# cbiffle/rtiow-rust

Hardware: AMD Instinct MI355X
Metric: Msamples/s (pixels*spp/s), book-1 random-spheres 1200x800 (higher is better)
Workload: dtype f32

## Files before the change

include/rtiow_gpu_debug.h:

```cpp
#ifndef RTIOW_GPU_DEBUG_H
#define RTIOW_GPU_DEBUG_H
#include "rtiow_gpu.h"
#ifdef __cplusplus
extern "C" {
#endif

int rtg_debug_box_plan(rtg_builder* b, const rtg_id* world, size_t n, const uint32_t* words, size_t n_records,
                       uint8_t* mask_out, size_t capacity);

int rtg_debug_production_program(rtg_builder* b, const rtg_id* world, size_t n, const uint32_t* words, size_t n_records,
                                 uint32_t* words_out, uint32_t* origin_out, uint8_t* mask_out, size_t capacity);

#ifdef __cplusplus
}
#endif
#endif
```

rtiow-rust_amd/capi.py:

```python
import ctypes as C
import math
import os
import time

import numpy as np

from . import noise

c_f32p = C.POINTER(C.c_float)
c_u32p = C.POINTER(C.c_uint32)
c_u8p = C.POINTER(C.c_uint8)

INVALID_ID = 0xFFFFFFFF
FLAG_COUNTERS = 1
FLAG_TRACE_KERNEL = 2
FLAG_PARTIAL = 4
FLAG_RESUME = 8
FLAG_SUM_SQUARES = 16
FLAG_SAMPLE_COUNTS = 32
FLAG_RETIRE = 64
RETIRE_MAX_RADIUS = 8
FLAG_DENOISE = 128
DENOISE_MAX_RADIUS = 8
DENOISE_MAX_PATCH = 3
# ... 288 lines not shown

    def copy_in(self, out=None, counts=None, retire=None):
        if out is not None:
            self.planes[...] = out
        if counts is not None:
            self.counts[...] = counts
        if retire is not None:
            C.memmove(C.addressof(self.retire), C.addressof(retire), C.sizeof(Retire))

    def copy_back(self, out=None, counts=None, retire=None):
        if out is not None:
            out[...] = self.planes
        if counts is not None:
            counts[...] = self.counts
        if retire is not None:
            C.memmove(C.addressof(retire), C.addressof(self.retire), C.sizeof(Retire))


class CountsFrame(Frame):

    def __init__(self, nx, ny, squares=False, retire=False, background=None):
        if retire and not squares:
            raise ValueError("a retire frame has two float planes: squares=True")
        super().__init__(nx, ny, squares, True, retire, background=background)


class DenoiseFrame(Frame):

    def __init__(self, nx, ny, counts=False, retire=False, denoise=None, error=False, background=None):
        super().__init__(nx, ny, True, counts, retire, denoise if _given(denoise) else True, None, error, background)


class FeaturesFrame(Frame):

    def __init__(self, nx, ny, squares=False, counts=False, retire=False, denoise=None, features=None, error=False, background=None):
        super().__init__(nx, ny, squares, counts, retire, denoise, features if _given(features) else True, error, background)


def features_frame(nx, ny, squares=False, counts=False, retire=False, denoise=None, features=None, error=False):
    return FeaturesFrame(nx, ny, squares, counts, retire, denoise, features, error)


def denoise_frame(nx, ny, counts=False, retire=False, denoise=None, error=False):
    return DenoiseFrame(nx, ny, counts, retire, denoise, error)


def counts_frame(nx, ny, squares=False, retire=False):
    return CountsFrame(nx, ny, squares, retire)


def _counts_call(out, counts, nx, ny, squares, retire=None):
    counts = np.asarray(counts)
    if counts.shape != (ny, nx):
        raise ValueError("counts= must have shape (ny, nx) = %s" % ((ny, nx),))
    if (out.dtype == np.float32 and out.flags.c_contiguous and counts.dtype == np.uint32 and counts.flags.c_contiguous
            and out.ctypes.data + out.nbytes == counts.ctypes.data
            and (retire is None or C.addressof(retire) == out.ctypes.data + retire_block_offset(nx, ny))):
        return out, None
    f = CountsFrame(nx, ny, squares, retire is not None)
    f.copy_in(out, counts, retire)
    return f.planes, f


def _host_frame(out, nx, ny, squares, kw):
    shape = (2, ny, nx, 3) if squares else (ny, nx, 3)
    if out is None:
        if _resumes(kw):
            raise ValueError("resume=True needs out= (the running sum to continue)")
        return np.zeros(shape, dtype=np.float32)
    if squares and not (isinstance(out, np.ndarray) and out.shape == shape and out.dtype == np.float32 and out.flags.c_contiguous):
        raise ValueError("squares=True needs out= a C-contiguous float32 array of shape %s" % (shape,))
    return out


def _render(supported, call, nx, ny, ns, seed, stats, out, counters, counts, retire, denoise, features, kw, exact, forward=False):
    kw = dict(kw)
    squares = kw.pop("squares", None)
    error = kw.pop("error", None)
    background = kw.pop("background", None)
    has_rt, has_dn, has_ft, has_er = _given(retire), _given(denoise), _given(features), _given(error)
    has_bg = _given(background)
    in_place = isinstance(out, Frame)
    f = None
    plain = forward and not (in_place or isinstance(counts, np.ndarray) or isinstance(retire, Retire) or has_bg
                             or isinstance(denoise, (dict, Denoise)) or isinstance(features, (dict, Features)))
    if plain:
        flags, parts = {"squares": squares, "counts": counts, "retire": retire, "denoise": denoise, "features": features}, ()
        if has_er:
            flags["error"], parts = True, ("error",)
    else:
        if has_er and not (has_dn or (in_place and out.denoise is not None)):
            raise ValueError("error=True needs denoise= (the filter writes the error plane)")
        if has_dn and not squares and (exact or not in_place):
            raise ValueError("denoise= needs squares=True (the filter reads both planes)")
        blocks = [make(x) for x, make in ((denoise, make_denoise), (features, make_features), (background, make_background))
                  if _given(x) and x is not True]
        if in_place:
            f, name = out, type(out).__name__
            if (f.nx, f.ny) != (nx, ny):
                raise ValueError("out= is a %s of another size" % name)
            if isinstance(counts, np.ndarray) or (exact and (counts is not None or retire is not None)):
                raise ValueError("out= a %s brings its own counts / retire views" % name)
            if has_ft and f.features is None:
                raise ValueError("features=: out= must be a FeaturesFrame or an array")
            if (has_dn and f.denoise is None) or (has_rt and f.retire is None):
                raise ValueError("out= a %s has no such block" % name)
            if ((squares is not None or exact) and bool(squares) != f.squares) or (
                    exact and (has_dn != (f.denoise is not None) or has_ft != (f.features is not None))):
                raise ValueError("out= a %s: squares= / denoise= / features= must say what the frame holds" % name)
            if (has_er and f.error is None) or (exact and not has_er and f.error is not None):
                raise ValueError("out= a %s: error= must say whether the frame has an error plane" % name)
            if has_bg and f.background is None:
                raise ValueError("background=: out= a %s has no background block (make the frame with background=)" % name)
            if isinstance(retire, Retire):
                blocks.append(retire)
            flags = f.flags()
        else:
            if has_rt and not (isinstance(retire, Retire) and isinstance(counts, np.ndarray) and squares):
                raise ValueError("retire= needs a Retire, squares=True and counts= a uint32 array (the call writes it)")
            if counts is not None and np.asarray(counts).shape != (ny, nx):
                raise ValueError("counts= must have shape (ny, nx) = %s" % ((ny, nx),))
            if out is None and _resumes(kw):
                raise ValueError("resume=True needs out= (the running sum to continue)")
            flags = {"squares": bool(squares), "counts": counts is not None, "retire": has_rt, "denoise": has_dn, "features": has_ft}
            if has_er:
                flags["error"] = True
            if has_bg:
                if background is True:
                    raise ValueError("background=True needs out= a frame that has the block")
                flags["background"] = True
        parts = sorted((part for part, on in flags.items() if on), key=lambda part: part != "error")
    for part in parts:
        supported(part)
    if in_place:
        for block in blocks:
            f.set_in(block)
        ret, buf = f, f.buf
    elif (has_dn or has_ft or has_bg) and not plain:
        bg = background if has_bg else None
        f = (FeaturesFrame(nx, ny, squares, counts is not None, has_rt, denoise if has_dn else None, features, has_er, bg) if has_ft else
             DenoiseFrame(nx, ny, counts is not None, has_rt, denoise, has_er, bg) if has_dn else
             Frame(nx, ny, squares, counts is not None, has_rt, background=bg))
        if not (has_dn or has_ft):
            out = _host_frame(out, nx, ny, squares, kw)
        f.copy_in(None if out is None else _host_frame(out, nx, ny, squares, kw), counts, retire if has_rt else None)
        ret, buf = f if has_dn or has_ft else out, f.buf
    else:
        ret = out = buf = _host_frame(out, nx, ny, squares, kw)
        if counts is not None and not plain:
            buf, f = _counts_call(out, counts, nx, ny, squares, retire if has_rt else None)
    p = make_params(nx, ny, ns, seed=seed, flags=FLAG_COUNTERS if stats and counters else 0, **flags, **kw)
    st = call(p, buf)
    if f is not None and not in_place:
        f.copy_back(out, counts if has_rt else None, retire if has_rt else None)
    return (ret, st.as_dict()) if stats else ret


def _adaptive_host(cast, nx, ny, ns, step, target_se, min_samples, budget_s, out, seed, stats, radius, denoise, features, kw,
                   error=False, background=None):
    if features is not None:
        f = FeaturesFrame(nx, ny, True, True, False, denoise, None, error, background) if out is None else out
        what = "features=: out= must be a FeaturesFrame(nx, ny, squares=True, counts=True, denoise=...)"
    elif denoise is not None:
        f = DenoiseFrame(nx, ny, True, error=error, background=background) if out is None else out
        what = "denoise=: out= must be a DenoiseFrame(nx, ny, counts=True)"
    else:
        f = CountsFrame(nx, ny, True, background=background) if out is None else out
        what = "out= must be a CountsFrame(nx, ny, squares=True)"
    on = {"denoise": True if denoise is not None else None, "features": True if features is not None else None}
    want = {"squares": True, "counts": True, "retire": False, "denoise": denoise is not None, "features": features is not None}
    if error:
        on["error"] = want["error"] = True
        what += " with error=True"
    if background is not None:
        on["background"] = want["background"] = True
        what += " with background="
    if not isinstance(f, Frame) or (f.nx, f.ny) != (nx, ny) or f.flags() != want:
        raise ValueError(what)
    for block in (features, denoise, background):
        if block is not None:
            f.set_in(block)
    more = () if features is None else (f,)
    f.counts[...] = ns
    active = np.ones((ny, nx), dtype=bool)
    t0 = time.perf_counter()
    done = 0
    while done < ns:
        end = min(ns, done + step)
        _, st = cast(end, seed=seed, out=f, sample_begin=done, resume=True, partial=True, squares=True, stats=True, counters=False,
                     **on, **kw)
        if features is not None:
            f.features.compute = 0
        if stats is not None:
            stats.append(st)
        done = end
        held = np.minimum(f.counts, done).astype(np.uint32)
        se = f.error.copy() if error else noise.standard_error_counts(f.planes[0], f.planes[1], held)
        if error:
            retire = noise.retire_filtered(active, done, se, f.counts, min_samples, target_se, radius=radius)
        elif radius:
            retire = noise.retire(active, done, se, min_samples, target_se, radius=radius, present=f.counts > 0)
        else:
            retire = noise.retire(active, done, se, min_samples, target_se)
        f.counts[retire] = done
        active &= ~retire
        pv = CountsFrame(nx, ny)
        pv.copy_in(f.planes[0], held)
        cast(done, seed=seed, out=pv, sample_begin=done, resume=True, **kw)
        if denoise is not None:
            yield (held, pv.planes, se, f.denoised.copy()) + more
        else:
            yield (held, pv.planes, se) + more
        if not active.any():
            return
        if budget_s is not None and time.perf_counter() - t0 >= budget_s:
            return


ERR_INVALID, ERR_EMPTY_BVH, ERR_NAN, ERR_RANGE, ERR_UNSUPPORTED, ERR_DEVICE = -1, -2, -3, -4, -5, -6


class RtError(RuntimeError):
    def __init__(self, code, msg):
        super().__init__("rt error %d: %s" % (code, msg))
        self.code = code


def _f3(v):
    return (C.c_float * 3)(float(v[0]), float(v[1]), float(v[2]))


ABI_SYMBOLS = [
    "version", "last_error", "device_count", "builder_create", "builder_destroy",
    "texture_constant", "texture_checker", "texture_perlin", "builder_set_perlin_tables",
    "material_lambertian", "material_metal", "material_dielectric", "material_diffuse_light",
    "material_isotropic", "object_sphere", "object_rect", "object_flip_normals", "object_translate",
    "object_scale", "object_rotate_y", "object_and", "object_rect_prism", "object_linear_move",
    "object_constant_medium", "object_bvh", "object_bvh_sah", "camera_look", "scene_create", "scene_destroy",
    "scene_set_option", "scene_info", "par_cast", "par_cast_device", "par_cast_multi", "multi_reset", "debug_hit_top", "debug_samples", "debug_math", "debug_flatten", "debug_flatten_pool2", "tonemap", "tonemap_device",
]


class Backend:

    def __init__(self, path, prefix):
        if not os.path.exists(path):
            raise FileNotFoundError(
                "%s not found -- build it first (python -c 'import __graft_entry__ as g; g.build()')" % path)
        self.path = path
        self.prefix = prefix
        self.lib = C.CDLL(path)
        f = self._fn
        f("last_error", C.c_char_p, [])
        f("version", C.c_char_p, [])
        f("builder_create", C.c_int, [C.POINTER(C.c_void_p)])
        f("builder_destroy", None, [C.c_void_p])
        f("texture_constant", C.c_uint32, [C.c_void_p, c_f32p])
        f("texture_checker", C.c_uint32, [C.c_void_p, C.c_uint32, C.c_uint32])
        f("texture_perlin", C.c_uint32, [C.c_void_p, C.c_float])
        f("builder_set_perlin_tables", C.c_int, [C.c_void_p, c_f32p, c_u8p, c_u8p, c_u8p])
        f("material_lambertian", C.c_uint32, [C.c_void_p, C.c_uint32])
        f("material_metal", C.c_uint32, [C.c_void_p, c_f32p, C.c_float])
        f("material_dielectric", C.c_uint32, [C.c_void_p, C.c_float])
        f("material_diffuse_light", C.c_uint32, [C.c_void_p, C.c_uint32, C.c_float])
        f("material_isotropic", C.c_uint32, [C.c_void_p, C.c_uint32])
        f("object_sphere", C.c_uint32, [C.c_void_p, C.c_float, C.c_uint32])
        f("object_rect", C.c_uint32, [C.c_void_p, C.c_int] + [C.c_float] * 5 + [C.c_uint32])
        f("object_flip_normals", C.c_uint32, [C.c_void_p, C.c_uint32])
        f("object_translate", C.c_uint32, [C.c_void_p, c_f32p, C.c_uint32])
        f("object_scale", C.c_uint32, [C.c_void_p, c_f32p, C.c_uint32])
        f("object_rotate_y", C.c_uint32, [C.c_void_p, C.c_float, C.c_uint32])
        f("object_and", C.c_uint32, [C.c_void_p, C.c_uint32, C.c_uint32])
        f("object_rect_prism", C.c_uint32, [C.c_void_p, c_f32p, c_f32p, C.c_uint32])
        f("object_linear_move", C.c_uint32, [C.c_void_p, C.c_uint32, c_f32p])
        f("object_constant_medium", C.c_uint32, [C.c_void_p, C.c_uint32, C.c_float, C.c_uint32])
        f("object_bvh", C.c_uint32, [C.c_void_p, c_u32p, C.c_size_t, C.c_float, C.c_float])
        f("object_bvh_sah", C.c_uint32, [C.c_void_p, c_u32p, C.c_size_t, C.c_float, C.c_float])
        f("camera_look", C.c_int, [c_f32p, c_f32p, c_f32p] + [C.c_float] * 6 + [C.POINTER(Camera)])
        f("scene_create", C.c_int, [C.c_void_p, c_u32p, C.c_size_t, C.c_int, C.POINTER(C.c_void_p)])
        f("scene_destroy", None, [C.c_void_p])
        self._declare_render()
        f("debug_hit_top", C.c_int, [C.c_void_p, C.c_size_t, c_f32p, C.c_uint64, C.c_float, c_f32p, c_u32p])
        f("debug_samples", C.c_int, [C.c_void_p, C.POINTER(Camera), C.POINTER(Params), C.c_size_t,
                                     c_u32p, c_u32p, c_u32p, c_f32p, c_u32p])
        f("debug_math", C.c_int, [C.c_int, C.c_int, C.c_size_t, c_f32p, c_f32p, c_f32p])
        f("tonemap", C.c_int, [C.c_int, C.c_size_t, c_f32p, c_u8p])

    def _declare_render(self):
        f = self._fn
        f("device_count", C.c_int, [C.POINTER(C.c_int)])
        f("scene_set_option", C.c_int, [C.c_void_p, C.c_char_p, C.c_int])
        f("scene_info", C.c_int, [C.c_void_p, c_u32p, c_u32p, c_u32p, C.POINTER(C.c_uint64), c_u32p])
        f("par_cast", C.c_int, [C.c_void_p, C.POINTER(Camera), C.POINTER(Params), c_f32p, C.POINTER(Stats)])
        f("par_cast_device", C.c_int, [C.c_void_p, C.POINTER(Camera), C.POINTER(Params), C.c_void_p,
                                       C.c_void_p, C.POINTER(Stats)])
        f("par_cast_multi", C.c_int, [C.POINTER(C.c_void_p), C.c_int, C.POINTER(Camera), C.POINTER(Params), c_f32p,
                                      C.POINTER(Stats)])
        f("multi_reset", C.c_int, [C.c_char_p, C.POINTER(C.c_uint64)])
        f("debug_flatten", C.c_int, [C.c_void_p, c_u32p, C.c_size_t, c_u32p, c_u32p, c_u32p, C.c_size_t])
        f("debug_flatten_pool2", C.c_int, [C.c_void_p, c_u32p, C.c_size_t, c_u32p, c_u32p, c_u32p, C.c_size_t])
        f("tonemap_device", C.c_int, [C.c_int, C.c_size_t, C.c_void_p, C.c_void_p, C.c_void_p])
        f("debug_box_plan", C.c_int, [C.c_void_p, c_u32p, C.c_size_t, c_u32p, C.c_size_t, c_u8p, C.c_size_t])
        f("debug_production_program", C.c_int, [C.c_void_p, c_u32p, C.c_size_t, c_u32p, C.c_size_t, c_u32p, c_u32p, c_u8p, C.c_size_t])

    def _fn(self, name, restype, argtypes):
        try:
            fn = getattr(self.lib, self.prefix + name)
        except AttributeError:
            def fn(*_a, _n=self.prefix + name):
                raise RtError(ERR_INVALID, "%s: symbol %s is not exported by this build" % (self.path, _n))
            setattr(self, "_" + name, fn)
            return fn
        fn.restype = restype
        fn.argtypes = argtypes
        setattr(self, "_" + name, fn)
        return fn

    def last_error(self):
        return (self._last_error() or b"").decode()

    def check(self, code):
        if code != 0:
            raise RtError(code, self.last_error())

    def check_id(self, i):
        if i == INVALID_ID:
            raise RtError(-1, self.last_error())
        return i

    def builder(self):
        return Builder(self)

    def device_count(self):
        n = C.c_int(0)
        self.check(self._device_count(C.byref(n)))
        return n.value

    def camera_look(self, look_from, look_at, up, fov, aspect, aperture, focus_dist, exposure=(0.0, 1.0)):
        cam = Camera()
        self.check(self._camera_look(_f3(look_from), _f3(look_at), _f3(up), fov, aspect, aperture,
                                     focus_dist, exposure[0], exposure[1], C.byref(cam)))
        return cam

    def par_cast_multi(self, scenes, camera, nx, ny, ns, seed=0xDEADBEEF, stats=False, out=None, counters=None, **kw):
        kw = dict(kw)
        counts, retire, denoise, features = (kw.pop(k, None) for k in ("counts", "retire", "denoise", "features"))
        return _render(lambda part: _supported(self, part), lambda p, buf: self._par_cast_multi_call(scenes, camera, p, buf),
                       nx, ny, ns, seed, stats, out, True if counters is None else counters, counts, retire, denoise, features, kw,
                       exact=False, forward=True)

    def _par_cast_multi_call(self, scenes, camera, p, buf):
        st = Stats.new()
        arr = (C.c_void_p * len(scenes))(*[s.h for s in scenes])
        self.check(self._par_cast_multi(arr, len(scenes), C.byref(camera), C.byref(p), buf.ctypes.data_as(c_f32p), C.byref(st)))
        return st

    def adaptive_multi(self, scenes, camera, nx, ny, ns, step, target_se, min_samples=16, budget_s=None, out=None, seed=0xDEADBEEF,
                       stats=None, radius=0, denoise=None, features=None, filtered_error=False, **kw):
        if step < 1:
            raise ValueError("step must be >= 1")
        if not 0 <= radius <= RETIRE_MAX_RADIUS:
            raise ValueError("radius must be in 0 .. %d" % RETIRE_MAX_RADIUS)
        if filtered_error:
            _supported(self, "error")
        _supported(self, "squares")
        _supported(self, "counts")
        if filtered_error and not _given(denoise):
            raise ValueError("filtered_error=True needs denoise= (the filter writes the error plane)")
        features = make_features(features) if _given(features) else None
        denoise = make_denoise(denoise) if _given(denoise) else None
        background = kw.pop("background", None)
        if _given(background):
            _supported(self, "background")
        background = make_background(background) if _given(background) else None
        yield from _adaptive_host(lambda n, **k: self.par_cast_multi(scenes, camera, nx, ny, n, **k), nx, ny, ns, step,
                                  target_se, min_samples, budget_s, out, seed, stats, radius, denoise, features, kw, bool(filtered_error),
                                  background)

    def multi_reset(self, rccl_library=None):
        n = C.c_uint64(0)
        self.check(self._multi_reset(rccl_library.encode() if rccl_library else None, C.byref(n)))
        return n.value

    def tonemap(self, img, device=0):
        x = np.ascontiguousarray(img, dtype=np.float32)
        out = np.empty(x.shape, dtype=np.uint8)
        self.check(self._tonemap(device, x.size, x.ctypes.data_as(c_f32p), out.ctypes.data_as(c_u8p)))
        return out

    def debug_math(self, op, x, y=None, device=0):
        x = np.ascontiguousarray(x, dtype=np.float32)
        out = np.empty_like(x)
        yp = None
        if y is not None:
            y = np.ascontiguousarray(y, dtype=np.float32)
            yp = y.ctypes.data_as(c_f32p)
        self.check(self._debug_math(device, op, x.size, x.ctypes.data_as(c_f32p), yp,
                                    out.ctypes.data_as(c_f32p)))
        return out


class Builder:

    def __init__(self, backend):
        self.be = backend
        h = C.c_void_p()
        backend.check(backend._builder_create(C.byref(h)))
        self.h = h
        self._scenes = []

    def close(self):
        if self.h:
            self.be._builder_destroy(self.h)
            self.h = None

    def __del__(self):
        try:
            self.close()
        except Exception:
            pass

    def constant(self, color):
        return self.be.check_id(self.be._texture_constant(self.h, _f3(color)))

    def checker(self, t0, t1):
        return self.be.check_id(self.be._texture_checker(self.h, t0, t1))

    def perlin(self, scale):
        return self.be.check_id(self.be._texture_perlin(self.h, scale))

    def set_perlin_tables(self, vecs, perm_x, perm_y, perm_z):
        vecs = np.ascontiguousarray(vecs, dtype=np.float32).reshape(768)
        px, py, pz = (np.ascontiguousarray(a, dtype=np.uint8) for a in (perm_x, perm_y, perm_z))
        self.be.check(self.be._builder_set_perlin_tables(
            self.h, vecs.ctypes.data_as(c_f32p), px.ctypes.data_as(c_u8p), py.ctypes.data_as(c_u8p),
            pz.ctypes.data_as(c_u8p)))

    def lambertian(self, albedo):
        return self.be.check_id(self.be._material_lambertian(self.h, albedo))

    def metal(self, albedo, fuzz):
        return self.be.check_id(self.be._material_metal(self.h, _f3(albedo), fuzz))

    def dielectric(self, ref_idx):
        return self.be.check_id(self.be._material_dielectric(self.h, ref_idx))

    def diffuse_light(self, emission, brightness):
        return self.be.check_id(self.be._material_diffuse_light(self.h, emission, brightness))

    def isotropic(self, albedo):
        return self.be.check_id(self.be._material_isotropic(self.h, albedo))

    def sphere(self, radius, material):
        return self.be.check_id(self.be._object_sphere(self.h, radius, material))

    def rect(self, orthogonal_to, range0, range1, k, material):
        return self.be.check_id(self.be._object_rect(self.h, orthogonal_to, range0[0], range0[1],
                                                     range1[0], range1[1], k, material))

    def flip_normals(self, obj):
        return self.be.check_id(self.be._object_flip_normals(self.h, obj))

    def translate(self, offset, obj):
        return self.be.check_id(self.be._object_translate(self.h, _f3(offset), obj))

    def scale(self, factor, obj):
        return self.be.check_id(self.be._object_scale(self.h, _f3(factor), obj))

    def rotate_y(self, degrees, obj):
        return self.be.check_id(self.be._object_rotate_y(self.h, degrees, obj))

    def and_(self, a, b):
        return self.be.check_id(self.be._object_and(self.h, a, b))

    def rect_prism(self, p0, p1, material):
        return self.be.check_id(self.be._object_rect_prism(self.h, _f3(p0), _f3(p1), material))

    def linear_move(self, obj, motion):
        return self.be.check_id(self.be._object_linear_move(self.h, obj, _f3(motion)))

    def constant_medium(self, boundary, density, material):
        return self.be.check_id(self.be._object_constant_medium(self.h, boundary, density, material))

    def bvh(self, objs, exposure=(0.0, 1.0)):
        arr = (C.c_uint32 * max(1, len(objs)))(*objs)
        return self.be.check_id(self.be._object_bvh(self.h, arr, len(objs), exposure[0], exposure[1]))

    def flatten(self, world):
        arr = (C.c_uint32 * max(1, len(world)))(*world)
        n, feat = C.c_uint32(), C.c_uint32()
        self.be.check(self.be._debug_flatten(self.h, arr, len(world), C.byref(n), C.byref(feat), None, 0))
        words = np.zeros((n.value, 8), dtype=np.uint32)
        self.be.check(self.be._debug_flatten(self.h, arr, len(world), C.byref(n), C.byref(feat),
                                             words.ctypes.data_as(c_u32p), n.value))
        return words, feat.value

    def flatten_pool2(self, world):
        arr = (C.c_uint32 * max(1, len(world)))(*world)
        n = C.c_uint32()
        table = np.zeros(24, dtype=np.uint32)
        self.be.check(self.be._debug_flatten_pool2(self.h, arr, len(world), C.byref(n), table.ctypes.data_as(c_u32p), None, 0))
        words = np.zeros((n.value, 8), dtype=np.uint32)
        self.be.check(self.be._debug_flatten_pool2(self.h, arr, len(world), C.byref(n), table.ctypes.data_as(c_u32p),
                                                   words.ctypes.data_as(c_u32p), n.value))
        items = [tuple(int(v) for v in table[4 * k:4 * k + 4]) for k in range(int(table[20]))]
        return words, items, int(table[21]), int(table[22])

    def box_plan(self, world=None, words=None):
        if words is not None:
            words = np.ascontiguousarray(words, dtype=np.uint32)
            mask = np.zeros(len(words), dtype=np.uint8)
            n = self.be._debug_box_plan(None, None, 0, words.ctypes.data_as(c_u32p), len(words), mask.ctypes.data_as(c_u8p), len(mask))
        else:
            arr = (C.c_uint32 * max(1, len(world)))(*world)
            n = self.be._debug_box_plan(self.h, arr, len(world), None, 0, None, 0)
            if n < 0:
                self.be.check(n)
            mask = np.zeros(n, dtype=np.uint8)
            n = self.be._debug_box_plan(self.h, arr, len(world), None, 0, mask.ctypes.data_as(c_u8p), len(mask))
        if n < 0:
            self.be.check(n)
        return mask

    def production_program(self, world=None, words=None):
        if words is not None:
            words = np.ascontiguousarray(words, dtype=np.uint32)
            head = (None, None, 0, words.ctypes.data_as(c_u32p), len(words))
            n = len(words)
        else:
            arr = (C.c_uint32 * max(1, len(world)))(*world)
            head = (self.h, arr, len(world), None, 0)
            n = self.be._debug_production_program(*head, None, None, None, 0)
            if n < 0:
                self.be.check(n)
        out = np.zeros((n, 8), dtype=np.uint32)
        origin = np.zeros(n, dtype=np.uint32)
        mask = np.zeros(n, dtype=np.uint8)
        n = self.be._debug_production_program(*head, out.ctypes.data_as(c_u32p), origin.ctypes.data_as(c_u32p), mask.ctypes.data_as(c_u8p), n)
        if n < 0:
            self.be.check(n)
        return out, origin, mask

    def bvh_sah(self, objs, exposure=(0.0, 1.0)):
        arr = (C.c_uint32 * max(1, len(objs)))(*objs)
        return self.be.check_id(self.be._object_bvh_sah(self.h, arr, len(objs), exposure[0], exposure[1]))

    def scene(self, world, device=0):
        arr = (C.c_uint32 * max(1, len(world)))(*world)
        h = C.c_void_p()
        self.be.check(self.be._scene_create(self.h, arr, len(world), device, C.byref(h)))
        sc = self.be.scene_class(self.be, h, self)
        sc.apply_env_options()
        return sc


class Scene:
    def __init__(self, backend, handle, builder):
        self.be = backend
        self.h = handle
        self._builder = builder

    def close(self):
        if self.h:
            self.be._scene_destroy(self.h)
            self.h = None

    def __del__(self):
        try:
            self.close()
        except Exception:
            pass

    ENV_OPTIONS = ("kernel", "chunks", "lpt", "lpt_phase1", "lpt_deep", "lpt_shift", "ray_lds", "sync", "block", "wg_per_cu", "window",
                   "box_leave", "refill_min", "gather_min", "run_ahead", "run_ahead_min", "sphere_min", "verbose", "bvh4", "box_chains", "box_prune", "box_tree", "force_rccl", "multi_gather", "multi_planes", "scratch_mb", "frames_in_flight", "small_frames", "drain_share", "hoist", "deep_sized", "mat_lds", "pool2", "p2_refill", "p2_box_leave", "p2_park", "p2_sphere", "p2_prism", "p2_list", "p2_push", "light_sampling")

    def set_option(self, name, value):
        self.be.check(self.be._scene_set_option(self.h, name.encode(), int(value)))

    def apply_env_options(self):
        if not hasattr(self.be, "_scene_set_option"):
            return
        for name in self.ENV_OPTIONS:
            v = os.environ.get("RTG_" + name.upper())
            if v is not None:
                self.set_option(name, int(v))

    def info(self):
        a, b, c, d, e = C.c_uint32(), C.c_uint32(), C.c_uint32(), C.c_uint64(), C.c_uint32()
        self.be.check(self.be._scene_info(self.h, C.byref(a), C.byref(b), C.byref(c), C.byref(d), C.byref(e)))
        return {"instructions": a.value, "materials": b.value, "textures": c.value, "hbm_bytes": d.value, "box_followers": e.value}

    def _par_cast_args(self, args, threads):
        return args

    def par_cast(self, camera, nx, ny, ns, seed=0xDEADBEEF, stats=False, out=None, threads=0, counts=None, counters=None,
                 retire=None, denoise=None, features=None, **kw):
        def call(p, buf):
            st = Stats.new()
            self.be.check(self.be._par_cast(*self._par_cast_args(
                [self.h, C.byref(camera), C.byref(p), buf.ctypes.data_as(c_f32p), C.byref(st)], threads)))
            return st
        return _render(lambda part: _supported(self.be, part), call, nx, ny, ns, seed, stats, out,
                       stats if counters is None else counters, counts, retire, denoise, features, kw, exact=True)

    def par_cast_device(self, camera, params, d_out_ptr, stream=None, want_stats=False, sample_begin=None, partial=None,
                        resume=None, squares=None, counts=None, retire=None, denoise=None, features=None, error=None,
                        background=None):
        if _given(background) and background is not True:
            background = make_background(background)
        over = {"squares": squares, "counts": counts, "retire": retire, "denoise": denoise, "features": features, "error": error,
                "background": background}
        bits = {"squares": FLAG_SUM_SQUARES, "counts": FLAG_SAMPLE_COUNTS, "retire": FLAG_RETIRE, "denoise": FLAG_DENOISE,
                "features": FLAG_FEATURES, "error": FLAG_DENOISE_ERROR, "background": FLAG_BACKGROUND}
        has = {part: bool(params.flags & bits[part] if on is None else on if isinstance(on, (bool, int)) else True)
               for part, on in over.items()}
        for part in ("background", "error", "features", "denoise", "squares", "counts", "retire"):
            if has[part] if part == "squares" else _given(over[part]):
                _supported(self.be, part)
        if has["error"] and not has["denoise"]:
            raise ValueError("error=True needs the denoise part (the filter writes the error plane)")
        lay = FrameLayout(params.nx, params.ny, **has)
        blocks = [(over[part], 4 * at, n) for part, at, n in (("retire", lay.retire, C.sizeof(Retire)),
                                                             ("denoise", lay.denoise, Denoise.OUT_OFFSET),
                                                             ("features", lay.features, Features.OUT_OFFSET),
                                                             ("background", lay.background, Background.OUT_OFFSET))
                  if isinstance(over[part], C.Structure)]
        for block, at, n in blocks:
            self._block_copy(d_out_ptr, block, stream, True, at, n)
        if _given(counts) and counts is not True:
            self._upload_counts(lay, counts, d_out_ptr, stream)
        if sample_begin is not None or partial is not None or resume is not None or any(on is not None for on in over.values()):
            q = Params()
            C.pointer(q)[0] = params
            if sample_begin is not None:
                q.sample_begin = sample_begin
            for on, bit in [(partial, FLAG_PARTIAL), (resume, FLAG_RESUME)] + [(on if on is None else has[part], bits[part])
                                                                             for part, on in over.items()]:
                if on is not None:
                    q.flags = (q.flags | bit) if on else (q.flags & ~bit)
            params = q
        st = Stats.new()
        self.be.check(self.be._par_cast_device(self.h, C.byref(camera), C.byref(params), d_out_ptr, stream,
                                               C.byref(st) if want_stats else None))
        for block, at, _ in blocks:
            self._block_copy(d_out_ptr, block, stream, False, at, C.sizeof(block))
        return st.as_dict() if want_stats else None

    def _block_copy(self, d_out_ptr, block, stream, to_device, offset, nbytes):
        hip, hs = _hip_runtime(), _stream(stream)
        dev, host = C.c_void_p(_device_ptr(d_out_ptr) + offset), C.c_void_p(C.addressof(block))
        what = "hipMemcpyAsync(%s block)" % type(block).__name__.lower()
        _hip_ok(hip.hipMemcpyAsync(*((dev, host, nbytes, 1) if to_device else (host, dev, nbytes, 2)), hs), what)
        _hip_ok(hip.hipStreamSynchronize(hs), what)

    def _upload_counts(self, lay, counts, d_out_ptr, stream):
        hip, hs = _hip_runtime(), _stream(stream)
        dst = C.c_void_p(_device_ptr(d_out_ptr) + 4 * lay.counts)
        if hasattr(counts, "data_ptr") and getattr(counts, "is_cuda", False):
            if tuple(counts.shape) != (lay.ny, lay.nx) or counts.element_size() != 4 or not counts.is_contiguous():
                raise ValueError("counts= must be a contiguous 4-byte [ny, nx] tensor")
            _hip_ok(hip.hipMemcpyAsync(dst, C.c_void_p(counts.data_ptr()), 4 * lay.n, 3, hs), "hipMemcpyAsync(count plane)")
        else:
            host = np.ascontiguousarray(counts, dtype=np.uint32)
            if host.shape != (lay.ny, lay.nx):
                raise ValueError("counts= must have shape (ny, nx) = %s" % ((lay.ny, lay.nx),))
            _hip_ok(hip.hipMemcpyAsync(dst, C.c_void_p(host.ctypes.data), 4 * lay.n, 1, hs), "hipMemcpyAsync(count plane)")
            _hip_ok(hip.hipStreamSynchronize(hs), "hipMemcpyAsync(count plane)")

    def _loop_block(self, part, given, make):
        if not _given(given):
            return None
        _supported(self.be, part)
        return make(given)

    def adaptive(self, camera, nx, ny, ns, step, target_se, min_samples=16, budget_s=None, out=None, seed=0xDEADBEEF,
                 stats=None, radius=0, preview=None, stream=None, denoise=None, denoised=None, features=None,
                 filtered_error=False, **kw):
        if step < 1:
            raise ValueError("step must be >= 1")
        if filtered_error:
            _supported(self.be, "error")
        _supported(self.be, "squares")
        _supported(self.be, "counts")
        if not 0 <= radius <= RETIRE_MAX_RADIUS:
            raise ValueError("radius must be in 0 .. %d" % RETIRE_MAX_RADIUS)
        if filtered_error and not _given(denoise):
            raise ValueError("filtered_error=True needs denoise= (the filter writes the error plane)")
        features, denoise = self._loop_block("features", features, make_features), self._loop_block("denoise", denoise, make_denoise)
        background = self._loop_block("background", kw.pop("background", None), make_background)
        if out is not None and not isinstance(out, Frame):
            _supported(self.be, "retire")
            if preview is None:
                raise ValueError("a device frame needs a device preview buffer (preview=)")
            if denoise is not None and denoised is None:
                raise ValueError("denoise= on a device frame needs a device buffer for the filtered frame (denoised=)")
            yield from self._adaptive_device(camera, nx, ny, ns, step, target_se, min_samples, budget_s, out, seed, stats,
                                             radius, preview, stream, kw, denoise, denoised, features, bool(filtered_error), background)
            return
        yield from _adaptive_host(lambda n, **k: self.par_cast(camera, nx, ny, n, **k), nx, ny, ns, step, target_se,
                                  min_samples, budget_s, out, seed, stats, radius, denoise, features, kw, bool(filtered_error), background)

    def _adaptive_device(self, camera, nx, ny, ns, step, target_se, min_samples, budget_s, out, seed, stats, radius, preview,
                         stream, kw, denoise=None, denoised=None, features=None, error=False, background=None):
        hip, hs, ok = _hip_runtime(), _stream(stream), _hip_ok
        d_out, d_pv = _device_ptr(out), _device_ptr(preview)
        lay = FrameLayout(nx, ny, True, True, True, denoise is not None, features is not None, error, background is not None)
        if background is not None:
            self._block_copy(d_out, background, stream, True, 4 * lay.background, Background.OUT_OFFSET)
        plane, counts_at = lay.n, d_out + 4 * lay.counts
        ok(hip.hipMemsetD32Async(C.c_void_p(counts_at), ns - (1 << 32) if ns >= 1 << 31 else ns, plane, hs), "hipMemsetD32Async(counts)")
        block = Retire(target_se=float(target_se), min_samples=int(min_samples), radius=int(radius))
        self._block_copy(d_out, block, stream, True, 4 * lay.retire, C.sizeof(Retire))
        if denoise is not None:
            self._block_copy(d_out, denoise, stream, True, 4 * lay.denoise, Denoise.OUT_OFFSET)
        more = ()
        if features is not None:
            self._block_copy(d_out, features, stream, True, 4 * lay.features, Features.OUT_OFFSET)
            more = (4 * lay.features,)
        t0 = time.perf_counter()
        done = 0
        while done < ns:
            end = min(ns, done + step)
            st = self.par_cast_device(camera, make_params(nx, ny, end, seed=seed, sample_begin=done, resume=True, partial=True,
                                                          squares=True, counts=True, retire=True, denoise=denoise is not None,
                                                          features=features is not None, error=error,
                                                          background=background is not None, **kw), d_out, hs,
                                      want_stats=stats is not None)
            if features is not None and features.compute:
                features.compute = 0
                self._block_copy(d_out, features, stream, True, 4 * lay.features, Features.OUT_OFFSET)
            if denoise is not None:
                ok(hip.hipMemcpyAsync(C.c_void_p(_device_ptr(denoised)), C.c_void_p(d_out + 4 * lay.denoised), plane * 3 * 4, 3, hs),
                   "hipMemcpyAsync(denoised)")
            if stats is not None:
                stats.append(st)
            done = end
            ok(hip.hipMemcpyAsync(C.c_void_p(d_pv), C.c_void_p(d_out), plane * 3 * 4, 3, hs), "hipMemcpyAsync(preview)")
            ok(hip.hipMemcpyAsync(C.c_void_p(d_pv + plane * 3 * 4), C.c_void_p(counts_at), plane * 4, 3, hs), "hipMemcpyAsync(preview counts)")
            self.par_cast_device(camera, make_params(nx, ny, done, seed=seed, sample_begin=done, resume=True, counts=True, **kw),
                                 d_pv, hs)
            self._block_copy(d_out, block, stream, False, 4 * lay.retire, C.sizeof(Retire))
            info = block.as_dict()
            if denoise is not None:
                yield (done, preview, info, denoised) + more
            else:
                yield (done, preview, info) + more
            if info["active"] == 0:
                return
            if budget_s is not None and time.perf_counter() - t0 >= budget_s:
                return

    def progressive(self, camera, nx, ny, ns, step, seed=0xDEADBEEF, budget_s=None, out=None, preview=None, stream=None,
                    squares=False, target_rmse=None, denoise=None, denoised=None, features=None, **kw):
        if step < 1:
            raise ValueError("step must be >= 1")
        features = self._loop_block("features", features, make_features)
        background = self._loop_block("background", kw.pop("background", None), make_background)
        squares = bool(squares) or target_rmse is not None or _given(denoise)
        if squares:
            _supported(self.be, "squares")
        denoise = self._loop_block("denoise", denoise, make_denoise)
        if out is not None and not isinstance(out, np.ndarray):
            if target_rmse is not None:
                raise ValueError("target_rmse needs host frames: there is no device-side error reduction")
            if preview is None:
                raise ValueError("a device running sum needs a device preview buffer (preview=)")
            if denoise is not None and denoised is None:
                raise ValueError("denoise= on a device frame needs a device buffer for the filtered frame (denoised=)")
            yield from self._progressive_device(camera, nx, ny, ns, step, seed, budget_s, out, preview, stream, squares, kw,
                                                denoise, denoised, features, background)
            return
        shape = (2, ny, nx, 3) if squares else (ny, nx, 3)
        acc = np.zeros(shape, dtype=np.float32) if out is None else out
        frame = None
        if features is not None:
            frame = FeaturesFrame(nx, ny, squares, denoise=denoise, features=features, background=background)
        elif denoise is not None:
            frame = DenoiseFrame(nx, ny, denoise=denoise, background=background)
        elif background is not None:
            frame = Frame(nx, ny, squares, background=background)
        if frame is not None:
            frame.copy_in(acc)
        on = {"denoise": True if denoise is not None else None, "features": True if features is not None else None}
        if background is not None:
            on["background"] = True
        more = () if features is None else (frame,)
        sums = acc[0] if squares else acc
        t0 = time.perf_counter()
        done = 0
        while done < ns:
            end = min(ns, done + step)
            self.par_cast(camera, nx, ny, end, seed=seed, out=acc if frame is None else frame, sample_begin=done, resume=True, partial=True,
                          squares=squares, **on, **kw)
            if frame is not None:
                frame.copy_back(acc)
            if features is not None:
                frame.features.compute = 0
            done = end
            pv = sums.copy()
            self.par_cast(camera, nx, ny, done, seed=seed, out=pv, sample_begin=done, resume=True, **kw)
            if squares:
                se = noise.standard_error(acc[0], acc[1], done)
                if denoise is not None:
                    yield (done, pv, se, frame.denoised.copy()) + more
                else:
                    yield (done, pv, se) + more
                if target_rmse is not None and float(np.sqrt(np.mean(se * se))) <= target_rmse:
                    return
            else:
                yield (done, pv) + more
            if budget_s is not None and time.perf_counter() - t0 >= budget_s:
                return

    def _progressive_device(self, camera, nx, ny, ns, step, seed, budget_s, acc, preview, stream, squares, kw, denoise=None,
                            denoised=None, features=None, background=None):
        hip, hs = _hip_runtime(), _stream(stream)
        d_acc, d_preview = C.c_void_p(_device_ptr(acc)), C.c_void_p(_device_ptr(preview))
        lay = FrameLayout(nx, ny, squares, False, False, denoise is not None, features is not None, background=background is not None)
        if background is not None:
            self._block_copy(acc, background, stream, True, 4 * lay.background, Background.OUT_OFFSET)
        if denoise is not None:
            self._block_copy(acc, denoise, stream, True, 4 * lay.denoise, Denoise.OUT_OFFSET)
        more = ()
        if features is not None:
            self._block_copy(acc, features, stream, True, 4 * lay.features, Features.OUT_OFFSET)
            more = (4 * lay.features,)
        t0 = time.perf_counter()
        done = 0
        while done < ns:
            end = min(ns, done + step)
            self.par_cast_device(camera, make_params(nx, ny, end, seed=seed, sample_begin=done, resume=True, partial=True,
                                                     squares=squares, denoise=denoise is not None, features=features is not None,
                                                     background=background is not None, **kw), d_acc, hs)
            if features is not None and features.compute:
                features.compute = 0
                self._block_copy(acc, features, stream, True, 4 * lay.features, Features.OUT_OFFSET)
            done = end
            if denoise is not None:
                _hip_ok(hip.hipMemcpyAsync(C.c_void_p(_device_ptr(denoised)), C.c_void_p(d_acc.value + 4 * lay.denoised), lay.n * 3 * 4, 3, hs),
                        "hipMemcpyAsync(denoised)")
            _hip_ok(hip.hipMemcpyAsync(d_preview, d_acc, lay.n * 3 * 4, 3, hs), "hipMemcpyAsync(preview)")
            self.par_cast_device(camera, make_params(nx, ny, done, seed=seed, sample_begin=done, resume=True, **kw), d_preview, hs)
            if denoise is not None:
                yield (done, preview, acc, denoised) + more
            else:
                yield ((done, preview, acc) if squares else (done, preview)) + more
            if budget_s is not None:
                _hip_ok(hip.hipStreamSynchronize(hs), "hipStreamSynchronize")
                if time.perf_counter() - t0 >= budget_s:
                    return

    def debug_hit_top(self, rays, seed=1, t_near=0.001):
        rays = np.ascontiguousarray(rays, dtype=np.float32).reshape(-1, 7)
        n = rays.shape[0]
        out = np.zeros((n, 8), dtype=np.float32)
        mat = np.zeros(n, dtype=np.uint32)
        self.be.check(self.be._debug_hit_top(self.h, n, rays.ctypes.data_as(c_f32p), seed, t_near,
                                             out.ctypes.data_as(c_f32p), mat.ctypes.data_as(c_u32p)))
        return out, mat

    def debug_samples(self, camera, nx, ny, ns, xs, ys, samples, seed=0xDEADBEEF, trace_kernel=False, **kw):
        p = make_params(nx, ny, ns, seed=seed, flags=FLAG_TRACE_KERNEL if trace_kernel else 0, **kw)
        xs, ys, samples = (np.ascontiguousarray(a, dtype=np.uint32) for a in (xs, ys, samples))
        n = xs.size
        rgb = np.zeros((n, 3), dtype=np.float32)
        info = np.zeros((n, 4), dtype=np.uint32)
        self.be.check(self.be._debug_samples(self.h, C.byref(camera), C.byref(p), n,
                                             xs.ctypes.data_as(c_u32p), ys.ctypes.data_as(c_u32p),
                                             samples.ctypes.data_as(c_u32p), rgb.ctypes.data_as(c_f32p),
                                             info.ctypes.data_as(c_u32p)))
        return rgb, info


Backend.scene_class = Scene
```

rtiow-rust_amd/csrc/rt_box_plan.h:

```cpp
#pragma once
#include <cmath>
#include <cstddef>
#include <cstdint>
#include <cstring>
#include <vector>

#include "flat_scene.h"

namespace rtg {

constexpr uint8_t BOX_KEPT = 0, BOX_FOLLOWER = 1, BOX_PRUNED = 2;
#ifndef RT_BOX_PLAN_PROBES
#define RT_BOX_PLAN_PROBES 256
#endif
#ifndef RT_BOX_PLAN_FULL
#define RT_BOX_PLAN_FULL 0
#endif
constexpr uint32_t BOX_PLAN_PROBES = RT_BOX_PLAN_PROBES;
constexpr bool BOX_PLAN_FULL = RT_BOX_PLAN_FULL != 0;
enum BoxPlanKind : int { BOX_PLAN_SURE = 0, BOX_PLAN_PROBE_DP = 1, BOX_PLAN_AREA = 2 };
constexpr BoxPlanKind BOX_PLAN_DEFAULT = BOX_PLAN_FULL ? BOX_PLAN_PROBE_DP : BOX_PLAN_SURE;
#ifndef RT_BOX_TREE_PLAN
#define RT_BOX_TREE_PLAN 2
#endif
constexpr BoxPlanKind BOX_TREE_PLAN = (BoxPlanKind)(RT_BOX_TREE_PLAN);

struct BoxPlan {
  uint32_t n_pruned = 0;
  uint32_t n_sure = 0;
  uint32_t n_rays = 0;
};

namespace box_plan_detail {
inline float as_f(uint32_t u) {
  float f;
  std::memcpy(&f, &u, 4);
  return f;
}
inline bool aabb_hit(const uint32_t* lo, const uint32_t* hi, const float* o, const float* inv, float t_near, float best) {
  const float mn[3] = {as_f(lo[0]), as_f(lo[2]), as_f(hi[0])}, mx[3] = {as_f(lo[1]), as_f(lo[3]), as_f(hi[1])};
  float t0[3], t1[3];
  for (int a = 0; a < 3; a++) {
    const float u = (mn[a] - o[a]) * inv[a], v = (mx[a] - o[a]) * inv[a];
    t0[a] = inv[a] < 0.f ? v : u, t1[a] = inv[a] < 0.f ? u : v;
  }
  const float start = fmaxf(t_near, fmaxf(fmaxf(t0[0], t0[1]), t0[2]));
  const float end = fminf(best, fminf(fminf(t1[0], t1[1]), t1[2]));
  return end > start;
}
inline bool sphere_hit(const uint32_t* lo, uint32_t flags, const float* o, const float* d, float dd, float t_near, float best, float* t_out) {
  float p[3] = {o[0], o[1], o[2]};
  if (flags & F_TRANSLATE)
    for (int a = 0; a < 3; a++) p[a] = o[a] - as_f(lo[a]);
  const float r = as_f(lo[3]);
  const float b = p[0] * d[0] + p[1] * d[1] + p[2] * d[2];
  const float c = p[0] * p[0] + p[1] * p[1] + p[2] * p[2] - r * r;
  const float disc = b * b - dd * c;
  if (disc > 0.f) {
    const float sq = sqrtf(disc);
    float t = (-b - sq) / dd;
    if (t < best && t >= t_near) return *t_out = t, true;
    t = (-b + sq) / dd;
    if (t < best && t >= t_near) return *t_out = t, true;
  }
  return false;
}
struct Rng {
  uint64_t s;
  uint64_t next() {
    uint64_t z = (s += 0x9e3779b97f4a7c15ull);
    z = (z ^ (z >> 30)) * 0xbf58476d1ce4e5b9ull;
    z = (z ^ (z >> 27)) * 0x94d049bb133111ebull;
    return z ^ (z >> 31);
  }
  float unit() { return (float)(next() >> 40) * (1.f / 16777216.f); }
  void in_unit_sphere(float* v) {
    do {
      for (int a = 0; a < 3; a++) v[a] = 2.f * unit() - 1.f;
    } while (v[0] * v[0] + v[1] * v[1] + v[2] * v[2] >= 1.f);
  }
};
inline bool finite6(const uint32_t* lo, const uint32_t* hi) {
  return std::isfinite(as_f(lo[0])) && std::isfinite(as_f(lo[1])) && std::isfinite(as_f(lo[2])) && std::isfinite(as_f(lo[3])) &&
         std::isfinite(as_f(hi[0])) && std::isfinite(as_f(hi[1]));
}
inline double box_area(const uint32_t* lo, const uint32_t* hi) {
  const double dx = (double)as_f(lo[1]) - (double)as_f(lo[0]), dy = (double)as_f(lo[3]) - (double)as_f(lo[2]),
               dz = (double)as_f(hi[1]) - (double)as_f(hi[0]);
  return 2.0 * (dx * dy + dy * dz + dz * dx);
}
struct Shape {
  std::vector<int32_t> parent;
  std::vector<uint32_t> depth;
  std::vector<uint8_t> prunable;
  uint32_t n_prunable = 0;
};
inline bool leaf_box_at(const uint32_t (*hi)[4], size_t n, size_t j) {
  return (hi[j][3] & 0xffu) == OP_BOX && j + 2 < n && (hi[j + 1][3] & 0xffu) == OP_SPHERE && hi[j][2] == j + 2;
}
inline bool program_shape(const uint32_t (*lo)[4], const uint32_t (*hi)[4], size_t n, Shape* sh) {
  auto op = [&](size_t j) { return hi[j][3] & 0xffu; };
  auto skip = [&](size_t j) { return (size_t)hi[j][2]; };
  sh->parent.assign(n, -1), sh->depth.assign(n, 0), sh->prunable.assign(n, 0), sh->n_prunable = 0;
  if (n < 4 || n > 0x7fffffffu) return false;
  std::vector<uint32_t> open;
  for (size_t j = 0; j < n; j++) {
    while (!open.empty() && skip(open.back()) <= j) open.pop_back();
    if (!open.empty()) sh->parent[j] = (int32_t)open.back(), sh->depth[j] = (uint32_t)open.size();
    if (op(j) != OP_BOX) continue;
    if (skip(j) <= j || skip(j) >= n || (!open.empty() && skip(j) > skip(open.back()))) return false;
    open.push_back((uint32_t)j);
  }
  auto contains = [&](size_t j, size_t c) {
    return as_f(lo[j][0]) <= as_f(lo[c][0]) && as_f(lo[j][1]) >= as_f(lo[c][1]) && as_f(lo[j][2]) <= as_f(lo[c][2]) &&
           as_f(lo[j][3]) >= as_f(lo[c][3]) && as_f(hi[j][0]) <= as_f(hi[c][0]) && as_f(hi[j][1]) >= as_f(hi[c][1]);
  };
  for (size_t j = n; j-- > 0;) {
    if (op(j) != OP_BOX || j + 1 >= n || op(j + 1) != OP_BOX) continue;
    const size_t L = j + 1, R = skip(L);
    if (!(L < R && R < skip(j)) || op(R) != OP_BOX || skip(R) != skip(j)) continue;
    if (!finite6(lo[j], hi[j]) || !finite6(lo[L], hi[L]) || !finite6(lo[R], hi[R]) || !contains(j, L) || !contains(j, R)) continue;
    if (!(leaf_box_at(hi, n, L) || sh->prunable[L]) || !(leaf_box_at(hi, n, R) || sh->prunable[R])) continue;
    sh->prunable[j] = 1, sh->n_prunable++;
  }
  return true;
}
}

inline BoxPlan box_plan(const uint32_t (*lo)[4], const uint32_t (*hi)[4], size_t n, const uint8_t* follower, uint8_t* mask,
                        uint8_t* sure = nullptr, uint32_t n_probes = BOX_PLAN_PROBES, BoxPlanKind kind = BOX_PLAN_DEFAULT) {
  using namespace box_plan_detail;
  BoxPlan out;
  for (size_t j = 0; j < n; j++) {
    mask[j] = follower && follower[j] ? BOX_FOLLOWER : BOX_KEPT;
    if (sure) sure[j] = 0;
  }
  auto op = [&](size_t j) { return hi[j][3] & 0xffu; };
  auto skip = [&](size_t j) { return (size_t)hi[j][2]; };
  Shape shape;
  if (!program_shape(lo, hi, n, &shape) || !shape.n_prunable) return out;
  const std::vector<int32_t>& parent = shape.parent;
  const std::vector<uint32_t>& depth = shape.depth;
  const std::vector<uint8_t>& prunable = shape.prunable;
  auto leaf_box = [&](size_t j) { return leaf_box_at(hi, n, j); };
  std::vector<uint8_t> choosable(prunable);
  for (size_t j = 0; j + 1 < n; j++) {
    if (!prunable[j] || !follower) continue;
    size_t k = j + 1;
    while (k + 1 < n && follower[k] && !leaf_box(k)) k++;
    if (follower[k] && leaf_box(k)) choosable[j] = 0;
  }

  std::vector<uint64_t> n_pass(n, 0);
  std::vector<uint32_t> spheres, starts;
  for (size_t j = 0; j < n; j++)
    if (op(j) == OP_SPHERE) spheres.push_back((uint32_t)j);
  auto centre = [&](uint32_t j, float* c) {
    for (int a = 0; a < 3; a++) c[a] = (hi[j][3] & F_TRANSLATE) ? as_f(lo[j][a]) : 0.f;
  };
  float cmin[3] = {INFINITY, INFINITY, INFINITY}, cmax[3] = {-INFINITY, -INFINITY, -INFINITY};
  for (uint32_t j : spheres) {
    float c[3];
    centre(j, c);
    for (int a = 0; a < 3; a++) cmin[a] = fminf(cmin[a], c[a]), cmax[a] = fmaxf(cmax[a], c[a]);
  }
  std::vector<uint8_t> enclosing(n, 0);
  for (uint32_t j : spheres) {
    float cj[3];
    centre(j, cj);
    const float r = as_f(lo[j][3]);
    float far2 = 0.f;
    for (int a = 0; a < 3; a++) {
      const float d = fmaxf(cmax[a] - cj[a], cj[a] - cmin[a]);
      far2 += d * d;
    }
    const bool all = spheres.size() > 1 && far2 < r * r;
    enclosing[j] = all;
    if (!all && std::isfinite(r) && std::isfinite(cj[0]) && std::isfinite(cj[1]) && std::isfinite(cj[2])) starts.push_back(j);
  }
  uint64_t n_rays = 0;
  if (!starts.empty() && kind != BOX_PLAN_AREA) {
    Rng rng{0x626f78706c616e31ull ^ (uint64_t)n};
    const float t_near = 0.001f;
    while (n_rays < n_probes) {
      const uint32_t s0 = starts[rng.next() % starts.size()];
      float c[3], nrm[3], o[3], d[3], v[3];
      centre(s0, c);
      do rng.in_unit_sphere(nrm);
      while (nrm[0] * nrm[0] + nrm[1] * nrm[1] + nrm[2] * nrm[2] < 1e-4f);
      const float len = sqrtf(nrm[0] * nrm[0] + nrm[1] * nrm[1] + nrm[2] * nrm[2]), r0 = as_f(lo[s0][3]);
      for (int a = 0; a < 3; a++) nrm[a] /= len, o[a] = c[a] + r0 * nrm[a];
      const uint32_t bounces = 1u + (uint32_t)(rng.next() % 3u);
      for (uint32_t k = 0; k <= bounces && n_rays < n_probes; k++) {
        rng.in_unit_sphere(v);
        for (int a = 0; a < 3; a++) d[a] = nrm[a] + v[a];
        const float inv[3] = {1.f / d[0], 1.f / d[1], 1.f / d[2]};
        const float dd = d[0] * d[0] + d[1] * d[1] + d[2] * d[2];
        float best = 3.402823466e+38f;
        int64_t best_pc = -1;
        n_rays++;
        for (size_t pc = 0; pc < n;) {
          const uint32_t o_ = op(pc);
          if (o_ == OP_BOX) {
            if (aabb_hit(lo[pc], hi[pc], o, inv, t_near, best)) n_pass[pc]++, pc++;
            else pc = skip(pc);
          } else if (o_ == OP_SPHERE) {
            float t;
            if (sphere_hit(lo[pc], hi[pc][3], o, d, dd, t_near, best, &t)) best = t, best_pc = (int64_t)pc;
            pc++;
          } else break;
        }
        if (best_pc < 0 || enclosing[best_pc]) break;
        centre((uint32_t)best_pc, c);
        const float r = as_f(lo[best_pc][3]);
        for (int a = 0; a < 3; a++) o[a] = o[a] + best * d[a], nrm[a] = (o[a] - c[a]) / r;
        if (!(std::isfinite(nrm[0]) && std::isfinite(nrm[1]) && std::isfinite(nrm[2]))) break;
      }
    }
  }
  out.n_rays = (uint32_t)n_rays;
  if (kind == BOX_PLAN_AREA) {
    constexpr uint64_t ONE = 1ull << 30;
    float rmin[3] = {INFINITY, INFINITY, INFINITY}, rmax[3] = {-INFINITY, -INFINITY, -INFINITY};
    for (size_t j = 0; j + 1 < n; j++) {
      if (!leaf_box(j) || enclosing[j + 1] || !finite6(lo[j], hi[j])) continue;
      const float mn[3] = {as_f(lo[j][0]), as_f(lo[j][2]), as_f(hi[j][0])}, mx[3] = {as_f(lo[j][1]), as_f(lo[j][3]), as_f(hi[j][1])};
      for (int a = 0; a < 3; a++) rmin[a] = fminf(rmin[a], mn[a]), rmax[a] = fmaxf(rmax[a], mx[a]);
    }
    const double dx = (double)rmax[0] - rmin[0], dy = (double)rmax[1] - rmin[1], dz = (double)rmax[2] - rmin[2];
    const double sa_ref = 2.0 * (dx * dy + dy * dz + dz * dx);
    if (!(sa_ref > 0.0) || !std::isfinite(sa_ref)) return out;
    for (size_t j = 0; j < n; j++) {
      if (op(j) != OP_BOX) continue;
      const double r = finite6(lo[j], hi[j]) ? box_area(lo[j], hi[j]) / sa_ref : 1.0;
      n_pass[j] = r >= 1.0 ? ONE : (r > 0.0 ? (uint64_t)(r * (double)ONE) : 0u);
    }
    n_rays = ONE;
  }

  uint64_t states = 0;
  for (size_t j = 0; kind != BOX_PLAN_SURE && j < n; j++)
    if (op(j) == OP_BOX) states += depth[j] + 2u;
  const bool dp = kind != BOX_PLAN_SURE && states <= (1ull << 26);
  std::vector<uint32_t> kidx(n, 0);
  std::vector<uint8_t> pruned(n, 0);
  if (dp) {
    std::vector<uint64_t> at(n + 1, 0);
    for (size_t j = 0; j < n; j++) at[j + 1] = at[j] + (op(j) == OP_BOX ? depth[j] + 2u : 0u);
    std::vector<uint64_t> acc(at[n], 0);
    std::vector<uint8_t> choice(at[n], 0);
    std::vector<uint64_t> path_pass, f;
    for (size_t j = n; j-- > 0;) {
      if (op(j) != OP_BOX) continue;
      const uint32_t dj = depth[j];
      uint64_t* acc_j = &acc[at[j]];
      uint8_t* choice_j = &choice[at[j]];
      path_pass.assign(dj + 1u, n_rays);
      for (int32_t a = parent[j], k = (int32_t)dj; a >= 0; a = parent[a], k--) path_pass[k] = n_pass[a];
      f.assign(dj + 1u, 0);
      for (uint32_t k = 0; k <= dj; k++) {
        const uint64_t own = follower && follower[j] ? 0u : path_pass[k];
        const uint64_t keep = own + acc_j[dj + 1u], leave = acc_j[k];
        if (choosable[j] && leave <= keep) f[k] = leave, choice_j[k] = 1;
        else f[k] = keep;
      }
      if (parent[j] >= 0) {
        uint64_t* up = &acc[at[parent[j]]];
        for (uint32_t k = 0; k <= dj; k++) up[k] += f[k];
      }
    }
    for (size_t j = 0; j < n; j++) {
      if (op(j) != OP_BOX) continue;
      const int32_t p = parent[j];
      kidx[j] = p < 0 ? 0u : (pruned[p] ? kidx[p] : depth[j]);
      pruned[j] = choice[at[j] + kidx[j]];
    }
  } else {
    for (size_t j = 0; j < n; j++) pruned[j] = choosable[j] && n_rays && n_pass[j] == n_rays && op(j) == OP_BOX;
  }
  for (size_t j = 0; j < n; j++) {
    if (!pruned[j] || mask[j] == BOX_FOLLOWER) continue;
    mask[j] = BOX_PRUNED, out.n_pruned++;
    if (n_pass[j] == n_rays) {
      out.n_sure++;
      if (sure) sure[j] = 1;
    }
  }
  return out;
}

constexpr uint32_t BOX_TREE_NEW = 0xffffffffu;
inline uint32_t box_tree_rebuild(const uint32_t (*lo)[4], const uint32_t (*hi)[4], size_t n, uint32_t (*out_lo)[4],
                                 uint32_t (*out_hi)[4], uint32_t* origin) {
  using namespace box_plan_detail;
  for (size_t j = 0; j < n; j++) {
    std::memcpy(out_lo[j], lo[j], 16), std::memcpy(out_hi[j], hi[j], 16);
    origin[j] = (uint32_t)j;
  }
  Shape shape;
  if (!program_shape(lo, hi, n, &shape) || !shape.n_prunable) return 0;
  struct Box { float mn[3], mx[3]; };
  auto merge = [](const Box& a, const Box& b) {
    Box m;
    for (int x = 0; x < 3; x++) m.mn[x] = b.mn[x] < a.mn[x] ? b.mn[x] : a.mn[x], m.mx[x] = b.mx[x] > a.mx[x] ? b.mx[x] : a.mx[x];
    return m;
  };
  auto area = [](const Box& b) {
    const double dx = (double)b.mx[0] - b.mn[0], dy = (double)b.mx[1] - b.mn[1], dz = (double)b.mx[2] - b.mn[2];
    return 2.0 * (dx * dy + dy * dz + dz * dx);
  };
  std::vector<uint32_t> leaf;
  std::vector<Box> box;
  std::vector<double> suffix;
  struct Job { uint32_t a, b, at; };
  std::vector<Job> jobs;
  std::vector<uint32_t> rec_lo, rec_hi, rec_origin;
  uint32_t regions = 0;
  for (size_t j = 0; j < n; j++) {
    if (!shape.prunable[j]) continue;
    const size_t end = hi[j][2];
    if (shape.parent[j] >= 0 && shape.prunable[shape.parent[j]]) continue;
    leaf.clear(), box.clear();
    bool ok = true;
    for (size_t i = j; i < end; i++) {
      if (!leaf_box_at(hi, n, i)) continue;
      ok = ok && finite6(lo[i], hi[i]);
      leaf.push_back((uint32_t)i);
      box.push_back(Box{{as_f(lo[i][0]), as_f(lo[i][2]), as_f(hi[i][0])}, {as_f(lo[i][1]), as_f(lo[i][3]), as_f(hi[i][1])}});
    }
    const size_t m = leaf.size();
    if (!ok || m < 2 || 3 * m - 1 != end - j) { j = end - 1; continue; }
    uint64_t budget = 64ull * m, work = 0;
    for (size_t v = m; v > 1; v >>= 1) budget += 64ull * m;
    const size_t len = end - j;
    rec_lo.assign(4 * len, 0), rec_hi.assign(4 * len, 0), rec_origin.assign(len, BOX_TREE_NEW);
    suffix.resize(m);
    jobs.clear();
    jobs.push_back(Job{0u, (uint32_t)m, 0u});
    while (!jobs.empty() && ok) {
      const Job t = jobs.back();
      jobs.pop_back();
      uint32_t* rl = &rec_lo[4 * t.at];
      uint32_t* rh = &rec_hi[4 * t.at];
      if (t.b - t.a == 1) {
        const uint32_t src = leaf[t.a];
        std::memcpy(rl, lo[src], 16), std::memcpy(rh, hi[src], 16), std::memcpy(rl + 4, lo[src + 1], 16), std::memcpy(rh + 4, hi[src + 1], 16);
        rh[2] = (uint32_t)j + t.at + 2u;
        rec_origin[t.at] = src, rec_origin[t.at + 1] = src + 1u;
        continue;
      }
      work += 2ull * (t.b - t.a);
      if (work > budget) { ok = false; break; }
      Box run = box[t.b - 1];
      for (uint32_t k = t.b - 1; k > t.a; k--) run = k == t.b - 1 ? run : merge(box[k], run), suffix[k] = area(run);
      run = box[t.a];
      uint32_t best_k = t.a + 1;
      double best_cost = INFINITY;
      for (uint32_t k = t.a + 1; k < t.b; k++) {
        if (k > t.a + 1) run = merge(run, box[k - 1]);
        const double cost = area(run) * (double)(k - t.a) + suffix[k] * (double)(t.b - k);
        if (cost < best_cost) best_cost = cost, best_k = k;
      }
      const Box all = merge(run, box[t.b - 1]);
      const float f[6] = {all.mn[0], all.mx[0], all.mn[1], all.mx[1], all.mn[2], all.mx[2]};
      std::memcpy(rl, f, 16), std::memcpy(rh, f + 4, 8);
      rh[2] = (uint32_t)j + t.at + 3u * (t.b - t.a) - 1u;
      rh[3] = t.at == 0u ? hi[j][3] : (hi[j][3] & ~F_BVH_ROOT);
      jobs.push_back(Job{best_k, t.b, t.at + 1u + 3u * (best_k - t.a) - 1u});
      jobs.push_back(Job{t.a, best_k, t.at + 1u});
    }
    if (ok) {
      for (size_t i = 0; i < len; i++) {
        std::memcpy(out_lo[j + i], &rec_lo[4 * i], 16), std::memcpy(out_hi[j + i], &rec_hi[4 * i], 16);
        origin[j + i] = rec_origin[i];
      }
      regions++;
    }
    j = end - 1;
  }
  return regions;
}

}
```

rtiow-rust_amd/csrc/rtg_api.hip:

```cpp
#include <hip/hip_runtime.h>

#include <dlfcn.h>
#include <rccl/rccl.h>

#include <chrono>
#include <cmath>
#include <cstdio>
#include <cstdlib>
#include <cstring>
#include <map>
#include <mutex>
#include <functional>
#include <string>
#include <tuple>
#include <vector>

#include "../../include/rtiow_gpu.h"
#include "../../include/rtiow_gpu_debug.h"
#include "rt_pool.h"
#include "rt_box_plan.h"
#include "rt_retire.h"
#include "rt_denoise.h"
#include "rt_features.h"
#include "rt_multi_planes.h"
#include "rt_pool_full.h"
#include "rt_sync_full.h"
#include "rt_pool2.h"
#include "rt_trace.h"
#include "rt_light.h"
#include "scene_builder.h"

using namespace rtg;

#include "rtg_kernels.inc"

namespace {
thread_local std::string g_err;

int fail(int code, const std::string& msg) {
  g_err = msg;
  return code;
}
int hip_fail(hipError_t e, const char* what) {
  return fail(RTG_ERR_DEVICE, std::string(what) + ": " + hipGetErrorString(e));
}
#define HIP_TRY(expr)                                   \
  do {                                                  \
    hipError_t e_ = (expr);                             \
    if (e_ != hipSuccess) return hip_fail(e_, #expr);   \
  } while (0)
}

struct rtg_builder {
  SceneBuilder sb;
};

constexpr int RTG_MAX_FRAMES = 4;
enum class KernelKind { baseline, lean_pool, full_pool, lock_step, pool2 };
struct LaunchCtx {
  unsigned long long* d_counters = nullptr;
  hipEvent_t ev0 = nullptr, ev1 = nullptr, done = nullptr;
  bool busy = false;
  float* d_stack = nullptr;
  size_t stack_bytes = 0;
  uint32_t* d_slots = nullptr;
  size_t slots_bytes = 0;
  float* d_scratch = nullptr;
  size_t scratch_bytes = 0;
  LaunchConsts* d_consts = nullptr;
  uint32_t* d_lpt = nullptr;
  size_t lpt_bytes = 0;
  LptQueue lpt_desc{};
  KernelKind last_kernel = KernelKind::baseline;
  uint32_t last_pix_work = 0;
  uint32_t* d_list = nullptr;
  size_t list_bytes = 0;
  uint32_t* d_compact = nullptr;
  size_t compact_bytes = 0;
  unsigned long long counts_samples = 0;
  void* d_retire = nullptr;
  size_t retire_bytes = 0;
  const char* refusal = nullptr;
  void* d_denoise = nullptr;
  size_t denoise_bytes = 0;
  uint32_t* d_features = nullptr;
  size_t features_bytes = 0;
};

struct LeanImages {
  const uint4* lo = nullptr;
  const uint4* hi = nullptr;
  const uint32_t* d_off = nullptr;
  uint32_t bytes = 0;
  uint32_t n_followers = 0;
  const uint32_t* d_chain_off = nullptr;
  uint32_t chain_bytes = 0;
  bool planned = false;
  uint32_t n_pruned = 0;
  float plan_ms = 0.f;
  const uint32_t* d_prune_off[2] = {nullptr, nullptr};
  uint32_t prune_bytes[2] = {0, 0};
  std::vector<uint32_t> plan_ops;
  std::vector<uint8_t> plan_mask;
  std::vector<uint8_t> follower;
  int slot = 12;
};

struct rtg_scene {
  int device = 0;
  DevScene dev{};
  uint32_t features = 0;
  uint32_t n_prog = 0, n_mat = 0, n_tex = 0;
  uint64_t bytes = 0;
  void* buffers[21] = {};
  const uint32_t* d_parent = nullptr;
  hipStream_t own_stream = nullptr;
  int num_cus = 0;
  float* d_frame = nullptr;
  size_t frame_bytes = 0;
  int force_chunks = 0;
  uint64_t scratch_limit = 0;
  bool whole_scratch = false;
  int verbose = 0;
  int window = -1;
  int ray_lds = 1;
  int force_rccl = 0;
  int multi_gather = 0;
  float* d_pack = nullptr;
  size_t pack_bytes = 0;
  float* d_recv = nullptr;
  size_t recv_bytes = 0;
  int multi_planes = 0;
  hipEvent_t post0 = nullptr, post1 = nullptr;
  hipEvent_t pack0 = nullptr, pack1 = nullptr, unpack0 = nullptr;
  int bvh4 = 0;
  uint32_t wide_bytes = 0;
  int box_chains = 1;
  int box_prune = 1;
  int box_tree = 1;
  LeanImages ref;
  LeanImages tree;
  bool tree_tried = false;
  float tree_ms = 0.f;
  uint32_t n_regions = 0;
  bool plannable = false;
  std::vector<Packet> h_lo, h_hi;
  int sync_full = -1;
  uint32_t n_box = 0;
  int lpt = 2;
  int lpt_deep = 4;
  int lpt_shift = 0;
  int lpt_phase1 = 0;
  int kernel_version = 3;
  PoolTuning pool_tune{40, 16, 24, 16, 16, 40};
  PoolTuning full_tune{20, 24, 32, 16, 24, 40};
  PoolTuning sync_tune{20, 16, 32, 16, 16, 40};
  int wg_per_cu = 0;
  int full_threads = 0;
  int pool_threads = 0;
  int mat_lds = 1;
  int deep_sized = 1;
  int hoist = 1;
  uint32_t seg_first = 0, seg_end = 0;
  int drain_share = 1;
  int pool2 = 1;
  uint32_t n_prog2 = 0, n_box2 = 0;
  DevScene dev2{};
  const P2Table* d_p2 = nullptr;
  Pool2Tuning pool2_tune{24, 48, 40, 4, 8, 24, 2};
  int guide_lds = 0;
  int small_frames = 1;
  int light_sampling = 0;
  uint32_t n_lights = 0;
  std::vector<LightRect> h_lights;
  std::vector<uint8_t> h_sampled;
  LightTable lights{nullptr, nullptr, 0};
  void* d_lights = nullptr;
  void* d_sampled = nullptr;
  LaunchCtx ctx[RTG_MAX_FRAMES];
  int n_ctx = 1, next_ctx = 0;
  LaunchCtx* cx = &ctx[0];
};

static void ctx_free_buffers(LaunchCtx* c) {
  if (c->busy) (void)hipEventSynchronize(c->done);
  c->busy = false;
  if (c->d_scratch) (void)hipFree(c->d_scratch);
  if (c->d_slots) (void)hipFree(c->d_slots);
  if (c->d_stack) (void)hipFree(c->d_stack);
  if (c->d_lpt) (void)hipFree(c->d_lpt);
  if (c->d_list) (void)hipFree(c->d_list);
  if (c->d_compact) (void)hipFree(c->d_compact);
  if (c->d_retire) (void)hipFree(c->d_retire);
  if (c->d_denoise) (void)hipFree(c->d_denoise);
  if (c->d_features) (void)hipFree(c->d_features);
  c->d_scratch = nullptr, c->scratch_bytes = 0, c->d_slots = nullptr, c->slots_bytes = 0;
  c->d_stack = nullptr, c->stack_bytes = 0, c->d_lpt = nullptr, c->lpt_bytes = 0;
  c->d_list = nullptr, c->list_bytes = 0, c->d_compact = nullptr, c->compact_bytes = 0;
  c->d_retire = nullptr, c->retire_bytes = 0;
  c->d_denoise = nullptr, c->denoise_bytes = 0;
  c->d_features = nullptr, c->features_bytes = 0;
}

static int ctx_acquire(rtg_scene* s) {
  LaunchCtx* c = &s->ctx[s->next_ctx];
  s->next_ctx = (s->next_ctx + 1) % s->n_ctx;
  if (!c->d_counters) {
    if (hipMalloc((void**)&c->d_counters, 64 * sizeof(unsigned long long)) != hipSuccess || hipMemset(c->d_counters, 0, 64 * sizeof(unsigned long long)) != hipSuccess ||
        hipMalloc((void**)&c->d_consts, sizeof(LaunchConsts) + sizeof(ListConsts)) != hipSuccess || hipEventCreate(&c->ev0) != hipSuccess ||
        hipEventCreate(&c->ev1) != hipSuccess || hipEventCreateWithFlags(&c->done, hipEventDisableTiming) != hipSuccess)
      return fail(RTG_ERR_DEVICE, "scene: launch-context allocation failed");
  }
  if (c->busy) {
    hipError_t e = hipEventSynchronize(c->done);
    c->busy = false;
    if (e != hipSuccess) return hip_fail(e, "hipEventSynchronize(previous frame of this launch context)");
  }
  s->cx = c;
  return RTG_OK;
}
static int ctx_release(rtg_scene* s, hipStream_t stream) {
  hipError_t e = hipEventRecord(s->cx->done, stream);
  if (e != hipSuccess) return hip_fail(e, "hipEventRecord(done)");
  s->cx->busy = true;
  return RTG_OK;
}

struct SampleSlice {
  uint32_t begin = 0;
  bool divide = true;
  bool squares = false;
  bool counts = false;
  uint32_t list_work = 0;
  ListConsts list{};
  bool retire = false;
  bool denoise = false;
  bool features = false;
  bool error = false;
  bool background = false;
  bool sliced() const { return begin != 0u || !divide; }
};
static SampleSlice slice_of(const rtg_params* p) {
  SampleSlice sl;
  if (p->flags & RTG_FLAG_RESUME) sl.begin = p->sample_begin;
  if (p->flags & RTG_FLAG_PARTIAL) sl.divide = false;
  if (p->flags & RTG_FLAG_SUM_SQUARES) sl.squares = true;
  if (p->flags & RTG_FLAG_SAMPLE_COUNTS) sl.counts = true;
  if (p->flags & RTG_FLAG_RETIRE) sl.retire = true;
  if (p->flags & RTG_FLAG_DENOISE) sl.denoise = true;
  if (p->flags & RTG_FLAG_FEATURES) sl.features = true;
  if (p->flags & RTG_FLAG_DENOISE_ERROR) sl.error = true;
  if (p->flags & RTG_FLAG_BACKGROUND) sl.background = true;
  return sl;
}

static const char* retire_refusal(const rtg_retire& r, uint32_t nranks) {
  if (r.radius > RTG_RETIRE_MAX_RADIUS) return "RTG_FLAG_RETIRE: radius > RTG_RETIRE_MAX_RADIUS";
  if (!(r.target_se >= 0.0)) return "RTG_FLAG_RETIRE: target_se is NaN or negative";
  if (r.radius > 0u && nranks > 1u) return "RTG_FLAG_RETIRE: radius > 0 needs nranks = 1 (the neighbours live on other ranks)";
  return nullptr;
}

static const char* denoise_refusal(const rtg_denoise& r, uint32_t nranks) {
  if (r.radius > RTG_DENOISE_MAX_RADIUS) return "RTG_FLAG_DENOISE: radius > RTG_DENOISE_MAX_RADIUS";
  if (r.patch > RTG_DENOISE_MAX_PATCH) return "RTG_FLAG_DENOISE: patch > RTG_DENOISE_MAX_PATCH";
  if (!(r.k > 0.f) || !std::isfinite(r.k)) return "RTG_FLAG_DENOISE: k is NaN, infinite or <= 0";
  if (r.reserved_in != 0u) return "RTG_FLAG_DENOISE: reserved_in != 0";
  if (nranks > 1u) return "RTG_FLAG_DENOISE needs nranks = 1 (the neighbours live on other ranks)";
  return nullptr;
}

static const char* features_refusal(const rtg_features& r, bool denoise) {
  if (r.grid == 0u || r.grid > RTG_FEATURES_MAX_GRID) return "RTG_FLAG_FEATURES: grid is 0 or > RTG_FEATURES_MAX_GRID";
  if (r.compute > 1u) return "RTG_FLAG_FEATURES: compute > 1";
  if (r.reserved_in != 0u) return "RTG_FLAG_FEATURES: reserved_in != 0";
  for (float sg : {r.sigma_normal, r.sigma_albedo, r.sigma_depth})
    if (denoise && (!(sg > 0.f) || !std::isfinite(sg))) return "RTG_FLAG_FEATURES with RTG_FLAG_DENOISE: a sigma is NaN, infinite or <= 0";
  return nullptr;
}

static const char* background_refusal(const rtg_background& r) {
  if (r.mode > 1u) return "RTG_FLAG_BACKGROUND: mode > 1";
  if (r.reserved_in != 0u) return "RTG_FLAG_BACKGROUND: reserved_in != 0";
  return nullptr;
}
static Background dev_background(const rtg_background& r) {
  Background b;
  b.mode = r.mode == 0u ? BG_CONSTANT : BG_GRADIENT;
  for (int c = 0; c < 3; c++) b.bottom[c] = r.bottom[c], b.top[c] = r.top[c];
  return b;
}

struct FrameBlocks {
  rtg_retire retire{};
  rtg_denoise denoise{};
  rtg_features features{};
  rtg_background background{};
};
static hipError_t read_blocks(const FrameLayout& L, const SampleSlice& sl, const float* d_out, hipStream_t stream, FrameBlocks* fb) {
  hipError_t e = hipSuccess;
  if (sl.retire) e = hipMemcpyAsync(&fb->retire, d_out + L.retire, offsetof(rtg_retire, active), hipMemcpyDeviceToHost, stream);
  if (e == hipSuccess && sl.denoise) e = hipMemcpyAsync(&fb->denoise, d_out + L.denoise, offsetof(rtg_denoise, filtered), hipMemcpyDeviceToHost, stream);
  if (e == hipSuccess && sl.features) e = hipMemcpyAsync(&fb->features, d_out + L.features, offsetof(rtg_features, traced), hipMemcpyDeviceToHost, stream);
  if (e == hipSuccess && sl.background) e = hipMemcpyAsync(&fb->background, d_out + L.background, offsetof(rtg_background, reserved), hipMemcpyDeviceToHost, stream);
  return e;
}
static const char* blocks_refusal(const SampleSlice& sl, const FrameBlocks& fb, uint32_t nranks) {
  const char* why = nullptr;
  if (sl.retire && (why = retire_refusal(fb.retire, nranks))) return why;
  if (sl.denoise && (why = denoise_refusal(fb.denoise, nranks))) return why;
  if (sl.features && (why = features_refusal(fb.features, sl.denoise))) return why;
  if (sl.background && (why = background_refusal(fb.background))) return why;
  return nullptr;
}

#include "rtg_launch.inc"

template <typename T>
struct DevBuf {
  T* p = nullptr;
  ~DevBuf() {
    if (p) (void)hipFree(p);
  }
  hipError_t alloc(size_t n) { return hipMalloc((void**)&p, (n ? n : 1) * sizeof(T)); }
};

extern "C" {

const char* rtg_version(void) { return "rtiow-rust_amd 0.2 (gfx950 HIP; flat-program ray-pool kernels; flat-program encoding 3: OP_SEG = 9, OP_SAVE / OP_MERGE / OP_EXT = 10 / 11 / 12, OP_LIST = 13, MEDIUM lo.y = 1 / density)"; }
const char* rtg_last_error(void) { return g_err.c_str(); }

int rtg_device_count(int* n) {
  if (!n) return fail(RTG_ERR_INVALID, "null argument");
  int c = 0;
  hipError_t e = hipGetDeviceCount(&c);
  if (e != hipSuccess) {
    *n = 0;
    return hip_fail(e, "hipGetDeviceCount");
  }
  *n = c;
  return RTG_OK;
}

int rtg_builder_create(rtg_builder** out) {
  if (!out) return fail(RTG_ERR_INVALID, "null argument");
  *out = new rtg_builder();
  return RTG_OK;
}
void rtg_builder_destroy(rtg_builder* b) { delete b; }

static rtg_id bad(const char* msg) {
  fail(RTG_ERR_INVALID, msg);
  return RTG_INVALID_ID;
}

rtg_id rtg_texture_constant(rtg_builder* b, const float rgb[3]) {
  if (!b || !rgb) return bad("null argument");
  HostTexture t;
  t.kind = TEX_CONSTANT;
  t.rgb[0] = rgb[0], t.rgb[1] = rgb[1], t.rgb[2] = rgb[2];
  b->sb.textures.push_back(t);
  return (rtg_id)b->sb.textures.size() - 1;
}
rtg_id rtg_texture_checker(rtg_builder* b, rtg_id t0, rtg_id t1) {
  if (!b) return bad("null argument");
  if (t0 >= b->sb.textures.size() || t1 >= b->sb.textures.size()) return bad("checker: bad texture handle");
  HostTexture t;
  t.kind = TEX_CHECKER;
  t.t0 = t0, t.t1 = t1;
  b->sb.textures.push_back(t);
  return (rtg_id)b->sb.textures.size() - 1;
}
rtg_id rtg_texture_perlin(rtg_builder* b, float scale) {
  if (!b) return bad("null argument");
  if (!b->sb.has_perlin) return bad("perlin: call rtg_builder_set_perlin_tables first");
  HostTexture t;
  t.kind = TEX_PERLIN;
  t.scale = scale;
  b->sb.textures.push_back(t);
  return (rtg_id)b->sb.textures.size() - 1;
}
int rtg_builder_set_perlin_tables(rtg_builder* b, const float vecs[768], const uint8_t px[256],
                                  const uint8_t py[256], const uint8_t pz[256]) {
  if (!b || !vecs || !px || !py || !pz) return fail(RTG_ERR_INVALID, "null argument");
  for (int i = 0; i < 256; i++) {
    b->sb.perlin_vecs[4 * i] = vecs[3 * i], b->sb.perlin_vecs[4 * i + 1] = vecs[3 * i + 1];
    b->sb.perlin_vecs[4 * i + 2] = vecs[3 * i + 2], b->sb.perlin_vecs[4 * i + 3] = 0.f;
    b->sb.perlin_perm[i] = px[i], b->sb.perlin_perm[256 + i] = py[i], b->sb.perlin_perm[512 + i] = pz[i];
  }
  b->sb.has_perlin = true;
  return RTG_OK;
}

static rtg_id push_material(rtg_builder* b, uint32_t kind, rtg_id tex, const float* albedo, float param) {
  if (!b) return bad("null argument");
  HostMaterial m;
  m.kind = kind;
  if (tex != RTG_INVALID_ID) {
    if (tex >= b->sb.textures.size()) return bad("material: bad texture handle");
    m.tex = tex;
  }
  if (albedo) m.albedo[0] = albedo[0], m.albedo[1] = albedo[1], m.albedo[2] = albedo[2];
  m.param = param;
  b->sb.materials.push_back(m);
  return (rtg_id)b->sb.materials.size() - 1;
}
rtg_id rtg_material_lambertian(rtg_builder* b, rtg_id albedo) {
  if (albedo == RTG_INVALID_ID) return bad("material: bad texture handle");
  return push_material(b, MAT_LAMBERTIAN, albedo, nullptr, 0.f);
}
rtg_id rtg_material_metal(rtg_builder* b, const float albedo[3], float fuzz) {
  if (!albedo) return bad("null argument");
  return push_material(b, MAT_METAL, RTG_INVALID_ID, albedo, fuzz);
}
rtg_id rtg_material_dielectric(rtg_builder* b, float ref_idx) {
  return push_material(b, MAT_DIELECTRIC, RTG_INVALID_ID, nullptr, ref_idx);
}
rtg_id rtg_material_diffuse_light(rtg_builder* b, rtg_id emission, float brightness) {
  if (emission == RTG_INVALID_ID) return bad("material: bad texture handle");
  return push_material(b, MAT_DIFFUSE_LIGHT, emission, nullptr, brightness);
}
rtg_id rtg_material_isotropic(rtg_builder* b, rtg_id albedo) {
  if (albedo == RTG_INVALID_ID) return bad("material: bad texture handle");
  return push_material(b, MAT_ISOTROPIC, albedo, nullptr, 0.f);
}

static rtg_id push_object(rtg_builder* b, const HostObject& o) {
  if (!b) return bad("null argument");
  try {
    return b->sb.add_object(o);
  } catch (const BuildError& e) {
    fail(e.code, e.msg);
    return RTG_INVALID_ID;
  }
}
rtg_id rtg_object_sphere(rtg_builder* b, float radius, rtg_id material) {
  HostObject o;
  o.kind = HostObject::SPHERE;
  o.f[0] = radius;
  o.mat = material;
  return push_object(b, o);
}
rtg_id rtg_object_rect(rtg_builder* b, int axis, float r0s, float r0e, float r1s, float r1e, float k, rtg_id material) {
  HostObject o;
  o.kind = HostObject::RECT;
  o.axis = axis;
  o.f[0] = k, o.f[1] = r0s, o.f[2] = r0e, o.f[3] = r1s, o.f[4] = r1e;
  o.mat = material;
  return push_object(b, o);
}
static rtg_id wrapper(rtg_builder* b, HostObject::Kind kind, const float* v, rtg_id child) {
  HostObject o;
  o.kind = kind;
  if (v) o.f[0] = v[0], o.f[1] = v[1], o.f[2] = v[2];
  o.a = child;
  return push_object(b, o);
}
rtg_id rtg_object_flip_normals(rtg_builder* b, rtg_id object) { return wrapper(b, HostObject::FLIP, nullptr, object); }
rtg_id rtg_object_translate(rtg_builder* b, const float offset[3], rtg_id object) {
  if (!offset) return bad("null argument");
  return wrapper(b, HostObject::TRANSLATE, offset, object);
}
rtg_id rtg_object_scale(rtg_builder* b, const float factor[3], rtg_id object) {
  if (!factor) return bad("null argument");
  return wrapper(b, HostObject::SCALE, factor, object);
}
rtg_id rtg_object_rotate_y(rtg_builder* b, float degrees, rtg_id object) {
  float radians = degrees * 3.14159265358979323846f / 180.f;
  float sc[3] = {sinf(radians), cosf(radians), 0.f};
  return wrapper(b, HostObject::ROTATE_Y, sc, object);
}
rtg_id rtg_object_and(rtg_builder* b, rtg_id o0, rtg_id o1) {
  HostObject o;
  o.kind = HostObject::AND;
  o.a = o0, o.b = o1;
  return push_object(b, o);
}
rtg_id rtg_object_rect_prism(rtg_builder* b, const float p0[3], const float p1[3], rtg_id m) {
  if (!b || !p0 || !p1) return bad("null argument");
  rtg_id zp = rtg_object_rect(b, 2, p0[0], p1[0], p0[1], p1[1], p1[2], m);
  rtg_id yp = rtg_object_rect(b, 1, p0[0], p1[0], p0[2], p1[2], p1[1], m);
  rtg_id xp = rtg_object_rect(b, 0, p0[1], p1[1], p0[2], p1[2], p1[0], m);
  if (zp == RTG_INVALID_ID || yp == RTG_INVALID_ID || xp == RTG_INVALID_ID) return RTG_INVALID_ID;
  rtg_id zn = rtg_object_flip_normals(b, rtg_object_rect(b, 2, p0[0], p1[0], p0[1], p1[1], p0[2], m));
  rtg_id yn = rtg_object_flip_normals(b, rtg_object_rect(b, 1, p0[0], p1[0], p0[2], p1[2], p0[1], m));
  rtg_id xn = rtg_object_flip_normals(b, rtg_object_rect(b, 0, p0[1], p1[1], p0[2], p1[2], p0[0], m));
  return rtg_object_and(b, rtg_object_and(b, zp, rtg_object_and(b, yp, xp)),
                        rtg_object_and(b, zn, rtg_object_and(b, yn, xn)));
}
rtg_id rtg_object_linear_move(rtg_builder* b, rtg_id object, const float motion[3]) {
  if (!motion) return bad("null argument");
  return wrapper(b, HostObject::MOVE, motion, object);
}
rtg_id rtg_object_constant_medium(rtg_builder* b, rtg_id boundary, float density, rtg_id material) {
  HostObject o;
  o.kind = HostObject::MEDIUM;
  o.f[0] = density;
  o.a = boundary;
  o.mat = material;
  return push_object(b, o);
}
rtg_id rtg_object_bvh(rtg_builder* b, const rtg_id* objects, size_t n, float e0, float e1) {
  if (!b || (!objects && n)) return bad("null argument");
  try {
    return b->sb.add_bvh(objects, n, e0, e1);
  } catch (const BuildError& e) {
    fail(e.code, e.msg);
    return RTG_INVALID_ID;
  }
}

rtg_id rtg_object_bvh_sah(rtg_builder* b, const rtg_id* objects, size_t n, float e0, float e1) {
  if (!b || (!objects && n)) return bad("null argument");
  try {
    return b->sb.add_bvh(objects, n, e0, e1, true);
  } catch (const BuildError& e) {
    fail(e.code, e.msg);
    return RTG_INVALID_ID;
  }
}

int rtg_camera_look(const float from[3], const float at[3], const float up[3], float fov, float aspect,
                    float aperture, float focus_dist, float e0, float e1, rtg_camera* out) {
  if (!from || !at || !up || !out) return fail(RTG_ERR_INVALID, "null argument");
  auto dot3 = [](const float* a, const float* b) { return (a[0] * b[0] + a[1] * b[1]) + a[2] * b[2]; };
  auto unit = [&](float* v) {
    float len = sqrtf(dot3(v, v));
    v[0] = v[0] / len, v[1] = v[1] / len, v[2] = v[2] / len;
  };
  auto cross3 = [](const float* a, const float* b, float* r) {
    r[0] = a[1] * b[2] - a[2] * b[1];
    r[1] = -(a[0] * b[2] - a[2] * b[0]);
    r[2] = a[0] * b[1] - a[1] * b[0];
  };
  float lens_radius = aperture / 2.f;
  float theta = fov * 3.14159265358979323846f / 180.f;
  float half_height = tanf(theta / 2.f);
  float half_width = aspect * half_height;
  float w[3] = {from[0] - at[0], from[1] - at[1], from[2] - at[2]};
  unit(w);
  float u[3], v[3];
  cross3(up, w, u);
  unit(u);
  cross3(w, u, v);
  float hw_fd = half_width * focus_dist, hh_fd = half_height * focus_dist;
  float h2 = (2.f * half_width) * focus_dist, v2 = (2.f * half_height) * focus_dist;
  for (int i = 0; i < 3; i++) {
    out->origin[i] = from[i];
    out->lower_left_corner[i] = ((from[i] - hw_fd * u[i]) - hh_fd * v[i]) - focus_dist * w[i];
    out->horizontal[i] = h2 * u[i];
    out->vertical[i] = v2 * v[i];
    out->u[i] = u[i];
    out->v[i] = v[i];
  }
  out->lens_radius = lens_radius;
  out->exposure_start = e0;
  out->exposure_end = e1;
  return RTG_OK;
}

static int upload(void** dst, const void* src, size_t bytes, uint64_t* total) {
  size_t alloc = bytes ? bytes : 16;
  HIP_TRY(hipMalloc(dst, alloc));
  if (bytes) HIP_TRY(hipMemcpy(*dst, src, bytes, hipMemcpyHostToDevice));
  *total += alloc;
  return RTG_OK;
}

static int prune_table(rtg_scene* s, LeanImages* im, int chains) {
  if (im->d_prune_off[chains] || !im->n_pruned) return RTG_OK;
  const size_t n = im->plan_mask.size();
  std::vector<uint8_t> drop(n);
  std::vector<uint32_t> off(n);
  for (size_t i = 0; i < n; i++) drop[i] = im->plan_mask[i] == BOX_PRUNED || (chains && im->plan_mask[i] == BOX_FOLLOWER);
  im->prune_bytes[chains] = lds_image_offsets(im->plan_ops.data(), n, off.data(), drop.data());
  int rc = upload(&s->buffers[im->slot + 1 + chains], off.data(), n * sizeof(uint32_t), &s->bytes);
  if (rc) return rc;
  im->d_prune_off[chains] = (const uint32_t*)s->buffers[im->slot + 1 + chains];
  return RTG_OK;
}

static int lean_images(rtg_scene* s, LeanImages* im, const std::vector<Packet>& lo, const std::vector<Packet>& hi, int off_slot) {
  std::vector<uint32_t> off(hi.size());
  im->plan_ops.resize(hi.size());
  for (size_t i = 0; i < hi.size(); i++) im->plan_ops[i] = hi[i].w[3];
  im->bytes = lds_image_offsets(im->plan_ops.data(), hi.size(), off.data());
  int rc = upload(&s->buffers[off_slot], off.data(), off.size() * sizeof(uint32_t), &s->bytes);
  if (rc) return rc;
  im->d_off = (const uint32_t*)s->buffers[off_slot];
  im->follower.resize(hi.size());
  im->n_followers = box_chain_followers(reinterpret_cast<const uint32_t (*)[4]>(lo.data()), reinterpret_cast<const uint32_t (*)[4]>(hi.data()), hi.size(), im->follower.data());
  if (im->n_followers) {
    im->chain_bytes = lds_image_offsets(im->plan_ops.data(), hi.size(), off.data(), im->follower.data());
    if ((rc = upload(&s->buffers[im->slot], off.data(), off.size() * sizeof(uint32_t), &s->bytes))) return rc;
    im->d_chain_off = (const uint32_t*)s->buffers[im->slot];
  }
  return RTG_OK;
}

static int lean_plan(rtg_scene* s, LeanImages* im, const std::vector<Packet>& lo, const std::vector<Packet>& hi, BoxPlanKind kind) {
  if (im->planned || !s->plannable) return RTG_OK;
  im->planned = true;
  im->plan_mask.resize(hi.size());
  const auto t0 = std::chrono::steady_clock::now();
  im->n_pruned = box_plan(reinterpret_cast<const uint32_t (*)[4]>(lo.data()), reinterpret_cast<const uint32_t (*)[4]>(hi.data()), hi.size(), im->follower.data(), im->plan_mask.data(), nullptr, BOX_PLAN_PROBES, kind).n_pruned;
  im->plan_ms = std::chrono::duration<float, std::milli>(std::chrono::steady_clock::now() - t0).count();
  return prune_table(s, im, 1);
}
static int ref_plan(rtg_scene* s) { return lean_plan(s, &s->ref, s->h_lo, s->h_hi, BOX_PLAN_DEFAULT); }

static int tree_program(rtg_scene* s) {
  if (s->tree_tried || !s->plannable) return RTG_OK;
  s->tree_tried = true;
  const size_t n = s->h_hi.size();
  std::vector<Packet> lo(n), hi(n);
  std::vector<uint32_t> origin(n);
  const auto t0 = std::chrono::steady_clock::now();
  s->n_regions = box_tree_rebuild(reinterpret_cast<const uint32_t (*)[4]>(s->h_lo.data()), reinterpret_cast<const uint32_t (*)[4]>(s->h_hi.data()), n,
                                  reinterpret_cast<uint32_t (*)[4]>(lo.data()), reinterpret_cast<uint32_t (*)[4]>(hi.data()), origin.data());
  s->tree_ms = std::chrono::duration<float, std::milli>(std::chrono::steady_clock::now() - t0).count();
  if (!s->n_regions) return RTG_OK;
  int rc;
  if ((rc = upload(&s->buffers[15], lo.data(), n * 16, &s->bytes)) || (rc = upload(&s->buffers[16], hi.data(), n * 16, &s->bytes))) return rc;
  s->tree.slot = 18;
  if ((rc = lean_images(s, &s->tree, lo, hi, 17)) || (rc = lean_plan(s, &s->tree, lo, hi, BOX_TREE_PLAN))) return rc;
  if (!s->box_chains && (rc = prune_table(s, &s->tree, 0))) return rc;
  s->tree.lo = (const uint4*)s->buffers[15], s->tree.hi = (const uint4*)s->buffers[16];
  return RTG_OK;
}

void rtg_scene_destroy(rtg_scene* s) {
  if (!s) return;
  (void)hipSetDevice(s->device);
  for (void* p : s->buffers)
    if (p) (void)hipFree(p);
  for (LaunchCtx& c : s->ctx) {
    ctx_free_buffers(&c);
    if (c.d_counters) (void)hipFree(c.d_counters);
    if (c.d_consts) (void)hipFree(c.d_consts);
    if (c.ev0) (void)hipEventDestroy(c.ev0);
    if (c.ev1) (void)hipEventDestroy(c.ev1);
    if (c.done) (void)hipEventDestroy(c.done);
  }
  if (s->d_frame) (void)hipFree(s->d_frame);
  if (s->d_lights) (void)hipFree(s->d_lights);
  if (s->d_sampled) (void)hipFree(s->d_sampled);
  if (s->d_pack) (void)hipFree(s->d_pack);
  if (s->d_recv) (void)hipFree(s->d_recv);
  if (s->post0) (void)hipEventDestroy(s->post0);
  if (s->post1) (void)hipEventDestroy(s->post1);
  for (hipEvent_t ev : {s->pack0, s->pack1, s->unpack0})
    if (ev) (void)hipEventDestroy(ev);
  if (s->own_stream) (void)hipStreamDestroy(s->own_stream);
  delete s;
}

int rtg_scene_create(rtg_builder* b, const rtg_id* world, size_t n, int device, rtg_scene** out) {
  if (!b || !out || (!world && n)) return fail(RTG_ERR_INVALID, "null argument");
  FlatScene fs;
  try {
    b->sb.flatten(world, n, &fs);
  } catch (const BuildError& e) {
    return fail(e.code, e.msg);
  }
  int ndev = 0;
  if (hipGetDeviceCount(&ndev) != hipSuccess || ndev == 0)
    return fail(RTG_ERR_DEVICE, "no HIP device: the rtiow hot path has no CPU fallback");
  if (device < 0 || device >= ndev) return fail(RTG_ERR_INVALID, "bad device index");
  HIP_TRY(hipSetDevice(device));
  rtg_scene* s = new rtg_scene();
  s->device = device;
  s->features = fs.features;
  s->n_prog = (uint32_t)fs.lo.size();
  s->n_mat = (uint32_t)fs.mat.size() / 2;
  s->n_tex = (uint32_t)fs.tex.size() / 2;
  int rc;
  if ((rc = upload(&s->buffers[0], fs.lo.data(), fs.lo.size() * 16, &s->bytes)) ||
      (rc = upload(&s->buffers[1], fs.hi.data(), fs.hi.size() * 16, &s->bytes)) ||
      (rc = upload(&s->buffers[2], fs.mat.data(), fs.mat.size() * 16, &s->bytes)) ||
      (rc = upload(&s->buffers[3], fs.tex.data(), fs.tex.size() * 16, &s->bytes)) ||
      (rc = upload(&s->buffers[4], fs.perlin_vecs.data(), sizeof(float) * 1024, &s->bytes)) ||
      (rc = upload(&s->buffers[5], fs.perlin_perm.data(), 768, &s->bytes))) {
    rtg_scene_destroy(s);
    return rc;
  }
  s->dev.lo = (const uint4*)s->buffers[0];
  s->dev.hi = (const uint4*)s->buffers[1];
  s->dev.mat = (const uint4*)s->buffers[2];
  s->dev.tex = (const uint4*)s->buffers[3];
  s->dev.perlin_vecs = (const float4*)s->buffers[4];
  s->dev.perlin_perm = (const uint8_t*)s->buffers[5];
  s->dev.n_prog = s->n_prog;
  s->dev.n_mat = s->n_mat;
  for (const Packet& h : fs.hi) s->n_box += (h.w[3] & 0xffu) == OP_BOX ? 1u : 0u;
  {
    std::vector<uint32_t> parent(fs.hi.size(), 0xffffffffu), open;
    for (size_t i = 0; i < fs.hi.size(); i++) {
      const uint32_t op = fs.hi[i].w[3] & 0xffu;
      if (op == OP_POP && !open.empty()) open.pop_back();
      parent[i] = open.empty() ? 0xffffffffu : open.back();
      if (op == OP_PUSH) open.push_back((uint32_t)i);
    }
    if ((rc = upload(&s->buffers[8], parent.data(), parent.size() * sizeof(uint32_t), &s->bytes))) {
      rtg_scene_destroy(s);
      return rc;
    }
    s->d_parent = (const uint32_t*)s->buffers[8];
  }
  for (size_t i = 0; i < fs.hi.size(); i++)
    if ((fs.hi[i].w[3] & 0xffu) == OP_SEG) s->seg_first = (uint32_t)i + 1u, s->seg_end = fs.hi[i].w[2];
  if (!fs.hi2.empty()) {
    if ((rc = upload(&s->buffers[9], fs.lo2.data(), fs.lo2.size() * 16, &s->bytes)) ||
        (rc = upload(&s->buffers[10], fs.hi2.data(), fs.hi2.size() * 16, &s->bytes)) ||
        (rc = upload(&s->buffers[11], &fs.p2, sizeof(P2Table), &s->bytes))) {
      rtg_scene_destroy(s);
      return rc;
    }
    s->dev2 = s->dev;
    s->dev2.lo = (const uint4*)s->buffers[9], s->dev2.hi = (const uint4*)s->buffers[10];
    s->dev2.n_prog = s->n_prog2 = (uint32_t)fs.hi2.size();
    s->dev2.lds_off = nullptr, s->dev2.lds_image_bytes = 0;
    s->d_p2 = (const P2Table*)s->buffers[11];
    for (const Packet& h : fs.hi2) s->n_box2 += (h.w[3] & 0xffu) == OP_BOX ? 1u : 0u;
  }
  if ((fs.features & (FEAT_ALL | FEAT_BOUNDARY)) == 0) {
    s->ref.lo = s->dev.lo, s->ref.hi = s->dev.hi, s->ref.slot = 12;
    if ((rc = lean_images(s, &s->ref, fs.lo, fs.hi, 6))) {
      rtg_scene_destroy(s);
      return rc;
    }
    s->dev.lds_off = s->ref.d_off, s->dev.lds_image_bytes = s->ref.bytes;
    s->plannable = s->dev.lds_image_bytes - LDS_BOX_BYTES * (s->n_box / 2u) <= 160u * 1024u;
    if (s->plannable) {
      s->h_lo = fs.lo, s->h_hi = fs.hi;
      if ((s->box_tree && (rc = tree_program(s))) || (!s->tree.lo && (rc = ref_plan(s)))) {
        rtg_scene_destroy(s);
        return rc;
      }
    }
    std::vector<uint32_t> wide;
    if (build_wide_image(fs.lo.data(), fs.hi.data(), fs.hi.size(), wide)) {
      if ((rc = upload(&s->buffers[7], wide.data(), wide.size() * sizeof(uint32_t), &s->bytes))) {
        rtg_scene_destroy(s);
        return rc;
      }
      s->wide_bytes = (uint32_t)(wide.size() * sizeof(uint32_t));
    }
  }
  b->sb.light_table(world, n, &s->h_lights, &s->h_sampled);
  s->n_lights = (uint32_t)s->h_lights.size();
  hipDeviceProp_t prop;
  if (hipGetDeviceProperties(&prop, device) == hipSuccess) s->num_cus = prop.multiProcessorCount;
  if (s->num_cus <= 0) s->num_cus = 256;
  if ((rc = ctx_acquire(s))) {
    rtg_scene_destroy(s);
    return rc;
  }
  s->next_ctx = 0;
  *out = s;
  return RTG_OK;
}


int rtg_scene_set_option(rtg_scene* s, const char* name, int value) {
  if (!s || !name) return fail(RTG_ERR_INVALID, "null argument");
  const std::string k(name);
  const uint32_t u = (uint32_t)value;
  if (k == "kernel") s->kernel_version = value;
  else if (k == "chunks") s->force_chunks = value;
  else if (k == "scratch_mb") s->scratch_limit = value > 0 ? (uint64_t)value << 20 : 0;
  else if (k == "lpt") s->lpt = value;
  else if (k == "lpt_phase1") s->lpt_phase1 = value;
  else if (k == "lpt_deep") s->lpt_deep = value;
  else if (k == "lpt_shift") s->lpt_shift = std::min(6, std::max(0, value));
  else if (k == "ray_lds") s->ray_lds = value;
  else if (k == "box_chains") {
    if (!value) {
      HIP_TRY(hipSetDevice(s->device));
      int rc = prune_table(s, &s->ref, 0);
      if (!rc) rc = prune_table(s, &s->tree, 0);
      if (rc) return rc;
    }
    s->box_chains = value;
  }
  else if (k == "box_tree") {
    if (value < 0 || value > 1) return fail(RTG_ERR_INVALID, "box_tree: 0 or 1");
    HIP_TRY(hipSetDevice(s->device));
    int rc = value ? tree_program(s) : ref_plan(s);
    if (!rc && !s->box_chains) rc = prune_table(s, value ? &s->tree : &s->ref, 0);
    if (rc) return rc;
    s->box_tree = value;
  }
  else if (k == "box_prune") {
    if (value < 0 || value > 2) return fail(RTG_ERR_INVALID, "box_prune: 0 .. 2");
    s->box_prune = value;
  }
  else if (k == "bvh4") {
    if (value && !s->wide_bytes) return fail(RTG_ERR_INVALID, "bvh4: the scene is not one Bvh of spheres (no 4-wide image)");
    if (value && pool_lds_bytes(s->wide_bytes, s->n_mat, (uint32_t)(s->pool_threads > 0 ? s->pool_threads : RT_POOL_MAX_THREADS) / 64u, true, false) > 160 * 1024)
      return fail(RTG_ERR_INVALID, "bvh4: the 4-wide image does not fit a CU's 160 KB of LDS (the 4-wide walk only exists LDS-staged)");
    s->bvh4 = value;
  }
  else if (k == "frames_in_flight") {
    if (value < 1 || value > RTG_MAX_FRAMES) return fail(RTG_ERR_INVALID, "frames_in_flight: 1 .. 4");
    HIP_TRY(hipSetDevice(s->device));
    for (int i = value; i < RTG_MAX_FRAMES; i++) ctx_free_buffers(&s->ctx[i]);
    s->n_ctx = value, s->next_ctx = 0;
  }
  else if (k == "force_rccl") s->force_rccl = value;
  else if (k == "multi_gather") s->multi_gather = value;
  else if (k == "multi_planes") s->multi_planes = value;
  else if (k == "sync") s->sync_full = value;
  else if (k == "block") {
    if (value < 64 || value > 1024 || value % 64) return fail(RTG_ERR_INVALID, "block: a multiple of 64 in [64, 1024]");
    s->pool_threads = s->full_threads = value;
  }
  else if (k == "wg_per_cu") s->wg_per_cu = value;
  else if (k == "drain_share") s->drain_share = value;
  else if (k == "hoist") s->hoist = value;
  else if (k == "pool2") s->pool2 = value;
  else if (k == "deep_sized") s->deep_sized = value;
  else if (k == "mat_lds") s->mat_lds = value;
  else if (k == "guide_lds") s->guide_lds = value;
  else if (k == "light_sampling") {
    if (value < 0 || value > 1) return fail(RTG_ERR_INVALID, "light_sampling: 0 or 1");
    if (value && s->n_lights > RT_MAX_LIGHTS) return fail(RTG_ERR_INVALID, "light_sampling: the scene's light table has " + std::to_string(s->n_lights) + " rects, more than RT_MAX_LIGHTS (64)");
    if (value && s->n_lights != 0u && !s->d_lights) {
      HIP_TRY(hipSetDevice(s->device));
      int rc = upload(&s->d_lights, s->h_lights.data(), s->h_lights.size() * sizeof(LightRect), &s->bytes);
      if (!rc) rc = upload(&s->d_sampled, s->h_sampled.data(), s->h_sampled.size(), &s->bytes);
      if (rc) return rc;
      s->lights = LightTable{(const LightRect*)s->d_lights, (const uint8_t*)s->d_sampled, s->n_lights};
    }
    if (s->verbose) {
      fprintf(stderr, "[rtg] light sampling %s: light table of %u rect(s)\n", value ? "on" : "off", s->n_lights);
      for (const LightRect& l : s->h_lights)
        fprintf(stderr, "[rtg]   light: axis %u k %.9g r0 %.9g %.9g r1 %.9g %.9g area %.9g material %u\n", l.axis, l.k, l.r0s, l.r0e, l.r1s, l.r1e, l.area, l.mat);
      std::string ids;
      for (size_t m = 0; m < s->h_sampled.size(); m++)
        if (s->h_sampled[m]) ids += " " + std::to_string(m);
      fprintf(stderr, "[rtg]   sampled materials:%s\n", ids.c_str());
    }
    s->light_sampling = value;
  }
  else if (k == "small_frames") s->small_frames = value;
  else if (k == "verbose") s->verbose = value;
  else if (k == "window") s->window = value;
  else if (k == "box_leave") s->pool_tune.box_leave = s->full_tune.box_leave = s->sync_tune.box_leave = u;
  else if (k == "refill_min") s->pool_tune.refill_min = s->full_tune.refill_min = s->sync_tune.refill_min = u;
  else if (k == "gather_min") s->pool_tune.gather_min = s->full_tune.gather_min = s->sync_tune.gather_min = u;
  else if (k == "run_ahead") s->pool_tune.run_ahead = s->full_tune.run_ahead = s->sync_tune.run_ahead = u;
  else if (k == "run_ahead_min") s->pool_tune.run_ahead_min = s->full_tune.run_ahead_min = s->sync_tune.run_ahead_min = u;
  else if (k == "sphere_min") s->pool_tune.sphere_min = s->full_tune.sphere_min = s->sync_tune.sphere_min = std::max(1u, u);
  else if (k == "p2_refill") s->pool2_tune.refill_min = u;
  else if (k == "p2_box_leave") s->pool2_tune.box_leave = u;
  else if (k == "p2_park") s->pool2_tune.park_max = u;
  else if (k == "p2_sphere") s->pool2_tune.t_sphere = std::max(1u, u);
  else if (k == "p2_prism") s->pool2_tune.t_prism = std::max(1u, u);
  else if (k == "p2_list") s->pool2_tune.t_list = std::max(1u, u);
  else if (k == "p2_push") s->pool2_tune.t_push = std::max(1u, u);
  else return fail(RTG_ERR_INVALID, "rtg_scene_set_option: unknown option '" + k + "'");
  return RTG_OK;
}

int rtg_scene_info(const rtg_scene* s, uint32_t* n_instructions, uint32_t* n_materials, uint32_t* n_textures,
                   uint64_t* hbm_bytes, uint32_t* n_box_followers) {
  if (!s) return fail(RTG_ERR_INVALID, "null argument");
  if (n_instructions) *n_instructions = s->n_prog;
  if (n_materials) *n_materials = s->n_mat;
  if (n_textures) *n_textures = s->n_tex;
  if (hbm_bytes) *hbm_bytes = s->bytes;
  if (n_box_followers) *n_box_followers = s->ref.n_followers;
  return RTG_OK;
}

static DevCamera to_dev(const rtg_camera* c) {
  DevCamera d;
  auto v = [](const float* p) { return V3{p[0], p[1], p[2]}; };
  d.origin = v(c->origin), d.llc = v(c->lower_left_corner), d.horizontal = v(c->horizontal);
  d.vertical = v(c->vertical), d.u = v(c->u), d.v = v(c->v);
  d.lens_radius = c->lens_radius, d.e0 = c->exposure_start, d.e1 = c->exposure_end;
  return d;
}

static int check_params(const rtg_scene* s, const rtg_camera* camera, const rtg_params* p, DevParams* out) {
  if (!s || !camera || !p) return fail(RTG_ERR_INVALID, "null argument");
  if (p->struct_size != sizeof(rtg_params)) return fail(RTG_ERR_INVALID, "rtg_params.struct_size mismatch");
  if (p->nx == 0 || p->ny == 0 || p->ns == 0) return fail(RTG_ERR_INVALID, "nx, ny, ns must be > 0");
  if ((uint64_t)p->nx * p->ny > 0xffffffffull) return fail(RTG_ERR_INVALID, "image too large for 32-bit pixel index");
  if (!(camera->exposure_start < camera->exposure_end))
    return fail(RTG_ERR_RANGE, "Uniform::sample_single called with low >= high");
  if (!std::isfinite(camera->exposure_start) || !std::isfinite(camera->exposure_end))
    return fail(RTG_ERR_RANGE, "Uniform::sample_single called with non-finite boundaries");
  if (!std::isfinite(camera->exposure_end - camera->exposure_start))
    return fail(RTG_ERR_RANGE, "exposure range wider than f32::MAX is not supported");
  DevParams d;
  d.nx = p->nx, d.ny = p->ny, d.ns = p->ns, d.max_bounces = p->max_bounces;
  d.t_near = p->t_near;
  d.seed_lo = (uint32_t)p->seed, d.seed_hi = (uint32_t)(p->seed >> 32);
  d.tile_w = p->tile_w ? p->tile_w : 16u;
  d.tile_h = p->tile_h ? p->tile_h : 16u;
  if (d.tile_w % 8u || d.tile_h % 8u) return fail(RTG_ERR_INVALID, "tile_w / tile_h must be multiples of 8");
  d.nranks = p->nranks ? p->nranks : 1u;
  d.rank = p->rank;
  d.bg = Background{BG_NONE, {0.f, 0.f, 0.f}, {0.f, 0.f, 0.f}};
  if (d.rank >= d.nranks) return fail(RTG_ERR_INVALID, "rank >= nranks");
  if ((p->flags & RTG_FLAG_RESUME) && p->sample_begin > p->ns) return fail(RTG_ERR_INVALID, "RTG_FLAG_RESUME: sample_begin > ns");
  if ((p->flags & RTG_FLAG_RETIRE) && (~p->flags & (RTG_FLAG_SAMPLE_COUNTS | RTG_FLAG_SUM_SQUARES)))
    return fail(RTG_ERR_INVALID, "RTG_FLAG_RETIRE needs RTG_FLAG_SAMPLE_COUNTS | RTG_FLAG_SUM_SQUARES");
  if ((p->flags & RTG_FLAG_DENOISE) && !(p->flags & RTG_FLAG_SUM_SQUARES)) return fail(RTG_ERR_INVALID, "RTG_FLAG_DENOISE needs RTG_FLAG_SUM_SQUARES");
  if ((p->flags & RTG_FLAG_DENOISE_ERROR) && !(p->flags & RTG_FLAG_DENOISE)) return fail(RTG_ERR_INVALID, "RTG_FLAG_DENOISE_ERROR needs RTG_FLAG_DENOISE");
  if ((p->flags & RTG_FLAG_DENOISE) && d.nranks > 1u) return fail(RTG_ERR_INVALID, "RTG_FLAG_DENOISE needs nranks = 1 (the neighbours live on other ranks)");
  *out = d;
  return RTG_OK;
}

static int print_schedule_stats(rtg_scene* s, float ms) {
  if (s->cx->lpt_desc.n_blocks && s->cx->d_lpt) {
    std::vector<uint32_t> ctl(LPT_CTL);
    HIP_TRY(hipMemcpy(ctl.data(), s->cx->lpt_desc.ctl, LPT_CTL * sizeof(uint32_t), hipMemcpyDeviceToHost));
    std::string line;
    for (uint32_t c = 0; c < LPT_CLASSES; c++)
      if (ctl[c]) line += " " + std::to_string(c) + ":" + std::to_string(ctl[c]);
    fprintf(stderr, "[rtg] cost-ordered queue: %u of %u blocks filed, class:blocks%s\n", ctl[LPT_CLASSES], s->cx->lpt_desc.n_blocks, line.c_str());
  }
  unsigned long long q[24];
  HIP_TRY(hipMemcpy(q, s->cx->d_counters + 8, sizeof(q), hipMemcpyDeviceToHost));
  if (q[18]) {
    const double us = (double)ms * 1000. / (double)q[16], n = (double)q[18];
    fprintf(stderr, "[rtg] wave timeline (us from its start): sees the work queue empty at min %.0f / mean %.0f / max %.0f; done at mean %.0f / max %.0f\n",
            (double)((1ull << 62) - q[19]) * us, (double)q[20] / n * us, (double)q[21] * us, (double)q[17] / n * us, (double)q[16] * us);
  }
  double tt = (double)(q[8] + q[9] + q[10] + q[11]);
  fprintf(stderr, "[rtg] wave-time shares (s_memtime, instrumented variant): shade %.1f%% gen+pull|service %.1f%% box %.1f%% sphere %.1f%%; "
          "per pass: shade %.0f, gen|service %.0f, box %.0f, sphere %.0f ticks\n", 100 * q[8] / tt, 100 * q[9] / tt, 100 * q[10] / tt,
          100 * q[11] / tt, q[4] ? (double)q[8] / q[4] : 0., q[4] ? (double)q[9] / q[4] : 0., q[0] ? (double)q[10] / q[0] : 0.,
          q[2] ? (double)q[11] / q[2] : 0.);
  if (q[15]) {
    unsigned long long f[2];
    HIP_TRY(hipMemcpy(f, s->cx->d_counters + 5, sizeof(f), hipMemcpyDeviceToHost));
    fprintf(stderr, "[rtg] services %llu: finish step %.1f%% of wave time (%.0f ticks each), refill step %.1f%% (%.0f ticks per refill)\n", f[0],
            100 * f[1] / tt, f[0] ? (double)f[1] / f[0] : 0., 100 * q[15] / tt, q[6] ? (double)q[15] / q[6] : 0.);
  }
#ifdef RT_CENSUS
  {
    unsigned long long c[32];
    HIP_TRY(hipMemcpy(c, s->cx->d_counters + 32, sizeof(c), hipMemcpyDeviceToHost));
    static const char* nm[13] = {"BOX", "END", "no-ray", "held", "?", "?", "SPHERE", "RECT", "PUSH", "POP", "MEDIUM", "PRISM", "BEND"};
    for (int k = 0; k < 2; k++) {
      std::string line;
      char buf[64];
      for (int j = 0; j < 13; j++)
        if (c[16 * k + j]) snprintf(buf, sizeof buf, " %s %.1f", nm[j], (double)c[16 * k + j] / (double)c[16 * k + 15]), line += buf;
      fprintf(stderr, "[rtg] lane census at %s (%llu):%s\n", k ? "slow-pass iterations" : "box steps", c[16 * k + 15], line.c_str());
    }
  }
#endif
  fprintf(stderr, "[rtg] pool schedule: box steps %llu (avg %.1f lanes), sphere passes %llu (avg %.1f lanes), shade passes %llu "
            "(avg %.1f lanes), end / camera-ray passes %llu (avg %.1f lanes), refills %llu (avg %.1f lanes)\n", q[0], q[0] ? (double)q[1] / q[0] : 0.0, q[2],
            q[2] ? (double)q[3] / q[2] : 0.0, q[4], q[4] ? (double)q[5] / q[4] : 0.0, q[12], q[12] ? (double)q[13] / q[12] : 0.0, q[6],
            q[6] && q[7] ? (double)q[7] / q[6] : 0.0);
  return RTG_OK;
}

int rtg_par_cast_device(rtg_scene* s, const rtg_camera* camera, const rtg_params* params, float* d_out,
                        void* hip_stream, rtg_stats* stats) {
  DevParams d;
  int rc = check_params(s, camera, params, &d);
  if (rc) return rc;
  if (!d_out) return fail(RTG_ERR_INVALID, "null output");
  if (stats && stats->struct_size != sizeof(rtg_stats)) return fail(RTG_ERR_INVALID, "rtg_stats.struct_size mismatch");
  HIP_TRY(hipSetDevice(s->device));
  hipStream_t stream = (hipStream_t)hip_stream;
  if ((rc = ctx_acquire(s))) return rc;
  DevCamera cam = to_dev(camera);
  bool count = stats && (params->flags & RTG_FLAG_COUNTERS);
  const SampleSlice sl = slice_of(params);
  const FrameLayout L(d.nx, d.ny, params->flags);
  FrameBlocks fb;
#define HIP_TRY_CTX(expr)                               \
  do {                                                  \
    hipError_t e_ = (expr);                             \
    if (e_ != hipSuccess) {                             \
      (void)hipStreamSynchronize(stream);               \
      return hip_fail(e_, #expr);                       \
    }                                                   \
  } while (0)
  if ((sl.denoise || sl.features || sl.background) && !sl.counts) {
    HIP_TRY(read_blocks(L, sl, d_out, stream, &fb));
    HIP_TRY(hipStreamSynchronize(stream));
    if (const char* why = blocks_refusal(sl, fb, d.nranks)) return fail(RTG_ERR_INVALID, why);
    if (sl.background) d.bg = dev_background(fb.background);
  }
  if (count) {
    HIP_TRY_CTX(hipMemsetAsync(s->cx->d_counters, 0, 7 * sizeof(unsigned long long), stream));
    HIP_TRY_CTX(hipMemsetAsync(s->cx->d_counters + 8, 0, 24 * sizeof(unsigned long long), stream));
    HIP_TRY_CTX(hipMemsetAsync(s->cx->d_counters + 32, 0, 32 * sizeof(unsigned long long), stream));
  }
#ifdef RT_TIMELINE
  static uint32_t* d_tl = nullptr;
  const size_t tl_bytes = (size_t)1024 * 16 * 16 * sizeof(uint32_t);
  if (!count) {
    if (!d_tl) HIP_TRY_CTX(hipMalloc((void**)&d_tl, tl_bytes));
    HIP_TRY_CTX(hipMemsetAsync(d_tl, 0, tl_bytes, stream));
    static unsigned long long tl_ptr;
    tl_ptr = (unsigned long long)(uintptr_t)d_tl;
    HIP_TRY_CTX(hipMemcpyAsync(s->cx->d_counters + 31, &tl_ptr, sizeof(tl_ptr), hipMemcpyHostToDevice, stream));
  }
#endif
  if (stats) HIP_TRY_CTX(hipEventRecord(s->cx->ev0, stream));
  s->cx->refusal = nullptr;
  HIP_TRY_CTX(count ? launch_render<true>(s, cam, d, d_out, stream, sl, L, fb) : launch_render<false>(s, cam, d, d_out, stream, sl, L, fb));
  if ((rc = ctx_release(s, stream))) {
    (void)hipStreamSynchronize(stream);
    return rc;
  }
#undef HIP_TRY_CTX
  if (s->cx->refusal) return fail(RTG_ERR_INVALID, s->cx->refusal);
  if (stats) {
    HIP_TRY(hipEventRecord(s->cx->ev1, stream));
    HIP_TRY(hipEventSynchronize(s->cx->ev1));
    float ms = 0.f;
    HIP_TRY(hipEventElapsedTime(&ms, s->cx->ev0, s->cx->ev1));
#ifdef RT_TIMELINE
    if (!count && getenv("RTG_TIMELINE_OUT")) {
      std::vector<uint32_t> h_tl(tl_bytes / sizeof(uint32_t));
      HIP_TRY(hipMemcpy(h_tl.data(), d_tl, tl_bytes, hipMemcpyDeviceToHost));
      if (FILE* f = fopen(getenv("RTG_TIMELINE_OUT"), "wb")) {
        fwrite(&ms, sizeof(ms), 1, f);
        fwrite(h_tl.data(), 1, tl_bytes, f);
        fclose(f);
      }
    }
#endif
    stats->kernel_ms = ms;
    stats->samples = sl.counts ? s->cx->counts_samples : owned_pixels(d) * (d.ns - sl.begin);
    unsigned long long h[8] = {0, 0, 0, 0, 0, 0, 0, 0};
    if (count) HIP_TRY(hipMemcpy(h, s->cx->d_counters, sizeof(h), hipMemcpyDeviceToHost));
    stats->aabb_tests = h[0], stats->prim_tests = h[1], stats->shaded_hits = h[2], stats->rays = h[3], stats->draws = h[4];
    if (count && s->verbose && (rc = print_schedule_stats(s, ms))) return rc;
  }
  return RTG_OK;
}

static int check_blocks(const FrameLayout& L, const SampleSlice& sl, const float* out_rgb, uint32_t nranks, FrameBlocks* fb) {
  if (sl.retire) memcpy(&fb->retire, out_rgb + L.retire, sizeof(rtg_retire));
  if (sl.denoise) memcpy(&fb->denoise, out_rgb + L.denoise, sizeof(rtg_denoise));
  if (sl.features) memcpy(&fb->features, out_rgb + L.features, sizeof(rtg_features));
  if (sl.background) memcpy(&fb->background, out_rgb + L.background, sizeof(rtg_background));
  if (const char* why = blocks_refusal(sl, *fb, nranks)) return fail(RTG_ERR_INVALID, why);
  return RTG_OK;
}

int rtg_par_cast(rtg_scene* s, const rtg_camera* camera, const rtg_params* params, float* out_rgb, rtg_stats* stats) {
  if (!s || !params || !out_rgb) return fail(RTG_ERR_INVALID, "null argument");
  {
    DevParams d;
    const int rc0 = check_params(s, camera, params, &d);
    if (rc0) return rc0;
  }
  const SampleSlice sl = slice_of(params);
  const FrameLayout L(params->nx, params->ny, params->flags);
  FrameBlocks fb;
  if (int rc0 = check_blocks(L, sl, out_rgb, params->nranks ? params->nranks : 1u, &fb)) return rc0;
  HIP_TRY(hipSetDevice(s->device));
  hipError_t e = grow((void**)&s->d_frame, &s->frame_bytes, L.words ? L.words * sizeof(float) : 16);
  if (e != hipSuccess) return hip_fail(e, "hipMalloc(framebuffer)");
  float* d_out = s->d_frame;
  char* dev = reinterpret_cast<char*>(d_out);
  char* host = reinterpret_cast<char*>(out_rgb);
  const Extents up = upload_extents(L, params->nranks > 1, sl.begin, fb.features.compute);
  for (int i = 0; i < up.n && e == hipSuccess; i++) e = hipMemcpy(dev + up.e[i].lo, host + up.e[i].lo, up.e[i].hi - up.e[i].lo, hipMemcpyHostToDevice);
  int rc = (e == hipSuccess) ? rtg_par_cast_device(s, camera, params, d_out, nullptr, stats) : hip_fail(e, "hipMemcpy");
  if (rc == RTG_OK) {
    e = hipDeviceSynchronize();
    const Extents back = copy_back_extents(L, fb.features.compute);
    for (int i = 0; i < back.n && e == hipSuccess; i++) e = hipMemcpy(host + back.e[i].lo, dev + back.e[i].lo, back.e[i].hi - back.e[i].lo, hipMemcpyDeviceToHost);
    if (e != hipSuccess) rc = hip_fail(e, "render / copy back");
  }
  return rc;
}

#include "rtg_multi.inc"

#include "rtg_probes.inc"

}
```

rtiow-rust_amd/csrc/rtg_launch.inc:

```
static uint64_t scratch_cap(int n_ctx) {
  size_t free_b = 0, total_b = 0;
  if (hipMemGetInfo(&free_b, &total_b) != hipSuccess) return (16ull << 30) / (uint64_t)std::max(1, n_ctx);
  return (uint64_t)free_b / 2 / (uint64_t)std::max(1, n_ctx);
}

static uint32_t samples_per_pass(const rtg_scene* s, uint64_t pix_work, uint32_t ns) {
  const uint64_t per_sample = pix_work * 3 * sizeof(float);
  uint64_t budget = s->scratch_limit ? s->scratch_limit : std::max<uint64_t>(scratch_cap(s->n_ctx), s->cx->scratch_bytes);
  if (s->whole_scratch) budget = ~0ull;
  uint64_t k = std::max<uint64_t>(1, budget / std::max<uint64_t>(per_sample, 1));
  k = std::min<uint64_t>(k, 0xfffffffeull / std::max<uint64_t>(pix_work, 1));
  k = std::max<uint64_t>(1, std::min<uint64_t>(k, ns));
  const uint64_t n_pass = (ns + k - 1) / k;
  return (uint32_t)((ns + n_pass - 1) / n_pass);
}

static uint64_t rank_pix_work(const DevParams& d) {
  const uint32_t tiles_x = (d.nx + d.tile_w - 1) / d.tile_w, tiles_y = (d.ny + d.tile_h - 1) / d.tile_h, tiles = tiles_x * tiles_y;
  const uint32_t owned = tiles > d.rank ? (tiles - d.rank + d.nranks - 1) / d.nranks : 0;
  return ((uint64_t)owned * d.tile_w * d.tile_h + 255u) & ~255ull;
}
static uint64_t owned_pixels(const DevParams& d) {
  uint64_t px = 0;
  uint32_t tiles_x = (d.nx + d.tile_w - 1) / d.tile_w, tiles_y = (d.ny + d.tile_h - 1) / d.tile_h;
  for (uint32_t ty = 0; ty < tiles_y; ty++)
    for (uint32_t tx = 0; tx < tiles_x; tx++) {
      if ((ty * tiles_x + tx) % d.nranks != d.rank) continue;
      uint32_t w = std::min(d.tile_w, d.nx - tx * d.tile_w), h = std::min(d.tile_h, d.ny - ty * d.tile_h);
      px += (uint64_t)w * h;
    }
  return px;
}

static hipError_t grow(void** buf, size_t* have, size_t need) {
  if (need <= *have) return hipSuccess;
  if (*buf) (void)hipFree(*buf);
  *buf = nullptr, *have = 0;
  hipError_t e = hipMalloc(buf, need);
  if (e == hipSuccess) *have = need;
  return e;
}

template <bool SIZED, typename F>
static void with_feat(const rtg_scene* s, F&& f) {
  constexpr uint32_t D = FEAT_ALL | FEAT_DEEP;
  if (s->features & FEAT_DEEP) {
    if constexpr (SIZED) {
      const bool few = s->deep_sized && (s->features & FEAT_DEEP_FEW_WRAPPERS) != 0, one = s->deep_sized && (s->features & FEAT_DEEP_ONE_LEVEL) != 0;
      if (few && one) return f(std::integral_constant<uint32_t, D | FEAT_DEEP_FEW_WRAPPERS | FEAT_DEEP_ONE_LEVEL>{});
      if (few) return f(std::integral_constant<uint32_t, D | FEAT_DEEP_FEW_WRAPPERS>{});
      if (one) return f(std::integral_constant<uint32_t, D | FEAT_DEEP_ONE_LEVEL>{});
    }
    return f(std::integral_constant<uint32_t, D>{});
  }
  if ((s->features & (FEAT_ALL | FEAT_BOUNDARY)) == 0) return f(std::integral_constant<uint32_t, 0u>{});
  return f(std::integral_constant<uint32_t, FEAT_ALL>{});
}
template <typename F>
static void with_bools(F&& f) {
  f();
}
template <typename F, typename... Rest>
static void with_bools(F&& f, bool b, Rest... rest) {
  if (b) with_bools([&](auto... c) { f(std::true_type{}, c...); }, rest...);
  else with_bools([&](auto... c) { f(std::false_type{}, c...); }, rest...);
}

static hipError_t setup_lpt(rtg_scene* s, ChunkMode& cm, uint64_t capacity);
static void launch_pass_setup(rtg_scene* s, const LaunchConsts& c, uint32_t* queue, hipStream_t stream);

static hipError_t kernel_setup(rtg_scene* s, const void* kernel, int bt, size_t lds, int* per_cu) {
  static std::mutex mu;
  static std::map<std::pair<int, const void*>, size_t> raised;
  static std::map<std::tuple<int, const void*, int, size_t>, int> occupancy;
  std::lock_guard<std::mutex> lock(mu);
  size_t& have = raised[std::make_pair(s->device, kernel)];
  if (have < lds) {
    static std::map<int, int> device_cap;
    int& cap = device_cap[s->device];
    if (cap == 0 && (hipDeviceGetAttribute(&cap, hipDeviceAttributeMaxSharedMemoryPerBlock, s->device) != hipSuccess || cap <= 0)) cap = 64 * 1024;
    const int want = std::min(160 * 1024, std::max(cap, (int)std::min<size_t>(lds, 160 * 1024)));
    hipError_t e = hipFuncSetAttribute(kernel, hipFuncAttributeMaxDynamicSharedMemorySize, want);
    if (e == hipSuccess) {
      have = (size_t)want;
    } else {
      (void)hipGetLastError();
      e = hipFuncSetAttribute(kernel, hipFuncAttributeMaxDynamicSharedMemorySize, (int)lds);
      if (e != hipSuccess) return e;
      have = lds;
    }
  }
  const auto key = std::make_tuple(s->device, kernel, bt, lds);
  auto it = occupancy.find(key);
  if (it == occupancy.end()) {
    int n = 0;
    hipError_t e = hipOccupancyMaxActiveBlocksPerMultiprocessor(&n, kernel, bt, lds);
    if (e != hipSuccess) return e;
    it = occupancy.emplace(key, n).first;
  }
  *per_cu = s->wg_per_cu > 0 ? s->wg_per_cu : std::max(1, it->second);
  return hipSuccess;
}

struct PoolGeometry { int bt; uint32_t grid, work_block; };
static PoolGeometry pool_geometry(const rtg_scene* s, uint64_t total_work, int bt_max, int forced_bt, uint32_t pool, bool shrink_mid) {
  PoolGeometry g;
  g.bt = forced_bt > 0 && forced_bt <= bt_max ? forced_bt : bt_max;
  g.work_block = WORK_BLOCK;
  const uint64_t lanes_worth = (total_work + 63) / 64;
  const uint64_t cus = (uint64_t)std::max(1, s->num_cus);
  if (s->small_frames && lanes_worth < cus * (uint64_t)(bt_max / 64)) {
    if (forced_bt <= 0) g.bt = 64 * (int)std::min<uint64_t>((uint64_t)(bt_max / 64), (lanes_worth + cus - 1) / cus);
    g.work_block = 64;
    g.grid = (uint32_t)std::max<uint64_t>(1, (lanes_worth + (uint64_t)(g.bt / 64) - 1) / (uint64_t)(g.bt / 64));
    return g;
  }
  const uint64_t waves = (uint64_t)(g.bt / 64);
  uint64_t want = (total_work + waves * pool - 1) / (waves * pool);
  g.grid = (uint32_t)std::min<uint64_t>(want ? want : 1, 0xffffffffull);
  if (s->small_frames && shrink_mid && total_work < std::min<uint64_t>(g.grid, cus) * waves * WORK_BLOCK * 4) g.work_block = 64;
  return g;
}

struct PoolLaunch {
  KernelKind kind;
  int bt, per_cu;
  size_t lds;
  PoolGeometry geo;
  uint32_t pool;
};

template <typename Chunks, typename Issue>
static hipError_t sample_passes(rtg_scene* s, const DevParams& d, float* d_out, hipStream_t stream, const SampleSlice& sl,
                                const PoolLaunch& L, uint32_t per_pass, Chunks chunks, Issue issue) {
  for (uint32_t s0 = sl.begin; s0 < d.ns; s0 += per_pass) {
    DevParams dp = d;
    dp.ns = std::min(d.ns, s0 + per_pass);
    ChunkMode cm = chunks(s0, dp.ns);
    cm.work_block = L.geo.work_block;
    const uint64_t total_work = (uint64_t)cm.pix_work * cm.n_chunks;
    if (total_work > 0xfffffffeull) return hipErrorInvalidValue;
    const uint32_t grid = (uint32_t)std::min<uint64_t>(L.geo.grid, (uint64_t)s->num_cus * L.per_cu);
    hipError_t e = setup_lpt(s, cm, (uint64_t)grid * (uint32_t)(L.bt / 64) * L.pool);
    if (e != hipSuccess) return e;
    if (cm.lpt) cm.work_block = WORK_BLOCK;
    e = issue(s0, dp, cm, grid, (uint32_t)total_work);
    if (e == hipSuccess) e = hipGetLastError();
    if (e != hipSuccess) return e;
    if (cm.scratch && sl.counts) {
      void (*fold)(DevParams, ChunkMode, PixMap, float*, ListConsts) = sl.squares ? fold_samples_list_kernel<true> : fold_samples_list_kernel<false>;
      hipLaunchKernelGGL(fold, dim3((uint32_t)(((uint64_t)cm.pix_work + 255) / 256)), dim3(256), 0, stream, dp, cm, make_pixmap(dp), d_out, sl.list);
      e = hipGetLastError();
      if (e != hipSuccess) return e;
    } else if (cm.scratch) {
      void (*fold)(DevParams, ChunkMode, PixMap, float*, uint32_t) = sl.squares ? fold_samples_sq_kernel : fold_samples_kernel;
      hipLaunchKernelGGL(fold, dim3((uint32_t)(((uint64_t)cm.pix_work + 255) / 256)), dim3(256), 0, stream, dp, cm, make_pixmap(dp), d_out,
                         sl.divide ? d.ns : 0u);
      e = hipGetLastError();
      if (e != hipSuccess) return e;
    }
  }
  return hipSuccess;
}

template <bool COUNT>
static hipError_t launch_pool(rtg_scene* s, const DevCamera& cam, const DevParams& d, float* d_out,
                              hipStream_t stream, const SampleSlice& sl) {
  const uint64_t pix_work = sl.counts ? sl.list_work : rank_pix_work(d);
  if (pix_work == 0) return hipSuccess;
  if (pix_work > 0xfffffffeull) return hipErrorInvalidValue;
  const uint32_t ns_call = d.ns - sl.begin;
  uint64_t n_chunks = ns_call;
  if (s->force_chunks > 0) n_chunks = (uint64_t)s->force_chunks;
  if (n_chunks > ns_call) n_chunks = ns_call;
  const bool use_scratch = n_chunks > 1 || sl.sliced() || sl.squares || sl.counts;
  uint32_t per_pass = d.ns, chunk = d.ns;
  if (use_scratch) {
    per_pass = samples_per_pass(s, pix_work, ns_call);
    chunk = (uint32_t)((ns_call + n_chunks - 1) / n_chunks);
    if (per_pass < ns_call || sl.begin % chunk != 0u || sl.squares || sl.counts) chunk = 1u;
    hipError_t ea = grow((void**)&s->cx->d_scratch, &s->cx->scratch_bytes, pix_work * per_pass * 3 * sizeof(float));
    if (ea != hipSuccess) return ea;
  }
  s->cx->last_pix_work = use_scratch && per_pass == d.ns ? (uint32_t)pix_work : 0u;
  uint32_t* queue = (uint32_t*)(s->cx->d_counters + 7);
  const uint64_t work0 = pix_work * (use_scratch ? (std::min(ns_call, per_pass) + chunk - 1) / chunk : 1u);
  const PoolGeometry geo = pool_geometry(s, work0, RT_POOL_MAX_THREADS, s->pool_threads, POOL, true);
  const int bt = geo.bt;
  const uint32_t waves = (uint32_t)bt / 64;
  const size_t lds_limit = 160 * 1024;
  const bool wide = s->bvh4 && s->wide_bytes != 0 && !sl.counts;
  const bool production = !COUNT || s->box_prune == 2;
  DevScene dev = s->dev;
  bool chains = false, prune = false;
  auto choose = [&](const LeanImages& im) {
    chains = !COUNT && !wide && s->box_chains && im.d_chain_off != nullptr;
    prune = !wide && s->box_prune && production && im.d_prune_off[s->box_chains ? 1 : 0] != nullptr;
    dev.lo = im.lo, dev.hi = im.hi, dev.lds_off = im.d_off, dev.lds_image_bytes = im.bytes;
    if (chains) dev.lds_off = im.d_chain_off, dev.lds_image_bytes = im.chain_bytes;
    if (prune) dev.lds_off = im.d_prune_off[s->box_chains ? 1 : 0], dev.lds_image_bytes = im.prune_bytes[s->box_chains ? 1 : 0];
  };
  bool tree = s->box_tree && s->tree.lo != nullptr && production && !wide && s->ref.lo != nullptr;
  if (tree) {
    choose(s->tree);
    if (pool_lds_bytes(dev.lds_image_bytes, s->n_mat, waves, true, false) > lds_limit) tree = false;
  }
  if (!tree && s->ref.lo != nullptr) choose(s->ref);
  const LeanImages& im = tree ? s->tree : s->ref;
  if (wide) dev.lds_off = (const uint32_t*)s->buffers[7], dev.lds_image_bytes = s->wide_bytes;
  const uint32_t image = dev.lds_image_bytes;
  bool use_lds = image != 0 && pool_lds_bytes(image, s->n_mat, waves, true, false) <= lds_limit;
  if (wide && !use_lds) return hipErrorNotSupported;
  bool ray_lds = s->ray_lds && pool_lds_bytes(image, s->n_mat, waves, use_lds, true) <= lds_limit && (!use_lds || image < (1u << 17));
  size_t lds = pool_lds_bytes(image, s->n_mat, waves, use_lds, ray_lds);
  if (s->verbose && s->ray_lds && !ray_lds && use_lds && image >= (1u << 17) && pool_lds_bytes(image, s->n_mat, waves, use_lds, true) <= lds_limit)
    fprintf(stderr, "[rtg] pool: the LDS image is %u B (>= 128 KB): the slots' hot fields stay in global memory although they would fit LDS (their 16-bit best_pc holds image offsets / 8 < 2^14)\n", image);
  void (*kernel)(DevScene, const LaunchConsts*, float*, uint32_t, uint32_t*, unsigned long long*, PoolTuning, uint32_t*);
  if (sl.counts) {
    if (ray_lds) kernel = use_lds ? render_lean_pool<true, COUNT, true, false, true> : render_lean_pool<false, COUNT, true, false, true>;
    else kernel = use_lds ? render_lean_pool<true, COUNT, false, false, true> : render_lean_pool<false, COUNT, false, false, true>;
  } else if (wide) kernel = ray_lds ? render_lean_pool<true, COUNT, true, true> : render_lean_pool<true, COUNT, false, true>;
  else if (ray_lds) kernel = use_lds ? render_lean_pool<true, COUNT, true> : render_lean_pool<false, COUNT, true>;
  else kernel = use_lds ? render_lean_pool<true, COUNT, false> : render_lean_pool<false, COUNT, false>;
  if (s->verbose && (chains || prune) && use_lds)
    fprintf(stderr, "[rtg] pool: %s program (%u region(s) rebuilt in %.2f ms), box chains: %u follower record(s)%s, box pruning: %u interior record(s)%s (plan %.2f ms): LDS image %u B, %u records of %u; without followers %u B, full image %u B\n",
            tree ? "rebuilt" : "reference", s->n_regions, s->tree_ms, im.n_followers, chains || (prune && s->box_chains) ? " dropped" : " kept", im.n_pruned, prune ? " dropped" : " kept", im.plan_ms, image,
            s->n_prog - (chains || (prune && s->box_chains) ? im.n_followers : 0u) - (prune ? im.n_pruned : 0u), s->n_prog, im.chain_bytes ? im.chain_bytes : im.bytes, im.bytes);
  PoolLaunch L{KernelKind::lean_pool, bt, 0, lds, geo, POOL};
  hipError_t e = kernel_setup(s, (const void*)kernel, bt, lds, &L.per_cu);
  if (e != hipSuccess) return e;
  auto chunks = [&](uint32_t s0, uint32_t end) {
    ChunkMode cm{};
    cm.scratch = nullptr, cm.chunk = d.ns, cm.n_chunks = 1, cm.pix_work = (uint32_t)pix_work, cm.s_begin = s0;
    if (use_scratch) {
      cm.chunk = chunk;
      cm.n_chunks = (end - s0 + chunk - 1) / chunk;
      cm.scratch = s->cx->d_scratch - 3ull * s0 * pix_work;
    }
    return cm;
  };
  auto issue = [&](uint32_t s0, const DevParams& dp, const ChunkMode& cm, uint32_t grid, uint32_t total_work) {
    if (s->verbose)
      fprintf(stderr, "[rtg] pool: samples [%u, %u) of %u: grid %u x %d threads, %d WG/CU, lds %zu B (program staged: %d, hot slot fields in LDS: %d), %u chunk(s) of %u samples, cost-ordered queue after %u chunk(s)\n",
              s0, dp.ns, d.ns, grid, bt, L.per_cu, lds, (int)use_lds, (int)ray_lds, cm.n_chunks, cm.chunk, (cm.lpt_samples - (cm.lpt_samples ? s0 : 0u)) / (cm.chunk ? cm.chunk : 1u));
    hipError_t eg = grow((void**)&s->cx->d_slots, &s->cx->slots_bytes, (size_t)grid * waves * POOL * POOL_FIELDS * sizeof(uint32_t));
    if (eg != hipSuccess) return eg;
    launch_pass_setup(s, LaunchConsts{cam, dp, cm, make_pixmap(dp)}, queue, stream);
    hipLaunchKernelGGL(kernel, dim3(grid), dim3(bt), lds, stream, dev, (const LaunchConsts*)s->cx->d_consts, d_out, total_work, queue,
                       s->cx->d_counters, s->pool_tune, s->cx->d_slots);
    return hipSuccess;
  };
  return sample_passes(s, d, d_out, stream, sl, L, per_pass, chunks, issue);
}

static bool build_wide_image(const Packet* lo, const Packet* hi, size_t n, std::vector<uint32_t>& out) {
  struct T { uint32_t box; int left, right; uint32_t sphere; };
  std::vector<T> nodes;
  auto op_of = [&](size_t i) { return hi[i].w[3] & 0xffu; };
  if (n < 4 || op_of(n - 1) != OP_END || op_of(0) != OP_BOX || hi[0].w[2] != n - 1) return false;
  bool ok = true;
  std::function<int(size_t, size_t&)> parse = [&](size_t i, size_t& end) -> int {
    if (i >= n || op_of(i) != OP_BOX) { ok = false; end = i + 1; return -1; }
    end = hi[i].w[2];
    const int id = (int)nodes.size();
    nodes.push_back(T{(uint32_t)i, -1, -1, 0});
    if (op_of(i + 1) == OP_SPHERE) {
      if (end != i + 2) ok = false;
      nodes[id].sphere = (uint32_t)(i + 1);
      return id;
    }
    size_t e1 = 0, e2 = 0;
    const int l = parse(i + 1, e1);
    if (!ok || e1 >= end) { ok = false; return id; }
    const int r = parse(e1, e2);
    if (e2 != end) ok = false;
    nodes[id].left = l, nodes[id].right = r;
    return id;
  };
  size_t end0 = 0;
  const int root = parse(0, end0);
  if (!ok || root < 0 || nodes[root].left < 0) return false;
  out.clear();
  auto alloc = [&](uint32_t bytes) { const uint32_t at = (uint32_t)out.size() * 4u; out.resize(out.size() + bytes / 4u, 0u); return at; };
  std::function<uint32_t(int, uint32_t, uint32_t)> emit = [&](int t, uint32_t parent, uint32_t level) -> uint32_t {
    if (level > 7u) { ok = false; return 0; }
    const uint32_t at = alloc(WIDE_NODE_BYTES);
    int entry[4];
    uint32_t n_ch = 0;
    for (int x : {nodes[t].left, nodes[t].right}) {
      if (nodes[x].left < 0) entry[n_ch++] = x;
      else entry[n_ch++] = nodes[x].left, entry[n_ch++] = nodes[x].right;
    }
    uint32_t child[4] = {0, 0, 0, 0}, leafmask = 0;
    for (uint32_t k = 0; k < n_ch; k++) {
      const T e = nodes[entry[k]];
      const Packet bl = lo[e.box], bh = hi[e.box];
      uint32_t* b = out.data() + at / 4u + 4u + 12u * k;
      b[0] = bl.w[0], b[1] = bl.w[1], b[2] = bl.w[2], b[3] = bl.w[3], b[4] = bh.w[0], b[5] = bh.w[1];
      b[6] = bl.w[1], b[7] = bl.w[0], b[8] = bl.w[3], b[9] = bl.w[2], b[10] = bh.w[1], b[11] = bh.w[0];
      if (e.left < 0) {
        const uint32_t sp = alloc(WIDE_SPHERE_BYTES);
        uint32_t* r = out.data() + sp / 4u;
        r[0] = hi[e.sphere].w[2], r[1] = hi[e.sphere].w[3];
        r[2] = lo[e.sphere].w[0], r[3] = lo[e.sphere].w[1], r[4] = lo[e.sphere].w[2], r[5] = lo[e.sphere].w[3];
        r[6] = at, r[7] = 0u;
        child[k] = sp, leafmask |= 1u << k;
      } else {
        child[k] = emit(entry[k], at, level + 1u);
      }
    }
    uint32_t* h = out.data() + at / 4u;
    h[0] = parent, h[1] = LDS_BOX_BIT | OP_BOX | (level << 8) | (n_ch << 12) | (leafmask << 16);
    h[2] = (child[0] >> 3) | ((child[1] >> 3) << 16), h[3] = (child[2] >> 3) | ((child[3] >> 3) << 16);
    return at;
  };
  emit(root, WIDE_NO_PARENT, 0u);
  return ok && out.size() * 4u < 512u * 1024u;
}

static hipError_t setup_lpt(rtg_scene* s, ChunkMode& cm, uint64_t capacity) {
  cm.lpt = nullptr, cm.lpt_samples = 0, cm.lpt_deep = 0;
  const uint32_t n_blocks = cm.pix_work / LPT_BLOCK;
  if (!s->lpt || !cm.scratch || cm.n_chunks < 6 || n_blocks < 64 || n_blocks > 65536 || cm.pix_work % LPT_BLOCK) return hipSuccess;
  uint32_t phase1 = std::max<uint32_t>(std::min(8u, std::max(2u, cm.n_chunks / 8u)), (uint32_t)((2 * capacity + cm.pix_work - 1) / cm.pix_work));
  if (s->lpt_phase1 > 0) phase1 = (uint32_t)s->lpt_phase1;
  if (phase1 < 1 || phase1 > cm.n_chunks / 3) return hipSuccess;
  const size_t words = 16 + (size_t)n_blocks * (1 + LPT_CLASSES) + LPT_CTL;
  hipError_t e = grow((void**)&s->cx->d_lpt, &s->cx->lpt_bytes, words * sizeof(uint32_t));
  if (e != hipSuccess) return e;
  LptQueue q;
  memset(&q, 0, sizeof(q));
  static_assert(sizeof(LptQueue) <= 64, "descriptor slot");
  q.cost = s->cx->d_lpt + 16, q.ctl = q.cost + n_blocks, q.list = q.ctl + LPT_CTL;
  q.n_blocks = n_blocks, q.phase1 = phase1;
  q.phase2_base = phase1 * cm.pix_work;
  q.span = LPT_BLOCK * (cm.n_chunks - phase1);
  q.mode = (uint32_t)s->lpt, q.shift = (uint32_t)s->lpt_shift;
  s->cx->lpt_desc = q;
  cm.lpt = reinterpret_cast<const LptQueue*>(s->cx->d_lpt);
  cm.lpt_samples = cm.s_begin + phase1 * cm.chunk;
  cm.lpt_deep = (uint32_t)s->lpt_deep;
  return hipSuccess;
}

static void launch_pass_setup(rtg_scene* s, const LaunchConsts& c, uint32_t* queue, hipStream_t stream) {
  const bool lpt = c.cm.lpt != nullptr;
  const LptQueue q = lpt ? s->cx->lpt_desc : LptQueue{};
  hipLaunchKernelGGL(write_pass_setup, dim3(1), dim3(256), 0, stream, s->cx->d_consts, c, (unsigned long long*)queue,
                     lpt ? reinterpret_cast<LptQueue*>(s->cx->d_lpt) : (LptQueue*)nullptr, q, lpt ? q.n_blocks + LPT_CTL : 0u);
}

template <bool COUNT>
static hipError_t launch_full_pool(rtg_scene* s, const DevCamera& cam, const DevParams& d, float* d_out,
                                   hipStream_t stream, const SampleSlice& sl) {
  const uint64_t pix_work = sl.counts ? sl.list_work : rank_pix_work(d);
  if (pix_work == 0) return hipSuccess;
  if (pix_work > 0xfffffffeull) return hipErrorInvalidValue;
  const uint32_t ns_call = d.ns - sl.begin;
  const uint32_t per_pass = samples_per_pass(s, pix_work, ns_call);
  const bool tex = (s->features & FEAT_TEXTURE) != 0;
  const int bt_max = tex ? RT_FULL_TEX_THREADS : 1024;
  const PoolGeometry geo = pool_geometry(s, pix_work * std::min(ns_call, per_pass), bt_max, s->full_threads, FPOOL, false);
  const int bt = geo.bt;
  const uint32_t waves = (uint32_t)bt / 64;
  hipError_t e = grow((void**)&s->cx->d_scratch, &s->cx->scratch_bytes, pix_work * per_pass * 3 * sizeof(float));
  if (e != hipSuccess) return e;
  s->cx->last_pix_work = per_pass == d.ns ? (uint32_t)pix_work : 0u;
  uint32_t* queue = (uint32_t*)(s->cx->d_counters + 7);
  const size_t list_bytes = full_pool_lds_bytes(0, waves);
  const size_t budget = 160 * 1024;
  uint32_t window = s->n_prog;
  int prog = 1;
  if ((size_t)window * 32 + list_bytes > budget) window = (uint32_t)((budget - list_bytes) / 32), prog = 2;
  if (s->window >= 0) {
    window = std::min<uint32_t>(s->n_prog, (uint32_t)s->window);
    prog = window == 0 ? 0 : (window == s->n_prog ? 1 : 2);
  }
  const size_t mat_bytes = (size_t)s->n_mat * 32;
  const bool mats_in_lds = s->mat_lds > 0 && prog == 1 && full_pool_lds_bytes(window, waves) + mat_bytes <= budget;
  const size_t lds = full_pool_lds_bytes(window, waves) + (mats_in_lds ? mat_bytes : 0);
  void (*kernel)(DevScene, const LaunchConsts*, float*, uint32_t, uint32_t*, unsigned long long*, PoolTuning, uint32_t*, float*,
                 uint32_t);
  const bool genb = (s->features & FEAT_BOUNDARY) != 0;
  void (*sync_kernel)(DevScene, const LaunchConsts*, float*, uint32_t, uint32_t*, unsigned long long*, PoolTuning, float*, uint32_t) = nullptr;
  void (*pool2_kernel)(DevScene, const LaunchConsts*, float*, uint32_t, uint32_t*, unsigned long long*, Pool2Tuning, uint32_t*, const P2Table*) = nullptr;
  with_bools([&](auto tex_c, auto genb_c, auto list_c) {
    constexpr bool T = decltype(tex_c)::value, G = decltype(genb_c)::value, LI = decltype(list_c)::value;
    kernel = prog == 0 ? render_full_pool<0, T, COUNT, G, LI> : (prog == 1 ? render_full_pool<1, T, COUNT, G, LI> : render_full_pool<2, T, COUNT, G, LI>);
    sync_kernel = render_full_sync<1, T, COUNT, G, LI>;
    pool2_kernel = render_full_pool2<T, COUNT, LI>;
  }, tex, genb, sl.counts);
  const bool tiny_bvh = s->n_box <= 32u;
  const bool tiny_frame = pix_work * std::min(ns_call, per_pass) <= (uint64_t)std::max(1, s->num_cus) * 64u;
  const bool lock_step = (s->sync_full > 0 || (s->sync_full < 0 && (s->n_box == 0 || tiny_bvh || tiny_frame))) && prog == 1;
  const bool p2_size_ok = s->pool2 > 1 || pix_work * (uint64_t)ns_call >= (32ull << 20);
  const bool mats3 = s->mat_lds > 0 && pool2_lds_bytes(s->n_prog2, s->n_mat, waves) <= budget;
  const size_t lds3 = pool2_lds_bytes(s->n_prog2, mats3 ? s->n_mat : 0u, waves);
  const bool pool2 = s->pool2 > 0 && p2_size_ok && s->n_prog2 != 0 && !lock_step && !genb && lds3 <= budget;
  PoolLaunch L{KernelKind::full_pool, bt, 0, lds, geo, FPOOL};
  LaunchConsts consts{};
  consts.parent = s->d_parent;
  e = kernel_setup(s, (const void*)kernel, bt, lds, &L.per_cu);
  if (e != hipSuccess) return e;
  if (lock_step) {
    L.kind = KernelKind::lock_step;
    L.lds = (size_t)window * 32;
    L.geo = pool_geometry(s, pix_work * std::min(ns_call, per_pass), bt_max, s->full_threads, 64u, false);
    if (L.geo.bt != bt) L.geo = geo;
    e = kernel_setup(s, (const void*)sync_kernel, bt, L.lds, &L.per_cu);
  } else if (pool2) {
    L.kind = KernelKind::pool2;
    L.lds = lds3;
    const uint32_t tab = s->n_prog2 * 32u + DC_WORDS * 4u;
    consts.mat_lds = mats3 ? tab + P2_TABLE_BYTES : 0u;
    consts.p2_lists = tab + P2_TABLE_BYTES + (mats3 ? s->n_mat * 32u : 0u);
    e = kernel_setup(s, (const void*)pool2_kernel, bt, L.lds, &L.per_cu);
  } else {
    if (mats_in_lds) consts.mat_lds = (uint32_t)full_pool_lds_bytes(window, waves);
    if (s->hoist > 0 && s->seg_end > s->seg_first) consts.seg_first = s->seg_first * RSZ, consts.seg_end = s->seg_end * RSZ;
  }
  if (e != hipSuccess) return e;
  s->cx->last_kernel = L.kind;
  auto chunks = [&](uint32_t s0, uint32_t end) {
    ChunkMode cm{};
    cm.scratch = s->cx->d_scratch - 3ull * s0 * pix_work, cm.chunk = 1u, cm.n_chunks = end - s0, cm.pix_work = (uint32_t)pix_work, cm.s_begin = s0;
    cm.drain_share = (uint32_t)std::max(0, s->drain_share);
    return cm;
  };
  auto issue = [&](uint32_t s0, const DevParams& dp, const ChunkMode& cm, uint32_t grid, uint32_t total_work) {
    hipError_t eg = grow((void**)&s->cx->d_slots, &s->cx->slots_bytes, (size_t)grid * std::max(full_pool_wg_words(waves), pool2_slot_words(waves)) * sizeof(uint32_t));
    if (eg != hipSuccess) return eg;
    eg = grow((void**)&s->cx->d_stack, &s->cx->stack_bytes, (size_t)grid * waves * (genb ? 2 : 1) * MAX_XFORM_DEPTH * 6 * 64 * sizeof(float));
    if (eg != hipSuccess) return eg;
    const bool p2 = L.kind == KernelKind::pool2;
    if (s->verbose)
      fprintf(stderr, "[rtg] full pool%s: samples [%u, %u) of %u: grid %u x %d threads, %d WG/CU, lds %zu B (program window: %u of %u records), cost-ordered queue after %u chunk(s)\n",
              p2 ? " 2 (second program)" : "", s0, dp.ns, d.ns, grid, bt, L.per_cu, p2 ? lds3 : lds, p2 ? s->n_prog2 : window, p2 ? s->n_prog2 : s->n_prog,
              cm.lpt_samples - (cm.lpt_samples ? s0 : 0u));
    LaunchConsts c = consts;
    c.cam = cam, c.P = dp, c.cm = cm, c.pm = make_pixmap(dp);
    launch_pass_setup(s, c, queue, stream);
    if (L.kind == KernelKind::lock_step)
      hipLaunchKernelGGL(sync_kernel, dim3(grid), dim3(bt), L.lds, stream, s->dev, (const LaunchConsts*)s->cx->d_consts, d_out, total_work, queue,
                         s->cx->d_counters, s->sync_tune, s->cx->d_stack, window);
    else if (p2)
      hipLaunchKernelGGL(pool2_kernel, dim3(grid), dim3(bt), L.lds, stream, s->dev2, (const LaunchConsts*)s->cx->d_consts, d_out, total_work, queue,
                         s->cx->d_counters, s->pool2_tune, s->cx->d_slots, s->d_p2);
    else
      hipLaunchKernelGGL(kernel, dim3(grid), dim3(bt), L.lds, stream, s->dev, (const LaunchConsts*)s->cx->d_consts, d_out, total_work, queue,
                         s->cx->d_counters, s->full_tune, s->cx->d_slots, s->cx->d_stack, window);
    return hipSuccess;
  };
  return sample_passes(s, d, d_out, stream, sl, L, per_pass, chunks, issue);
}

static hipError_t launch_resolve(const DevParams& d, float* d_out, hipStream_t stream) {
  const uint64_t pix_work = rank_pix_work(d);
  if (pix_work == 0) return hipSuccess;
  if (pix_work > 0xfffffffeull) return hipErrorInvalidValue;
  hipLaunchKernelGGL(resolve_sum_kernel, dim3((uint32_t)((pix_work + 255) / 256)), dim3(256), 0, stream, d, make_pixmap(d), (uint32_t)pix_work, d_out);
  return hipGetLastError();
}

static hipError_t launch_resolve_counts(const DevParams& d, float* d_out, hipStream_t stream, const FrameLayout& L) {
  const uint64_t pix_work = rank_pix_work(d);
  if (pix_work == 0) return hipSuccess;
  if (pix_work > 0xfffffffeull) return hipErrorInvalidValue;
  hipLaunchKernelGGL(resolve_counts_kernel, dim3((uint32_t)(pix_work / 256u)), dim3(256), 0, stream, d, make_pixmap(d), (uint32_t)pix_work, d_out,
                     L.at(reinterpret_cast<const uint32_t*>(d_out), L.counts));
  return hipGetLastError();
}

static hipError_t launch_retire(rtg_scene* s, const DevParams& d, float* d_out, hipStream_t stream, const FrameLayout& L, uint64_t pix_work,
                                const rtg_retire& r) {
  const uint32_t n_blk = (uint32_t)(pix_work / 256u);
  const float* errp = L.at(d_out, L.error);
  RetireBufs b;
  b.pitch = (d.nx + 31u) / 32u + 1u;
  hipError_t e = grow(&s->cx->d_retire, &s->cx->retire_bytes, (size_t)n_blk * 28u + (size_t)d.ny * b.pitch * 4u);
  if (e != hipSuccess) return e;
  b.blk_se2 = reinterpret_cast<double*>(s->cx->d_retire);
  b.blk_held = reinterpret_cast<unsigned long long*>(b.blk_se2 + n_blk);
  b.blk_u32 = reinterpret_cast<uint32_t*>(b.blk_held + n_blk);
  b.okbits = b.blk_u32 + 3ull * n_blk;
  b.planes = d_out;
  b.counts = reinterpret_cast<uint32_t*>(d_out) + L.counts;
  b.block = reinterpret_cast<uint32_t*>(d_out) + L.retire;
  b.errp = errp;
  const RetireArgs a{r.target_se, d.ns, r.min_samples, r.radius};
  if (n_blk != 0u) {
    const PixMap pm = make_pixmap(d);
    if (errp) hipLaunchKernelGGL(retire_mark_error_kernel, dim3(n_blk), dim3(256), 0, stream, d, pm, a, b, r.target_se * r.target_se);
    else hipLaunchKernelGGL(retire_mark_kernel, dim3(n_blk), dim3(256), 0, stream, d, pm, a, b);
    hipLaunchKernelGGL(retire_apply_kernel, dim3(n_blk), dim3(256), 0, stream, d, pm, a, b);
  }
  hipLaunchKernelGGL(retire_finish_kernel, dim3(1), dim3(256), 0, stream, n_blk, b);
  return hipGetLastError();
}

static hipError_t launch_denoise(rtg_scene* s, const DevParams& d, float* d_out, hipStream_t stream, const FrameLayout& L, const rtg_denoise& in,
                                 const rtg_features* guide = nullptr) {
  const uint64_t n_pix = L.n;
  const bool error = L.has(L.error);
  const uint32_t n_blk = (uint32_t)((n_pix + 255u) / 256u);
  const size_t frec_at = (size_t)n_pix * 32u + (((size_t)n_blk * 8u + 15u) & ~(size_t)15u);
  hipError_t e = grow(&s->cx->d_denoise, &s->cx->denoise_bytes, frec_at + (guide ? (size_t)n_pix * 32u : 0u));
  if (e != hipSuccess) return e;
  uint32_t* words = reinterpret_cast<uint32_t*>(d_out);
  DenoiseBufs b;
  b.planes = d_out;
  b.counts = L.at(words, L.counts);
  b.rec = reinterpret_cast<float4*>(s->cx->d_denoise);
  b.blk_u32 = reinterpret_cast<uint32_t*>(b.rec + 2ull * n_pix);
  b.block = words + L.denoise;
  b.outp = d_out + L.denoised;
  b.errp = L.at(d_out, L.error);
  const DenoiseArgs a{in.k, in.radius, in.patch, d.ns};
  const int guided = !guide ? 0 : (s->guide_lds > 0 ? 2 : 1);
  void (*filter)(uint32_t, uint32_t, DenoiseArgs, DenoiseBufs, DenoiseGuide) =
      error ? (guided == 0 ? denoise_filter_kernel<0, true> : (guided == 1 ? denoise_filter_kernel<1, true> : denoise_filter_kernel<2, true>))
               : (guided == 0 ? denoise_filter_kernel<0, false> : (guided == 1 ? denoise_filter_kernel<1, false> : denoise_filter_kernel<2, false>));
  const size_t lds = denoise_lds_bytes(in.radius, in.patch, guided == 2);
  int per_cu = 0;
  e = kernel_setup(s, (const void*)filter, (int)DN_THREADS, lds, &per_cu);
  if (e != hipSuccess) return e;
  const uint64_t tiles = (uint64_t)((d.nx + DN_TW - 1u) / DN_TW) * ((d.ny + DN_TH - 1u) / DN_TH);
  if (tiles > 0x7fffffffull) return hipErrorInvalidValue;
  DenoiseGuide gd{nullptr, 1.f, 1.f, 1.f};
  if (guide) {
    float4* frec = reinterpret_cast<float4*>(reinterpret_cast<char*>(s->cx->d_denoise) + frec_at);
    gd = DenoiseGuide{frec, guide->sigma_normal, guide->sigma_albedo, guide->sigma_depth};
    hipLaunchKernelGGL(denoise_guide_kernel, dim3(n_blk), dim3(256), 0, stream, (uint32_t)n_pix, (const float*)d_out + L.albedo, (const float*)d_out + L.normal,
                       (const float*)d_out + L.depth, frec);
  }
  hipLaunchKernelGGL(error ? denoise_prepare_kernel<true> : denoise_prepare_kernel<false>, dim3(n_blk), dim3(256), 0, stream, (uint32_t)n_pix, a, b);
  hipLaunchKernelGGL(filter, dim3((uint32_t)tiles), dim3(DN_THREADS), lds, stream, d.nx, d.ny, a, b, gd);
  hipLaunchKernelGGL(denoise_finish_kernel, dim3(1), dim3(256), 0, stream, n_blk, b);
  return hipGetLastError();
}

static hipError_t launch_features(rtg_scene* s, const DevCamera& cam, const DevParams& d, float* d_out, hipStream_t stream, const FrameLayout& L,
                                  const rtg_features& in) {
  const uint64_t blocks = (uint64_t)((d.nx + 15u) / 16u) * ((d.ny + 15u) / 16u);
  if (blocks > 0x7fffffffull) return hipErrorInvalidValue;
  const uint32_t n_blk = in.compute ? (uint32_t)blocks : 0u;
  hipError_t e = grow((void**)&s->cx->d_features, &s->cx->features_bytes, (size_t)std::max<uint64_t>(blocks, 1) * 8u);
  if (e != hipSuccess) return e;
  FeatureBufs b;
  b.block = reinterpret_cast<uint32_t*>(d_out) + L.features;
// ... 136 lines not shown
```

rtiow-rust_amd/csrc/rtg_probes.inc:

```
int rtg_debug_hit_top(rtg_scene* s, size_t n, const float* rays, uint64_t seed, float t_near, float* out,
                      uint32_t* out_material) {
  if (!s || !rays || !out || !out_material) return fail(RTG_ERR_INVALID, "null argument");
  HIP_TRY(hipSetDevice(s->device));
  DevBuf<float> d_rays, d_out;
  DevBuf<uint32_t> d_mat;
  HIP_TRY(d_rays.alloc(7 * n));
  HIP_TRY(d_out.alloc(8 * n));
  HIP_TRY(d_mat.alloc(n));
  HIP_TRY(hipMemcpy(d_rays.p, rays, 7 * n * sizeof(float), hipMemcpyHostToDevice));
  dim3 grid((uint32_t)((n + 63) / 64)), block(64);
  if (n)
    with_feat<false>(s, [&](auto feat) {
      hipLaunchKernelGGL((debug_hit_top_kernel<decltype(feat)::value>), grid, block, 0, 0, s->dev, (uint32_t)n, d_rays.p, (uint32_t)seed, (uint32_t)(seed >> 32),
                         t_near, d_out.p, d_mat.p);
    });
  HIP_TRY(hipGetLastError());
  HIP_TRY(hipDeviceSynchronize());
  HIP_TRY(hipMemcpy(out, d_out.p, 8 * n * sizeof(float), hipMemcpyDeviceToHost));
  HIP_TRY(hipMemcpy(out_material, d_mat.p, n * sizeof(uint32_t), hipMemcpyDeviceToHost));
  return RTG_OK;
}

int rtg_debug_samples(rtg_scene* s, const rtg_camera* camera, const rtg_params* params, size_t n, const uint32_t* xs,
                      const uint32_t* ys, const uint32_t* samples, float* out_rgb, uint32_t* out_info) {
  DevParams d;
  int rc = check_params(s, camera, params, &d);
  if (rc) return rc;
  if (!xs || !ys || !samples || !out_rgb || !out_info) return fail(RTG_ERR_INVALID, "null argument");
  if (params->flags & (RTG_FLAG_PARTIAL | RTG_FLAG_RESUME)) return fail(RTG_ERR_INVALID, "rtg_debug_samples renders whole frames: RTG_FLAG_PARTIAL / RTG_FLAG_RESUME are not accepted");
  if (params->flags & RTG_FLAG_SUM_SQUARES) return fail(RTG_ERR_INVALID, "rtg_debug_samples: RTG_FLAG_SUM_SQUARES is not accepted");
  if (params->flags & RTG_FLAG_SAMPLE_COUNTS) return fail(RTG_ERR_INVALID, "rtg_debug_samples: RTG_FLAG_SAMPLE_COUNTS is not accepted");
  if (params->flags & RTG_FLAG_RETIRE) return fail(RTG_ERR_INVALID, "rtg_debug_samples: RTG_FLAG_RETIRE is not accepted");
  if (params->flags & RTG_FLAG_DENOISE) return fail(RTG_ERR_INVALID, "rtg_debug_samples: RTG_FLAG_DENOISE is not accepted");
  if (params->flags & RTG_FLAG_FEATURES) return fail(RTG_ERR_INVALID, "rtg_debug_samples: RTG_FLAG_FEATURES is not accepted");
  if (params->flags & RTG_FLAG_DENOISE_ERROR) return fail(RTG_ERR_INVALID, "rtg_debug_samples: RTG_FLAG_DENOISE_ERROR is not accepted");
  if (params->flags & RTG_FLAG_BACKGROUND) return fail(RTG_ERR_INVALID, "rtg_debug_samples: RTG_FLAG_BACKGROUND is not accepted");
  HIP_TRY(hipSetDevice(s->device));
  if (params->flags & RTG_FLAG_TRACE_KERNEL) {
    const uint32_t tiles_x = (d.nx + d.tile_w - 1) / d.tile_w;
    const uint64_t pix_work = rank_pix_work(d);
    const size_t trace_waves = (size_t)s->num_cus * std::max(32, s->wg_per_cu > 0 ? s->wg_per_cu * 16 : 0);
    const size_t table = (size_t)4 * d.ns * pix_work, slots = trace_waves * std::max(std::max(FPOOL, POOL), P2POOL) * 3;
    DevBuf<uint32_t> d_trace;
    HIP_TRY(d_trace.alloc(table + slots));
    HIP_TRY(hipMemset(d_trace.p, 0, (table + slots) * sizeof(uint32_t)));
    if ((rc = ctx_acquire(s))) return rc;
    HIP_TRY(grow((void**)&s->d_frame, &s->frame_bytes, (size_t)d.nx * d.ny * 3 * sizeof(float)));
    HIP_TRY(hipMemset(s->cx->d_counters, 0, 32 * sizeof(unsigned long long)));
    const unsigned long long ptrs[2] = {(unsigned long long)(uintptr_t)d_trace.p, (unsigned long long)(uintptr_t)(d_trace.p + table)};
    HIP_TRY(hipMemcpy(s->cx->d_counters + 30, ptrs, sizeof(ptrs), hipMemcpyHostToDevice));
    const DevCamera cam = to_dev(camera);
    s->whole_scratch = true;
    hipError_t e = launch_render<true>(s, cam, d, s->d_frame, nullptr, SampleSlice{}, FrameLayout(d.nx, d.ny, 0u), FrameBlocks{});
    s->whole_scratch = false;
    if (e == hipSuccess) e = hipDeviceSynchronize();
    (void)hipMemset(s->cx->d_counters + 30, 0, 2 * sizeof(unsigned long long));
    if (e != hipSuccess) return hip_fail(e, "trace launch");
    if (s->cx->last_kernel == KernelKind::baseline || s->cx->last_pix_work == 0)
      return fail(RTG_ERR_UNSUPPORTED, "this scene / frame runs on the baseline kernel (or without the per-sample scratch): nothing to trace");
    std::vector<uint32_t> h_trace(table);
    std::vector<float> h_col((size_t)3 * d.ns * pix_work);
    HIP_TRY(hipMemcpy(h_trace.data(), d_trace.p, table * sizeof(uint32_t), hipMemcpyDeviceToHost));
    HIP_TRY(hipMemcpy(h_col.data(), s->cx->d_scratch, h_col.size() * sizeof(float), hipMemcpyDeviceToHost));
    for (size_t i = 0; i < n; i++) {
      const uint32_t x = xs[i], row = d.ny - 1u - ys[i], sm = samples[i];
      const uint32_t tx = x / d.tile_w, ty = row / d.tile_h, tile = ty * tiles_x + tx;
      if (x >= d.nx || ys[i] >= d.ny || sm >= d.ns || tile % d.nranks != d.rank) return fail(RTG_ERR_INVALID, "trace key outside this rank's frame");
      const uint32_t k = tile / d.nranks, lx = x - tx * d.tile_w, ly = row - ty * d.tile_h;
      const uint32_t b = (ly >> 3) * (d.tile_w >> 3) + (lx >> 3);
      const size_t w = (size_t)k * d.tile_w * d.tile_h + b * 64u + (ly & 7u) * 8u + (lx & 7u);
      const size_t at = (size_t)sm * pix_work + w;
      for (int c = 0; c < 3; c++) out_rgb[3 * i + c] = h_col[3 * at + c];
      for (int c = 0; c < 4; c++) out_info[4 * i + c] = h_trace[4 * at + c];
    }
    return RTG_OK;
  }
  DevBuf<uint32_t> dx, dy, ds, dinfo;
  DevBuf<float> drgb;
  HIP_TRY(dx.alloc(n));
  HIP_TRY(dy.alloc(n));
  HIP_TRY(ds.alloc(n));
  HIP_TRY(dinfo.alloc(4 * n));
  HIP_TRY(drgb.alloc(3 * n));
  HIP_TRY(hipMemcpy(dx.p, xs, n * 4, hipMemcpyHostToDevice));
  HIP_TRY(hipMemcpy(dy.p, ys, n * 4, hipMemcpyHostToDevice));
  HIP_TRY(hipMemcpy(ds.p, samples, n * 4, hipMemcpyHostToDevice));
  DevCamera cam = to_dev(camera);
  dim3 grid((uint32_t)((n + 63) / 64)), block(64);
  if (n && s->light_sampling && s->lights.n != 0u)
    with_feat<false>(s, [&](auto feat) {
      constexpr uint32_t F = decltype(feat)::value;
      if constexpr (F != 0u)
        hipLaunchKernelGGL((debug_samples_light_kernel<F>), grid, block, 0, 0, s->dev, s->lights, cam, d, (uint32_t)n, dx.p, dy.p, ds.p, drgb.p, dinfo.p);
    });
  else if (n)
    with_feat<false>(s, [&](auto feat) {
      hipLaunchKernelGGL((debug_samples_kernel<decltype(feat)::value>), grid, block, 0, 0, s->dev, cam, d, (uint32_t)n, dx.p, dy.p, ds.p, drgb.p, dinfo.p);
    });
  HIP_TRY(hipGetLastError());
  HIP_TRY(hipDeviceSynchronize());
  HIP_TRY(hipMemcpy(out_rgb, drgb.p, 3 * n * sizeof(float), hipMemcpyDeviceToHost));
  HIP_TRY(hipMemcpy(out_info, dinfo.p, 4 * n * sizeof(uint32_t), hipMemcpyDeviceToHost));
  return RTG_OK;
}

int rtg_tonemap_device(int device, size_t n, const float* d_rgb, uint8_t* d_out, void* hip_stream) {
  if (!d_rgb || !d_out) return fail(RTG_ERR_INVALID, "null argument");
  HIP_TRY(hipSetDevice(device));
  if (n) hipLaunchKernelGGL(tonemap_kernel, dim3((uint32_t)((n + 255) / 256)), dim3(256), 0, (hipStream_t)hip_stream, n, d_rgb, d_out);
  HIP_TRY(hipGetLastError());
  return RTG_OK;
}

int rtg_tonemap(int device, size_t n, const float* rgb, uint8_t* out) {
  if (!rgb || !out) return fail(RTG_ERR_INVALID, "null argument");
  int ndev = 0;
  if (hipGetDeviceCount(&ndev) != hipSuccess || device < 0 || device >= ndev) return fail(RTG_ERR_DEVICE, "no HIP device");
  HIP_TRY(hipSetDevice(device));
  DevBuf<float> di;
  DevBuf<uint8_t> dout;
  HIP_TRY(di.alloc(n));
  HIP_TRY(dout.alloc(n));
  HIP_TRY(hipMemcpy(di.p, rgb, n * sizeof(float), hipMemcpyHostToDevice));
  int rc = rtg_tonemap_device(device, n, di.p, dout.p, nullptr);
  if (rc) return rc;
  HIP_TRY(hipDeviceSynchronize());
  HIP_TRY(hipMemcpy(out, dout.p, n, hipMemcpyDeviceToHost));
  return RTG_OK;
}

int rtg_debug_flatten(rtg_builder* b, const rtg_id* world, size_t n, uint32_t* n_instructions, uint32_t* features,
                      uint32_t* words_out, size_t capacity) {
  if (!b || (!world && n)) return fail(RTG_ERR_INVALID, "null argument");
  FlatScene fs;
  try {
    b->sb.flatten(world, n, &fs);
  } catch (const BuildError& e) {
    return fail(e.code, e.msg);
  }
  if (n_instructions) *n_instructions = (uint32_t)fs.lo.size();
  if (features) *features = fs.features;
  if (words_out) {
    size_t m = fs.lo.size() < capacity ? fs.lo.size() : capacity;
    for (size_t i = 0; i < m; i++) {
      std::memcpy(words_out + 8 * i, fs.lo[i].w, 16);
      std::memcpy(words_out + 8 * i + 4, fs.hi[i].w, 16);
    }
  }
  return RTG_OK;
}

int rtg_debug_flatten_pool2(rtg_builder* b, const rtg_id* world, size_t n, uint32_t* n_instructions, uint32_t* table_out,
                            uint32_t* words_out, size_t capacity) {
  if (!b || (!world && n)) return fail(RTG_ERR_INVALID, "null argument");
  FlatScene fs;
  try {
    b->sb.flatten(world, n, &fs);
  } catch (const BuildError& e) {
    return fail(e.code, e.msg);
  }
  if (n_instructions) *n_instructions = (uint32_t)fs.lo2.size();
  static_assert(sizeof(P2Table) == 24 * sizeof(uint32_t), "rtg_debug_flatten_pool2: table_out holds 24 words");
  if (table_out) std::memcpy(table_out, &fs.p2, sizeof(P2Table));
  if (words_out) {
    size_t m = fs.lo2.size() < capacity ? fs.lo2.size() : capacity;
    for (size_t i = 0; i < m; i++) {
      std::memcpy(words_out + 8 * i, fs.lo2[i].w, 16);
      std::memcpy(words_out + 8 * i + 4, fs.hi2[i].w, 16);
    }
  }
  return RTG_OK;
}

static int debug_lean_program(const char* who, rtg_builder* b, const rtg_id* world, size_t n, const uint32_t* words, size_t n_records,
                              std::vector<Packet>* lo, std::vector<Packet>* hi, bool* lean) {
  *lean = true;
  if (words) {
    lo->resize(n_records), hi->resize(n_records);
    for (size_t i = 0; i < n_records; i++) {
      std::memcpy((*lo)[i].w, words + 8 * i, 16), std::memcpy((*hi)[i].w, words + 8 * i + 4, 16);
      const uint32_t op = (*hi)[i].w[3] & 0xffu;
      *lean = *lean && (op == OP_BOX || op == OP_SPHERE || op == OP_END) && !((*hi)[i].w[3] & F_MOVE);
      if (op == OP_BOX && (*hi)[i].w[2] >= n_records) return fail(RTG_ERR_INVALID, std::string(who) + ": a skip pointer leaves the program");
    }
  } else {
    if (!b || (!world && n)) return fail(RTG_ERR_INVALID, "null argument");
    FlatScene fs;
    try {
      b->sb.flatten(world, n, &fs);
    } catch (const BuildError& e) {
      return fail(e.code, e.msg);
    }
    *lean = (fs.features & (FEAT_ALL | FEAT_BOUNDARY)) == 0;
    lo->swap(fs.lo), hi->swap(fs.hi);
  }
  if (hi->size() > 0x7fffffffu) return fail(RTG_ERR_INVALID, std::string(who) + ": program too large");
  return RTG_OK;
}

int rtg_debug_box_plan(rtg_builder* b, const rtg_id* world, size_t n, const uint32_t* words, size_t n_records, uint8_t* mask_out,
                       size_t capacity) {
  std::vector<Packet> lo, hi;
  bool lean = true;
  int rc = debug_lean_program("rtg_debug_box_plan", b, world, n, words, n_records, &lo, &hi, &lean);
  if (rc) return rc;
  std::vector<uint8_t> follower(hi.size(), 0), mask(hi.size(), 0);
  if (lean && !hi.empty()) {
    box_chain_followers(reinterpret_cast<const uint32_t (*)[4]>(lo.data()), reinterpret_cast<const uint32_t (*)[4]>(hi.data()), hi.size(), follower.data());
    box_plan(reinterpret_cast<const uint32_t (*)[4]>(lo.data()), reinterpret_cast<const uint32_t (*)[4]>(hi.data()), hi.size(), follower.data(), mask.data());
  }
  if (mask_out) std::memcpy(mask_out, mask.data(), std::min(mask.size(), capacity));
  return (int)hi.size();
}

int rtg_debug_production_program(rtg_builder* b, const rtg_id* world, size_t n, const uint32_t* words, size_t n_records,
                                 uint32_t* words_out, uint32_t* origin_out, uint8_t* mask_out, size_t capacity) {
  std::vector<Packet> lo, hi;
  bool lean = true;
  int rc = debug_lean_program("rtg_debug_production_program", b, world, n, words, n_records, &lo, &hi, &lean);
  if (rc) return rc;
  const size_t m = hi.size();
  std::vector<Packet> plo(lo), phi(hi);
  std::vector<uint32_t> origin(m);
  std::vector<uint8_t> follower(m, 0), mask(m, 0);
  for (size_t i = 0; i < m; i++) origin[i] = (uint32_t)i;
  if (lean && m) {
    box_tree_rebuild(reinterpret_cast<const uint32_t (*)[4]>(lo.data()), reinterpret_cast<const uint32_t (*)[4]>(hi.data()), m,
                     reinterpret_cast<uint32_t (*)[4]>(plo.data()), reinterpret_cast<uint32_t (*)[4]>(phi.data()), origin.data());
    box_chain_followers(reinterpret_cast<const uint32_t (*)[4]>(plo.data()), reinterpret_cast<const uint32_t (*)[4]>(phi.data()), m, follower.data());
    box_plan(reinterpret_cast<const uint32_t (*)[4]>(plo.data()), reinterpret_cast<const uint32_t (*)[4]>(phi.data()), m, follower.data(), mask.data(), nullptr, BOX_PLAN_PROBES, BOX_TREE_PLAN);
  }
  const size_t k = std::min(m, capacity);
  for (size_t i = 0; words_out && i < k; i++) std::memcpy(words_out + 8 * i, plo[i].w, 16), std::memcpy(words_out + 8 * i + 4, phi[i].w, 16);
  if (origin_out) std::memcpy(origin_out, origin.data(), k * sizeof(uint32_t));
  if (mask_out) std::memcpy(mask_out, mask.data(), k);
  return (int)m;
}

int rtg_debug_math(int device, int op, size_t n, const float* in, const float* in2, float* out) {
  if (!in || !out || op < 0 || op > 5 || (op == 5 && !in2)) return fail(RTG_ERR_INVALID, "bad argument");
  int ndev = 0;
  if (hipGetDeviceCount(&ndev) != hipSuccess || device < 0 || device >= ndev) return fail(RTG_ERR_DEVICE, "no HIP device");
  HIP_TRY(hipSetDevice(device));
  DevBuf<float> di, di2, dout;
  HIP_TRY(di.alloc(n));
  HIP_TRY(di2.alloc(n));
  HIP_TRY(dout.alloc(n));
  HIP_TRY(hipMemcpy(di.p, in, n * sizeof(float), hipMemcpyHostToDevice));
  if (in2) HIP_TRY(hipMemcpy(di2.p, in2, n * sizeof(float), hipMemcpyHostToDevice));
  if (n) hipLaunchKernelGGL(debug_math_kernel, dim3((uint32_t)((n + 255) / 256)), dim3(256), 0, 0, op, n, di.p, di2.p, dout.p);
  HIP_TRY(hipGetLastError());
  HIP_TRY(hipDeviceSynchronize());
  HIP_TRY(hipMemcpy(out, dout.p, n * sizeof(float), hipMemcpyDeviceToHost));
  return RTG_OK;
}
```

Before: 8047.

## Plan box pruning from camera-specific GPU probe path counts

Adds a GPU probe kernel that traces a small grid of camera paths through the program and counts how often each box record is entered. Those counts feed a new count-based box plan that decides which interior box records to prune, and the resulting LDS image is cached per camera key. The aim is a smaller, camera-tuned LDS program image so the render kernel does less box traversal or can stage more of the program in LDS. It costs an extra probe kernel, an asynchronous readback and host-side planning on first use of each camera, and it risks choosing a plan from a sample that does not represent the full render.

```diff
diff --git a/include/rtiow_gpu_debug.h b/include/rtiow_gpu_debug.h
--- a/include/rtiow_gpu_debug.h
+++ b/include/rtiow_gpu_debug.h
@@ -11,6 +11,9 @@
 int rtg_debug_production_program(rtg_builder* b, const rtg_id* world, size_t n, const uint32_t* words, size_t n_records,
                                  uint32_t* words_out, uint32_t* origin_out, uint8_t* mask_out, size_t capacity);
 
+int rtg_debug_camera_plan(rtg_builder* b, const rtg_id* world, size_t n, const uint32_t* words, size_t n_records,
+                          const uint32_t* counts, uint64_t n_rays, uint8_t* mask_out, size_t capacity);
+
 #ifdef __cplusplus
 }
 #endif
diff --git a/rtiow-rust_amd/capi.py b/rtiow-rust_amd/capi.py
--- a/rtiow-rust_amd/capi.py
+++ b/rtiow-rust_amd/capi.py
@@ -614,6 +614,7 @@
         f("tonemap_device", C.c_int, [C.c_int, C.c_size_t, C.c_void_p, C.c_void_p, C.c_void_p])
         f("debug_box_plan", C.c_int, [C.c_void_p, c_u32p, C.c_size_t, c_u32p, C.c_size_t, c_u8p, C.c_size_t])
         f("debug_production_program", C.c_int, [C.c_void_p, c_u32p, C.c_size_t, c_u32p, C.c_size_t, c_u32p, c_u32p, c_u8p, C.c_size_t])
+        f("debug_camera_plan", C.c_int, [C.c_void_p, c_u32p, C.c_size_t, c_u32p, C.c_size_t, c_u32p, C.c_uint64, c_u8p, C.c_size_t])
 
     def _fn(self, name, restype, argtypes):
         try:
@@ -853,6 +854,18 @@
             self.be.check(n)
         return out, origin, mask
 
+    def camera_plan(self, words, counts, n_rays):
+        words = np.ascontiguousarray(words, dtype=np.uint32)
+        counts = np.ascontiguousarray(counts, dtype=np.uint32)
+        if len(counts) != len(words):
+            raise ValueError("camera_plan: one count per record")
+        mask = np.zeros(len(words), dtype=np.uint8)
+        n = self.be._debug_camera_plan(None, None, 0, words.ctypes.data_as(c_u32p), len(words), counts.ctypes.data_as(c_u32p), int(n_rays),
+                                       mask.ctypes.data_as(c_u8p), len(mask))
+        if n < 0:
+            self.be.check(n)
+        return mask
+
     def bvh_sah(self, objs, exposure=(0.0, 1.0)):
         arr = (C.c_uint32 * max(1, len(objs)))(*objs)
         return self.be.check_id(self.be._object_bvh_sah(self.h, arr, len(objs), exposure[0], exposure[1]))
@@ -884,7 +897,7 @@
             pass
 
     ENV_OPTIONS = ("kernel", "chunks", "lpt", "lpt_phase1", "lpt_deep", "lpt_shift", "ray_lds", "sync", "block", "wg_per_cu", "window",
-                   "box_leave", "refill_min", "gather_min", "run_ahead", "run_ahead_min", "sphere_min", "verbose", "bvh4", "box_chains", "box_prune", "box_tree", "force_rccl", "multi_gather", "multi_planes", "scratch_mb", "frames_in_flight", "small_frames", "drain_share", "hoist", "deep_sized", "mat_lds", "pool2", "p2_refill", "p2_box_leave", "p2_park", "p2_sphere", "p2_prism", "p2_list", "p2_push", "light_sampling")
+                   "box_leave", "refill_min", "gather_min", "run_ahead", "run_ahead_min", "sphere_min", "verbose", "bvh4", "box_chains", "box_prune", "box_tree", "box_camera", "force_rccl", "multi_gather", "multi_planes", "scratch_mb", "frames_in_flight", "small_frames", "drain_share", "hoist", "deep_sized", "mat_lds", "pool2", "p2_refill", "p2_box_leave", "p2_park", "p2_sphere", "p2_prism", "p2_list", "p2_push", "light_sampling")
 
     def set_option(self, name, value):
         self.be.check(self.be._scene_set_option(self.h, name.encode(), int(value)))
diff --git a/rtiow-rust_amd/csrc/rt_box_plan.h b/rtiow-rust_amd/csrc/rt_box_plan.h
--- a/rtiow-rust_amd/csrc/rt_box_plan.h
+++ b/rtiow-rust_amd/csrc/rt_box_plan.h
@@ -18,7 +18,7 @@
 #endif
 constexpr uint32_t BOX_PLAN_PROBES = RT_BOX_PLAN_PROBES;
 constexpr bool BOX_PLAN_FULL = RT_BOX_PLAN_FULL != 0;
-enum BoxPlanKind : int { BOX_PLAN_SURE = 0, BOX_PLAN_PROBE_DP = 1, BOX_PLAN_AREA = 2 };
+enum BoxPlanKind : int { BOX_PLAN_SURE = 0, BOX_PLAN_PROBE_DP = 1, BOX_PLAN_AREA = 2, BOX_PLAN_COUNTS = 3 };
 constexpr BoxPlanKind BOX_PLAN_DEFAULT = BOX_PLAN_FULL ? BOX_PLAN_PROBE_DP : BOX_PLAN_SURE;
 #ifndef RT_BOX_TREE_PLAN
 #define RT_BOX_TREE_PLAN 2
@@ -125,10 +125,40 @@
   }
   return true;
 }
+inline void sphere_centre(const uint32_t (*lo)[4], const uint32_t (*hi)[4], uint32_t j, float* c) {
+  for (int a = 0; a < 3; a++) c[a] = (hi[j][3] & F_TRANSLATE) ? as_f(lo[j][a]) : 0.f;
+}
+inline void enclosing_spheres(const uint32_t (*lo)[4], const uint32_t (*hi)[4], size_t n, std::vector<uint8_t>* enclosing,
+                              std::vector<uint32_t>* starts = nullptr) {
+  std::vector<uint32_t> spheres;
+  for (size_t j = 0; j < n; j++)
+    if ((hi[j][3] & 0xffu) == OP_SPHERE) spheres.push_back((uint32_t)j);
+  float cmin[3] = {INFINITY, INFINITY, INFINITY}, cmax[3] = {-INFINITY, -INFINITY, -INFINITY};
+  for (uint32_t j : spheres) {
+    float c[3];
+    sphere_centre(lo, hi, j, c);
+    for (int a = 0; a < 3; a++) cmin[a] = fminf(cmin[a], c[a]), cmax[a] = fmaxf(cmax[a], c[a]);
+  }
+  enclosing->assign(n, 0);
+  for (uint32_t j : spheres) {
+    float cj[3];
+    sphere_centre(lo, hi, j, cj);
+    const float r = as_f(lo[j][3]);
+    float far2 = 0.f;
+    for (int a = 0; a < 3; a++) {
+      const float d = fmaxf(cmax[a] - cj[a], cj[a] - cmin[a]);
+      far2 += d * d;
+    }
+    const bool all = spheres.size() > 1 && far2 < r * r;
+    (*enclosing)[j] = all;
+    if (starts && !all && std::isfinite(r) && std::isfinite(cj[0]) && std::isfinite(cj[1]) && std::isfinite(cj[2])) starts->push_back(j);
+  }
+}
 }
 
 inline BoxPlan box_plan(const uint32_t (*lo)[4], const uint32_t (*hi)[4], size_t n, const uint8_t* follower, uint8_t* mask,
-                        uint8_t* sure = nullptr, uint32_t n_probes = BOX_PLAN_PROBES, BoxPlanKind kind = BOX_PLAN_DEFAULT) {
+                        uint8_t* sure = nullptr, uint32_t n_probes = BOX_PLAN_PROBES, BoxPlanKind kind = BOX_PLAN_DEFAULT,
+                        const uint32_t* counts = nullptr, uint64_t count_rays = 0) {
   using namespace box_plan_detail;
   BoxPlan out;
   for (size_t j = 0; j < n; j++) {
@@ -152,34 +182,17 @@
   }
 
   std::vector<uint64_t> n_pass(n, 0);
-  std::vector<uint32_t> spheres, starts;
-  for (size_t j = 0; j < n; j++)
-    if (op(j) == OP_SPHERE) spheres.push_back((uint32_t)j);
-  auto centre = [&](uint32_t j, float* c) {
-    for (int a = 0; a < 3; a++) c[a] = (hi[j][3] & F_TRANSLATE) ? as_f(lo[j][a]) : 0.f;
-  };
-  float cmin[3] = {INFINITY, INFINITY, INFINITY}, cmax[3] = {-INFINITY, -INFINITY, -INFINITY};
-  for (uint32_t j : spheres) {
-    float c[3];
-    centre(j, c);
-    for (int a = 0; a < 3; a++) cmin[a] = fminf(cmin[a], c[a]), cmax[a] = fmaxf(cmax[a], c[a]);
-  }
-  std::vector<uint8_t> enclosing(n, 0);
-  for (uint32_t j : spheres) {
-    float cj[3];
-    centre(j, cj);
-    const float r = as_f(lo[j][3]);
-    float far2 = 0.f;
-    for (int a = 0; a < 3; a++) {
-      const float d = fmaxf(cmax[a] - cj[a], cj[a] - cmin[a]);
-      far2 += d * d;
-    }
-    const bool all = spheres.size() > 1 && far2 < r * r;
-    enclosing[j] = all;
-    if (!all && std::isfinite(r) && std::isfinite(cj[0]) && std::isfinite(cj[1]) && std::isfinite(cj[2])) starts.push_back(j);
-  }
+  std::vector<uint32_t> starts;
+  std::vector<uint8_t> enclosing;
+  enclosing_spheres(lo, hi, n, &enclosing, &starts);
+  auto centre = [&](uint32_t j, float* c) { sphere_centre(lo, hi, j, c); };
   uint64_t n_rays = 0;
-  if (!starts.empty() && kind != BOX_PLAN_AREA) {
+  if (kind == BOX_PLAN_COUNTS) {
+    if (!counts) return out;
+    for (size_t j = 0; j < n; j++)
+      if (op(j) == OP_BOX) n_pass[j] = counts[j] < count_rays ? counts[j] : count_rays;
+    n_rays = count_rays;
+  } else if (!starts.empty() && kind != BOX_PLAN_AREA) {
     Rng rng{0x626f78706c616e31ull ^ (uint64_t)n};
     const float t_near = 0.001f;
     while (n_rays < n_probes) {
diff --git a/rtiow-rust_amd/csrc/rt_camera_probe.h b/rtiow-rust_amd/csrc/rt_camera_probe.h
--- /dev/null
+++ b/rtiow-rust_amd/csrc/rt_camera_probe.h
@@ -0,0 +1,159 @@
+#pragma once
+#include <cmath>
+#include <vector>
+
+#include "rt_box_plan.h"
+#include "rt_trace.h"
+
+namespace rtg {
+
+#ifndef RT_CAMERA_PROBE_PATHS
+#define RT_CAMERA_PROBE_PATHS 4096
+#endif
+#ifndef RT_CAMERA_PROBE_BOUNCES
+#define RT_CAMERA_PROBE_BOUNCES 2
+#endif
+constexpr uint32_t CAMERA_PROBE_PATHS = RT_CAMERA_PROBE_PATHS, CAMERA_PROBE_BOUNCES = RT_CAMERA_PROBE_BOUNCES;
+constexpr uint32_t CAMERA_PROBE_MAX_RECORDS = 4550;
+#ifndef RT_CAMERA_PROBE_TRIPS
+#define RT_CAMERA_PROBE_TRIPS 64
+#endif
+constexpr uint32_t CAMERA_PROBE_TRIPS = RT_CAMERA_PROBE_TRIPS;
+constexpr uint32_t CAMERA_PROBE_STOP = 0x80000000u;
+constexpr uint32_t CAMERA_PROBE_BLOCK = 64, CAMERA_PROBE_WALKERS = 16;
+
+struct CameraProbe {
+  const uint4* lo;
+  const uint4* hi;
+  const uint8_t* stop;
+  uint32_t* n_pass;
+  uint32_t n;
+  uint32_t grid_w, grid_h;
+  uint32_t bounces;
+  uint32_t max_trips;
+  float t_near;
+};
+
+inline void camera_probe_grid(const DevCamera& cam, uint32_t paths, uint32_t* grid_w, uint32_t* grid_h) {
+  const double h = std::sqrt((double)cam.horizontal.x * cam.horizontal.x + (double)cam.horizontal.y * cam.horizontal.y + (double)cam.horizontal.z * cam.horizontal.z);
+  const double v = std::sqrt((double)cam.vertical.x * cam.vertical.x + (double)cam.vertical.y * cam.vertical.y + (double)cam.vertical.z * cam.vertical.z);
+  double aspect = h / v;
+  if (!(aspect > 1.0 / 64.0) || !(aspect < 64.0)) aspect = 1.0;
+  paths = paths < 1u ? 1u : (paths > (1u << 20) ? (1u << 20) : paths);
+  uint32_t w = (uint32_t)std::ceil(std::sqrt((double)paths * aspect));
+  w = w < 1u ? 1u : w;
+  *grid_w = w, *grid_h = (paths + w - 1u) / w;
+}
+
+inline void camera_probe_stops(const uint32_t (*lo)[4], const uint32_t (*hi)[4], size_t n, std::vector<uint8_t>* stop) {
+  box_plan_detail::enclosing_spheres(lo, hi, n, stop);
+  for (size_t j = 0; j < n; j++)
+    if ((hi[j][3] & 0xffu) == OP_SPHERE && ((hi[j][3] >> F_MATKIND_SHIFT) & 7u) == MAT_DIFFUSE_LIGHT) (*stop)[j] = 1;
+}
+
+RT_DEV void camera_probe_path(const CameraProbe& p, const uint4* lo, const uint4* hi, const DevCamera& cam, uint32_t i, uint32_t* s_pass) {
+  uint32_t state = i * 0x9e3779b9u + 0x7f4a7c15u;
+  auto unit = [&]() {
+    state = state * 747796405u + 2891336453u;
+    uint32_t w = ((state >> ((state >> 28) + 4u)) ^ state) * 277803737u;
+    w = (w >> 22) ^ w;
+    return (float)(w >> 8) * (1.0f / 16777216.0f);
+  };
+  const uint32_t cx = i % p.grid_w, cy = i / p.grid_w;
+  const float s = ((float)cx + unit()) * __builtin_amdgcn_rcpf((float)p.grid_w), t = ((float)cy + unit()) * __builtin_amdgcn_rcpf((float)p.grid_h);
+  float lx = 2.f * unit() - 1.f, ly = 2.f * unit() - 1.f;
+  if (lx * lx + ly * ly >= 1.f) lx *= 0.5f, ly *= 0.5f;
+  const V3 offset = vadd(smul(cam.lens_radius * lx, cam.u), smul(cam.lens_radius * ly, cam.v));
+  V3 o = vadd(cam.origin, offset);
+  V3 d = vsub(vsub(vadd(vadd(cam.llc, smul(s, cam.horizontal)), smul(t, cam.vertical)), cam.origin), offset);
+  V3 inv = mk(__builtin_amdgcn_rcpf(d.x), __builtin_amdgcn_rcpf(d.y), __builtin_amdgcn_rcpf(d.z));
+  float dd = vdot(d, d), inv_dd = __builtin_amdgcn_rcpf(dd);
+  float best = F32_MAX, best_r = 1.f;
+  uint32_t best_pc = 0xffffffffu, pc = 0, bounce = 0;
+  V3 best_c = mk(0.f, 0.f, 0.f);
+  bool best_stop = false;
+  atomicAdd(&s_pass[p.n], 1u);
+  const uint32_t bound = (p.bounces + 1u) * (p.n + 1u), max_trips = bound < p.max_trips ? bound : p.max_trips;
+  for (uint32_t trip = 0; trip < max_trips; trip++) {
+    if (pc < p.n) {
+      const uint4 l = lo[pc], h = hi[pc];
+      const uint32_t op = h.w & 0xffu;
+      if (op == OP_BOX) {
+        const float ax = (__uint_as_float(l.x) - o.x) * inv.x, bx = (__uint_as_float(l.y) - o.x) * inv.x;
+        const float ay = (__uint_as_float(l.z) - o.y) * inv.y, by = (__uint_as_float(l.w) - o.y) * inv.y;
+        const float az = (__uint_as_float(h.x) - o.z) * inv.z, bz = (__uint_as_float(h.y) - o.z) * inv.z;
+        const float start = rs_max(p.t_near, rs_max(rs_max(inv.x < 0.f ? bx : ax, inv.y < 0.f ? by : ay), inv.z < 0.f ? bz : az));
+        const float end = rs_min(best, rs_min(rs_min(inv.x < 0.f ? ax : bx, inv.y < 0.f ? ay : by), inv.z < 0.f ? az : bz));
+        if (end > start) {
+          atomicAdd(&s_pass[pc], 1u);
+          pc++;
+        } else {
+          pc = h.z > pc ? h.z : pc + 1u;
+        }
+      } else if (op == OP_SPHERE) {
+        const bool tr = (h.w & F_TRANSLATE) != 0u;
+        const V3 c = tr ? mk(__uint_as_float(l.x), __uint_as_float(l.y), __uint_as_float(l.z)) : mk(0.f, 0.f, 0.f);
+        const float r = __uint_as_float(l.w);
+        const V3 q = vsub(o, c);
+        const float b = vdot(q, d), cc = vdot(q, q) - r * r, disc = b * b - dd * cc;
+        if (disc > 0.f) {
+          const float sq = __builtin_amdgcn_sqrtf(disc);
+          float th = (-b - sq) * inv_dd;
+          if (!(th < best && th >= p.t_near)) th = (-b + sq) * inv_dd;
+          if (th < best && th >= p.t_near) best = th, best_pc = pc, best_c = c, best_r = r, best_stop = (h.w & CAMERA_PROBE_STOP) != 0u;
+        }
+        pc++;
+      } else {
+        pc = p.n;
+      }
+    }
+    if (pc >= p.n) {
+      if (best_pc >= p.n || best_stop || bounce >= p.bounces) break;
+      o = vadd(o, smul(best, d));
+      const V3 nrm = smul(__builtin_amdgcn_rcpf(best_r), vsub(o, best_c));
+      const float wx = 2.f * unit() - 1.f, wy = 2.f * unit() - 1.f, wz = 2.f * unit() - 1.f;
+      const float ws = wx * wx + wy * wy + wz * wz < 1.f ? 1.f : 0.5f;
+      const V3 v = mk(ws * wx, ws * wy, ws * wz);
+      d = vadd(nrm, v);
+      dd = vdot(d, d);
+      if (!(dd < F32_MAX)) break;
+      inv = mk(__builtin_amdgcn_rcpf(d.x), __builtin_amdgcn_rcpf(d.y), __builtin_amdgcn_rcpf(d.z)), inv_dd = __builtin_amdgcn_rcpf(dd);
+      best = F32_MAX, best_pc = 0xffffffffu, best_stop = false, pc = 0, bounce++;
+      atomicAdd(&s_pass[p.n], 1u);
+    }
+  }
+}
+
+inline size_t camera_probe_lds_bytes(size_t n) { return n * 32u + (n + 1u) * sizeof(uint32_t); }
+__global__ __launch_bounds__(CAMERA_PROBE_BLOCK) void camera_probe_kernel(CameraProbe p, DevCamera cam) {
+  extern __shared__ uint4 s_probe[];
+  uint4* s_lo = s_probe;
+  uint4* s_hi = s_probe + p.n;
+  uint32_t* s_pass = reinterpret_cast<uint32_t*>(s_probe + 2u * p.n);
+  for (uint32_t j0 = threadIdx.x; j0 < p.n; j0 += 8u * CAMERA_PROBE_BLOCK) {
+    uint4 l[8], h[8];
+    uint32_t st[8];
+#pragma unroll
+    for (uint32_t k = 0; k < 8u; k++) {
+      const uint32_t j = j0 + k * CAMERA_PROBE_BLOCK;
+      if (j < p.n) l[k] = p.lo[j], h[k] = p.hi[j], st[k] = p.stop[j];
+    }
+#pragma unroll
+    for (uint32_t k = 0; k < 8u; k++) {
+      const uint32_t j = j0 + k * CAMERA_PROBE_BLOCK;
+      if (j < p.n) {
+        if (st[k]) h[k].w |= CAMERA_PROBE_STOP;
+        s_lo[j] = l[k], s_hi[j] = h[k];
+      }
+    }
+  }
+  for (uint32_t j = threadIdx.x; j <= p.n; j += blockDim.x) s_pass[j] = 0u;
+  __syncthreads();
+  const uint32_t i = blockIdx.x * CAMERA_PROBE_WALKERS + threadIdx.x;
+  if (threadIdx.x < CAMERA_PROBE_WALKERS && i < p.grid_w * p.grid_h) camera_probe_path(p, s_lo, s_hi, cam, i, s_pass);
+  __syncthreads();
+  for (uint32_t j = threadIdx.x; j <= p.n; j += blockDim.x)
+    if (s_pass[j]) atomicAdd(&p.n_pass[j], s_pass[j]);
+}
+
+}
diff --git a/rtiow-rust_amd/csrc/rtg_api.hip b/rtiow-rust_amd/csrc/rtg_api.hip
--- a/rtiow-rust_amd/csrc/rtg_api.hip
+++ b/rtiow-rust_amd/csrc/rtg_api.hip
@@ -19,6 +19,7 @@
 #include "../../include/rtiow_gpu_debug.h"
 #include "rt_pool.h"
 #include "rt_box_plan.h"
+#include "rt_camera_probe.h"
 #include "rt_retire.h"
 #include "rt_denoise.h"
 #include "rt_features.h"
@@ -87,6 +88,22 @@
   size_t features_bytes = 0;
 };
 
+constexpr int CAMERA_PLANS = 4;
+constexpr size_t CAMERA_KEY_BYTES = sizeof(DevCamera) + 2;
+struct CameraPlan {
+  enum State { FREE, PROBING, PLANNED } state = FREE;
+  unsigned char key[CAMERA_KEY_BYTES] = {};
+  uint64_t stamp = 0;
+  hipEvent_t ev = nullptr;
+  hipStream_t up_stream = nullptr;
+  uint32_t* d_counts = nullptr;
+  uint32_t* h_words = nullptr;
+  uint32_t* d_off = nullptr;
+  uint32_t bytes = 0;
+  uint32_t n_pruned = 0, n_rays = 0;
+  float plan_ms = 0.f;
+};
+
 struct LeanImages {
   const uint4* lo = nullptr;
   const uint4* hi = nullptr;
@@ -104,6 +121,10 @@
   std::vector<uint8_t> plan_mask;
   std::vector<uint8_t> follower;
   int slot = 12;
+  const std::vector<Packet>* h_lo = nullptr;
+  const std::vector<Packet>* h_hi = nullptr;
+  int probe_ok = -1;
+  uint8_t* d_stop = nullptr;
 };
 
 struct rtg_scene {
@@ -138,6 +159,11 @@
   int box_chains = 1;
   int box_prune = 1;
   int box_tree = 1;
+  int box_camera = 1;
+  int cam_paths = (int)CAMERA_PROBE_PATHS, cam_bounces = (int)CAMERA_PROBE_BOUNCES, cam_trips = (int)CAMERA_PROBE_TRIPS;
+  CameraPlan cam_plans[CAMERA_PLANS];
+  uint64_t cam_clock = 0;
+  std::vector<Packet> t_lo, t_hi;
   LeanImages ref;
   LeanImages tree;
   bool tree_tried = false;
@@ -626,6 +652,8 @@
   if ((rc = lean_images(s, &s->tree, lo, hi, 17)) || (rc = lean_plan(s, &s->tree, lo, hi, BOX_TREE_PLAN))) return rc;
   if (!s->box_chains && (rc = prune_table(s, &s->tree, 0))) return rc;
   s->tree.lo = (const uint4*)s->buffers[15], s->tree.hi = (const uint4*)s->buffers[16];
+  s->t_lo.swap(lo), s->t_hi.swap(hi);
+  s->tree.h_lo = &s->t_lo, s->tree.h_hi = &s->t_hi;
   return RTG_OK;
 }
 
@@ -642,6 +670,14 @@
     if (c.ev1) (void)hipEventDestroy(c.ev1);
     if (c.done) (void)hipEventDestroy(c.done);
   }
+  for (CameraPlan& c : s->cam_plans) {
+    if (c.ev) (void)hipEventDestroy(c.ev);
+    if (c.d_counts) (void)hipFree(c.d_counts);
+    if (c.d_off) (void)hipFree(c.d_off);
+    if (c.h_words) (void)hipHostFree(c.h_words);
+  }
+  for (LeanImages* im : {&s->ref, &s->tree})
+    if (im->d_stop) (void)hipFree(im->d_stop);
   if (s->d_frame) (void)hipFree(s->d_frame);
   if (s->d_lights) (void)hipFree(s->d_lights);
   if (s->d_sampled) (void)hipFree(s->d_sampled);
@@ -733,6 +769,7 @@
     s->plannable = s->dev.lds_image_bytes - LDS_BOX_BYTES * (s->n_box / 2u) <= 160u * 1024u;
     if (s->plannable) {
       s->h_lo = fs.lo, s->h_hi = fs.hi;
+      s->ref.h_lo = &s->h_lo, s->ref.h_hi = &s->h_hi;
       if ((s->box_tree && (rc = tree_program(s))) || (!s->tree.lo && (rc = ref_plan(s)))) {
         rtg_scene_destroy(s);
         return rc;
@@ -794,6 +831,18 @@
   else if (k == "box_prune") {
     if (value < 0 || value > 2) return fail(RTG_ERR_INVALID, "box_prune: 0 .. 2");
     s->box_prune = value;
+  }
+  else if (k == "box_camera") {
+    if (value < 0 || value > 2) return fail(RTG_ERR_INVALID, "box_camera: 0 .. 2");
+    s->box_camera = value;
+  }
+  else if (k == "box_camera_paths" || k == "box_camera_bounces" || k == "box_camera_trips") {
+    HIP_TRY(hipSetDevice(s->device));
+    HIP_TRY(hipDeviceSynchronize());
+    for (CameraPlan& c : s->cam_plans) c.state = CameraPlan::FREE;
+    if (k == "box_camera_paths") s->cam_paths = std::min(1 << 20, std::max(1, value));
+    else if (k == "box_camera_bounces") s->cam_bounces = std::min(16, std::max(0, value));
+    else s->cam_trips = std::max(1, value);
   }
   else if (k == "bvh4") {
     if (value && !s->wide_bytes) return fail(RTG_ERR_INVALID, "bvh4: the scene is not one Bvh of spheres (no 4-wide image)");
diff --git a/rtiow-rust_amd/csrc/rtg_launch.inc b/rtiow-rust_amd/csrc/rtg_launch.inc
--- a/rtiow-rust_amd/csrc/rtg_launch.inc
+++ b/rtiow-rust_amd/csrc/rtg_launch.inc
@@ -163,6 +163,91 @@
   return hipSuccess;
 }
 
+constexpr uint64_t CAMERA_PLAN_MIN_SAMPLES = 33500000ull;
+
+static hipError_t camera_plan_make(rtg_scene* s, const LeanImages& im, CameraPlan* e, bool chains, hipStream_t stream) {
+  hipError_t err = hipEventSynchronize(e->ev);
+  if (err != hipSuccess) return err;
+  const size_t n = im.h_hi->size();
+  const auto t0 = std::chrono::steady_clock::now();
+  std::vector<uint8_t> mask(n), drop(n);
+  e->n_rays = e->h_words[n];
+  e->n_pruned = box_plan(reinterpret_cast<const uint32_t (*)[4]>(im.h_lo->data()), reinterpret_cast<const uint32_t (*)[4]>(im.h_hi->data()), n, im.follower.data(),
+                         mask.data(), nullptr, 0u, BOX_PLAN_COUNTS, e->h_words, e->n_rays).n_pruned;
+  for (size_t i = 0; i < n; i++) drop[i] = mask[i] == BOX_PRUNED || (chains && mask[i] == BOX_FOLLOWER);
+  uint32_t* off = e->h_words + n + 1u;
+  e->bytes = lds_image_offsets(im.plan_ops.data(), n, off, drop.data());
+  e->plan_ms = std::chrono::duration<float, std::milli>(std::chrono::steady_clock::now() - t0).count();
+  if ((err = hipMemcpyAsync(e->d_off, off, n * sizeof(uint32_t), hipMemcpyHostToDevice, stream)) != hipSuccess) return err;
+  if ((err = hipEventRecord(e->ev, stream)) != hipSuccess) return err;
+  e->up_stream = stream, e->state = CameraPlan::PLANNED;
+  if (s->verbose)
+    fprintf(stderr, "[rtg] camera plan: %u rays probed, %u interior record(s) left out (the scene's plan: %u), image %u B, DP + table %.3f ms\n", e->n_rays, e->n_pruned,
+            im.n_pruned, e->bytes, e->plan_ms);
+  return hipSuccess;
+}
+
+static hipError_t camera_plan(rtg_scene* s, LeanImages& im, bool tree, const DevCamera& cam, hipStream_t stream, uint64_t samples, const CameraPlan** out) {
+  *out = nullptr;
+  if (!s->box_camera || !im.h_lo || !im.h_hi) return hipSuccess;
+  const size_t n = im.h_hi->size();
+  if (im.probe_ok < 0) {
+    box_plan_detail::Shape shape;
+    im.probe_ok = n == s->n_prog && n <= CAMERA_PROBE_MAX_RECORDS && box_plan_detail::program_shape(reinterpret_cast<const uint32_t (*)[4]>(im.h_lo->data()), reinterpret_cast<const uint32_t (*)[4]>(im.h_hi->data()), n, &shape) &&
+                  shape.n_prunable != 0u;
+  }
+  if (!im.probe_ok) return hipSuccess;
+  const bool chains = s->box_chains != 0;
+  unsigned char key[CAMERA_KEY_BYTES];
+  memcpy(key, &cam, sizeof(DevCamera));
+  key[sizeof(DevCamera)] = tree ? 1 : 0, key[sizeof(DevCamera) + 1] = chains ? 1 : 0;
+  CameraPlan* e = nullptr;
+  for (CameraPlan& c : s->cam_plans)
+    if (c.state != CameraPlan::FREE && !memcmp(c.key, key, CAMERA_KEY_BYTES)) e = &c;
+  hipError_t err;
+  if (!e) {
+    if (s->box_camera == 1 && samples < CAMERA_PLAN_MIN_SAMPLES) return hipSuccess;
+    for (CameraPlan& c : s->cam_plans)
+      if (c.state == CameraPlan::FREE && (!e || e->state != CameraPlan::FREE)) e = &c;
+      else if (!e || (e->state != CameraPlan::FREE && c.stamp < e->stamp)) e = &c;
+    if (e->state != CameraPlan::FREE) {
+      if ((err = hipDeviceSynchronize()) != hipSuccess) return err;
+      e->state = CameraPlan::FREE;
+    }
+    if (!e->ev && (err = hipEventCreateWithFlags(&e->ev, hipEventDisableTiming)) != hipSuccess) return err;
+    if (!e->d_counts && (err = hipMalloc((void**)&e->d_counts, (n + 1u) * sizeof(uint32_t))) != hipSuccess) return err;
+    if (!e->d_off) {
+      if ((err = hipMalloc((void**)&e->d_off, n * sizeof(uint32_t))) != hipSuccess) return err;
+      s->bytes += (2u * n + 1u) * sizeof(uint32_t);
+    }
+    if (!e->h_words && (err = hipHostMalloc((void**)&e->h_words, (2u * n + 1u) * sizeof(uint32_t))) != hipSuccess) return err;
+    if (!im.d_stop) {
+      std::vector<uint8_t> stop;
+      camera_probe_stops(reinterpret_cast<const uint32_t (*)[4]>(im.h_lo->data()), reinterpret_cast<const uint32_t (*)[4]>(im.h_hi->data()), n, &stop);
+      if ((err = hipMalloc((void**)&im.d_stop, n)) != hipSuccess) return err;
+      if ((err = hipMemcpy(im.d_stop, stop.data(), n, hipMemcpyHostToDevice)) != hipSuccess) return err;
+      s->bytes += n;
+    }
+    CameraProbe p{im.lo, im.hi, im.d_stop, e->d_counts, (uint32_t)n, 0u, 0u, (uint32_t)s->cam_bounces, (uint32_t)s->cam_trips, 0.001f};
+    camera_probe_grid(cam, (uint32_t)s->cam_paths, &p.grid_w, &p.grid_h);
+    if ((err = hipMemsetAsync(e->d_counts, 0, (n + 1u) * sizeof(uint32_t), stream)) != hipSuccess) return err;
+    int probe_per_cu = 0;
+    if ((err = kernel_setup(s, (const void*)camera_probe_kernel, (int)CAMERA_PROBE_BLOCK, camera_probe_lds_bytes(n), &probe_per_cu)) != hipSuccess) return err;
+    hipLaunchKernelGGL(camera_probe_kernel, dim3((p.grid_w * p.grid_h + CAMERA_PROBE_WALKERS - 1u) / CAMERA_PROBE_WALKERS), dim3(CAMERA_PROBE_BLOCK), camera_probe_lds_bytes(n), stream, p, cam);
+    if ((err = hipGetLastError()) != hipSuccess) return err;
+    if ((err = hipMemcpyAsync(e->h_words, e->d_counts, (n + 1u) * sizeof(uint32_t), hipMemcpyDeviceToHost, stream)) != hipSuccess) return err;
+    if ((err = hipEventRecord(e->ev, stream)) != hipSuccess) return err;
+    memcpy(e->key, key, CAMERA_KEY_BYTES);
+    e->state = CameraPlan::PROBING, e->stamp = ++s->cam_clock;
+    if (s->box_camera != 2) return hipSuccess;
+  }
+  e->stamp = ++s->cam_clock;
+  if (e->state == CameraPlan::PROBING && (err = camera_plan_make(s, im, e, chains, stream)) != hipSuccess) return err;
+  if (e->up_stream != stream && (err = hipStreamWaitEvent(stream, e->ev, 0)) != hipSuccess) return err;
+  *out = e;
+  return hipSuccess;
+}
+
 template <bool COUNT>
 static hipError_t launch_pool(rtg_scene* s, const DevCamera& cam, const DevParams& d, float* d_out,
                               hipStream_t stream, const SampleSlice& sl) {
@@ -206,9 +291,29 @@
     if (pool_lds_bytes(dev.lds_image_bytes, s->n_mat, waves, true, false) > lds_limit) tree = false;
   }
   if (!tree && s->ref.lo != nullptr) choose(s->ref);
-  const LeanImages& im = tree ? s->tree : s->ref;
+  LeanImages& im = tree ? s->tree : s->ref;
+  const bool camera_ok = prune && pool_lds_bytes(dev.lds_image_bytes, s->n_mat, waves, true, false) <= lds_limit;
+  const CameraPlan* cplan = nullptr;
+  uint32_t sized_for = 0;
+  auto kernel_for = [&](uint32_t bytes) {
+    const bool u = bytes != 0 && pool_lds_bytes(bytes, s->n_mat, waves, true, false) <= lds_limit;
+    const bool r = s->ray_lds && pool_lds_bytes(bytes, s->n_mat, waves, u, true) <= lds_limit && (!u || bytes < (1u << 17));
+    return (u ? 1u : 0u) | (r ? 2u : 0u);
+  };
+  auto camera_image = [&]() {
+    if (!camera_ok || cplan) return hipSuccess;
+    const CameraPlan* cp = nullptr;
+    hipError_t ec = camera_plan(s, im, tree, cam, stream, pix_work * ns_call, &cp);
+    if (ec != hipSuccess || !cp) return ec;
+    const bool take = sized_for ? cp->bytes <= sized_for : (cp->bytes <= dev.lds_image_bytes || kernel_for(cp->bytes) == kernel_for(dev.lds_image_bytes));
+    if (take) cplan = cp, dev.lds_off = cp->d_off, dev.lds_image_bytes = cp->bytes;
+    else if (s->verbose) fprintf(stderr, "[rtg] camera plan: image %u B against %u B: not staged by this %s\n", cp->bytes, sized_for ? sized_for : dev.lds_image_bytes, sized_for ? "call" : "launch");
+    return hipSuccess;
+  };
+  if (hipError_t ec = camera_image(); ec != hipSuccess) return ec;
   if (wide) dev.lds_off = (const uint32_t*)s->buffers[7], dev.lds_image_bytes = s->wide_bytes;
   const uint32_t image = dev.lds_image_bytes;
+  sized_for = image;
   bool use_lds = image != 0 && pool_lds_bytes(image, s->n_mat, waves, true, false) <= lds_limit;
   if (wide && !use_lds) return hipErrorNotSupported;
   bool ray_lds = s->ray_lds && pool_lds_bytes(image, s->n_mat, waves, use_lds, true) <= lds_limit && (!use_lds || image < (1u << 17));
@@ -223,9 +328,10 @@
   else if (ray_lds) kernel = use_lds ? render_lean_pool<true, COUNT, true> : render_lean_pool<false, COUNT, true>;
   else kernel = use_lds ? render_lean_pool<true, COUNT, false> : render_lean_pool<false, COUNT, false>;
   if (s->verbose && (chains || prune) && use_lds)
-    fprintf(stderr, "[rtg] pool: %s program (%u region(s) rebuilt in %.2f ms), box chains: %u follower record(s)%s, box pruning: %u interior record(s)%s (plan %.2f ms): LDS image %u B, %u records of %u; without followers %u B, full image %u B\n",
-            tree ? "rebuilt" : "reference", s->n_regions, s->tree_ms, im.n_followers, chains || (prune && s->box_chains) ? " dropped" : " kept", im.n_pruned, prune ? " dropped" : " kept", im.plan_ms, image,
-            s->n_prog - (chains || (prune && s->box_chains) ? im.n_followers : 0u) - (prune ? im.n_pruned : 0u), s->n_prog, im.chain_bytes ? im.chain_bytes : im.bytes, im.bytes);
+    fprintf(stderr, "[rtg] pool: %s program (%u region(s) rebuilt in %.2f ms), box chains: %u follower record(s)%s, box pruning: %u interior record(s)%s (%s plan %.2f ms): LDS image %u B, %u records of %u; without followers %u B, full image %u B\n",
+            tree ? "rebuilt" : "reference", s->n_regions, s->tree_ms, im.n_followers, chains || (prune && s->box_chains) ? " dropped" : " kept", cplan ? cplan->n_pruned : im.n_pruned, prune ? " dropped" : " kept",
+            cplan ? "the camera's" : "the scene's", cplan ? cplan->plan_ms : im.plan_ms, image,
+            s->n_prog - (chains || (prune && s->box_chains) ? im.n_followers : 0u) - (prune ? (cplan ? cplan->n_pruned : im.n_pruned) : 0u), s->n_prog, im.chain_bytes ? im.chain_bytes : im.bytes, im.bytes);
   PoolLaunch L{KernelKind::lean_pool, bt, 0, lds, geo, POOL};
   hipError_t e = kernel_setup(s, (const void*)kernel, bt, lds, &L.per_cu);
   if (e != hipSuccess) return e;
@@ -245,6 +351,7 @@
               s0, dp.ns, d.ns, grid, bt, L.per_cu, lds, (int)use_lds, (int)ray_lds, cm.n_chunks, cm.chunk, (cm.lpt_samples - (cm.lpt_samples ? s0 : 0u)) / (cm.chunk ? cm.chunk : 1u));
     hipError_t eg = grow((void**)&s->cx->d_slots, &s->cx->slots_bytes, (size_t)grid * waves * POOL * POOL_FIELDS * sizeof(uint32_t));
     if (eg != hipSuccess) return eg;
+    if (s0 != sl.begin && (eg = camera_image()) != hipSuccess) return eg;
     launch_pass_setup(s, LaunchConsts{cam, dp, cm, make_pixmap(dp)}, queue, stream);
     hipLaunchKernelGGL(kernel, dim3(grid), dim3(bt), lds, stream, dev, (const LaunchConsts*)s->cx->d_consts, d_out, total_work, queue,
                        s->cx->d_counters, s->pool_tune, s->cx->d_slots);
diff --git a/rtiow-rust_amd/csrc/rtg_probes.inc b/rtiow-rust_amd/csrc/rtg_probes.inc
--- a/rtiow-rust_amd/csrc/rtg_probes.inc
+++ b/rtiow-rust_amd/csrc/rtg_probes.inc
@@ -237,6 +237,23 @@
   return (int)m;
 }
 
+int rtg_debug_camera_plan(rtg_builder* b, const rtg_id* world, size_t n, const uint32_t* words, size_t n_records, const uint32_t* counts,
+                          uint64_t n_rays, uint8_t* mask_out, size_t capacity) {
+  if (!counts) return fail(RTG_ERR_INVALID, "null argument");
+  std::vector<Packet> lo, hi;
+  bool lean = true;
+  int rc = debug_lean_program("rtg_debug_camera_plan", b, world, n, words, n_records, &lo, &hi, &lean);
+  if (rc) return rc;
+  std::vector<uint8_t> follower(hi.size(), 0), mask(hi.size(), 0);
+  if (lean && !hi.empty()) {
+    box_chain_followers(reinterpret_cast<const uint32_t (*)[4]>(lo.data()), reinterpret_cast<const uint32_t (*)[4]>(hi.data()), hi.size(), follower.data());
+    box_plan(reinterpret_cast<const uint32_t (*)[4]>(lo.data()), reinterpret_cast<const uint32_t (*)[4]>(hi.data()), hi.size(), follower.data(), mask.data(), nullptr, 0u,
+             BOX_PLAN_COUNTS, counts, n_rays);
+  }
+  if (mask_out) std::memcpy(mask_out, mask.data(), std::min(mask.size(), capacity));
+  return (int)hi.size();
+}
+
 int rtg_debug_math(int device, int op, size_t n, const float* in, const float* in2, float* out) {
   if (!in || !out || op < 0 || op > 5 || (op == 5 && !in2)) return fail(RTG_ERR_INVALID, "bad argument");
   int ndev = 0;
```

New measurement: 8383, median of 6. +4.2%, better.
